# nanless/universal-speech-enhancement

Hardware: AMD Instinct MI355X
Metric: spectrogram-frames/sec through 30-step PC sampler, 24 kHz (higher is better)
Workload: dtype bf16; 1 GPU; configs[1]: NCSN++ Large score net, batch=8x4 s utterances per GPU, 30-step PC sampler (reverse_diffusion + langevin x1, snr 0.5, 60 NFE), bf16, hipGraph=on; global_batch=8, frames_per_utt=601, padded_frames_per_utt=640, n_freq=512, N=30, nfe=60, parallelism=utterance-sharded x1

## Files before the change

### include/use_hip.h

```cpp
#ifndef USE_HIP_H
#define USE_HIP_H

#include <stddef.h>
#include <stdint.h>

#ifdef __cplusplus
extern "C" {
#endif

typedef struct use_handle use_handle;
typedef void* use_stream_t;

enum { USE_OK = 0, USE_E_INVALID = -1, USE_E_HIP = -2, USE_E_STATE = -3, USE_E_NOMEM = -4 };
enum { USE_PREC_FP32 = 0, USE_PREC_BF16 = 1, USE_PREC_FP16 = 2 };
enum { USE_PRED_REVERSE_DIFFUSION = 0, USE_PRED_EULER_MARUYAMA = 1, USE_PRED_NONE = 2 };
enum { USE_CORR_NONE = 0, USE_CORR_LANGEVIN = 1, USE_CORR_ALD = 2 };

typedef struct use_config {
    int nf;
    int n_levels;
    int ch_mult[8];
    int num_res_blocks;
    int n_freq;
    int precision;
    float theta, sigma_min, sigma_max;
    int input_channels;
    int unconditional;
    int no_sigma_scale;
} use_config;

typedef struct use_sampler_config {
    int N;
    int predictor;
    int corrector;
    int corrector_steps;
    float snr;
    float t_eps;
    int use_graph;
} use_sampler_config;

int use_set_option(const char* name, long long value);
const char* use_last_error(void);
const char* use_version(void);

int use_create(const use_config* cfg, int device, use_handle** out);
int use_destroy(use_handle* h);

int use_set_weight(use_handle* h, const char* name, const float* data, const int64_t* shape, int ndim);
int use_commit_weights(use_handle* h);
int use_alloc_weight_blob(use_handle* h);
int use_weight_blob(use_handle* h, void** dev_ptr, size_t* bytes);
int use_save_weight_blob(use_handle* h, const char* path);
int use_load_weight_blob(use_handle* h, const char* path);
int use_num_expected_weights(use_handle* h);
int use_expected_weight(use_handle* h, int index, const char** name, int64_t* shape4, int* ndim);

int use_plan(use_handle* h, int B, int Tpad);
int use_workspace_bytes(use_handle* h, size_t* bytes);

int use_score(use_handle* h, const void* x, const void* y, const float* t, void* out, use_stream_t stream);
int use_score2(use_handle* h, const void* x, const void* y, const void* y2, const float* t, void* out, use_stream_t stream);

int use_set_sampler(use_handle* h, const use_sampler_config* sc);
int use_num_noise_draws(use_handle* h);
int use_get_timesteps(use_handle* h, float* out, int n);
int use_sample(use_handle* h, const void* y, const void* noise, uint64_t seed, void* out, use_stream_t stream);
int use_sample_cond(use_handle* h, const void* y, const void* cond, const void* noise, uint64_t seed, void* out, use_stream_t stream);
int use_sample_cond2(use_handle* h, const void* y, const void* cond, const void* cond2, const void* noise, uint64_t seed, void* out,
                     use_stream_t stream);

int use_sample_items(use_handle* h, const void* y, const void* cond, const void* cond2, const void* noise,
                     const uint64_t* seeds_host , void* out, use_stream_t stream);

typedef struct use_ode_config {
    float rtol, atol;
    float t_eps;
    int N;
    int group;
    int denoise;
    float first_step, max_step;
    int max_nfe;
    int use_graph;
} use_ode_config;
enum { USE_ODE_FINISHED = 0, USE_ODE_TOO_SMALL_STEP = -1, USE_ODE_MAX_NFE = -2 };
int use_set_ode(use_handle* h, const use_ode_config* cfg);
int use_sample_ode(use_handle* h, const void* y, const void* cond, const void* cond2, const void* noise, uint64_t seed, void* out,
                   int* nfev, int* status, use_stream_t stream);
typedef struct use_ode use_ode;
int use_ode_create(use_handle* h, int B, int64_t n_per_item, const use_ode_config* cfg, use_ode** out);
int use_ode_start(use_ode* o, const void* y_sde, const void* x0, use_stream_t stream);
int use_ode_request(use_ode* o, void* x, float* t, use_stream_t stream);
int use_ode_supply(use_ode* o, const void* f, int kind, use_stream_t stream);
int use_ode_result(use_ode* o, void* out, int* nfev, int* status, use_stream_t stream);
int use_ode_state(use_ode* o, double* t, double* h_abs, int* nfev, int* status, int* steps, use_stream_t stream);
int use_ode_num_groups(use_ode* o);
int use_ode_destroy(use_ode* o);

int use_sde_prior(use_handle* h, const void* y, const void* noise, uint64_t seed, void* x, int64_t n, use_stream_t s);
int use_sde_predictor(use_handle* h, int predictor, float t, int N, const void* x, const void* y, const void* score,
                      const void* noise, uint64_t seed, void* x_out, void* x_mean, int64_t n, use_stream_t s);
int use_sde_corrector(use_handle* h, int corrector, float t, float snr, int B, const void* x, const void* score,
                      const void* noise, uint64_t seed, void* x_out, void* x_mean, int64_t n, use_stream_t s);

int use_fill_noise(use_handle* h, uint64_t seed, int draw, void* out, int64_t n, use_stream_t s);

int use_fill_noise_items(use_handle* h, const uint64_t* seeds_host , int B, int draw, void* out,
                         int64_t n , use_stream_t s);

int use_forward(use_handle* h, const void* x, const void* y, const float* t, void* out, use_stream_t stream);

int use_spec_fwd(const void* stft, void* Y, int B, int F, int T, int Tpad, float factor, float exponent, use_stream_t s);
int use_spec_back(const void* X, void* stft, int B, int F, int T, int Tpad, float factor, float exponent, use_stream_t s);

int use_stft_fwd(const float* wav, void* Y, int B, int L, int n_fft, int hop, const float* window, int Tpad, float factor,
                 float exponent, use_stream_t s);
int use_istft_back(const void* X, float* wav, int B, int L, int n_fft, int hop, const float* window, int Tpad, float factor,
                   float exponent, use_stream_t s);

int use_chunk_count(int Tp, int C, int overlap);
int use_chunk_split(const void* Y, void* chunks, int B, int F, int Tp, int C, int overlap, use_stream_t s);
int use_chunk_merge(const void* chunks, void* X, int B, int F, int Tp, int C, int overlap, use_stream_t s);

enum { USE_METRIC_SI_SDR = 0, USE_METRIC_SI_SIR = 1, USE_METRIC_SI_SAR = 2, USE_METRIC_LSD = 3, USE_METRIC_COUNT = 4 };
size_t use_metrics_workspace(int B, int stride);
int use_metrics(const float* est, const float* clean, const float* noise, const int* len_host, int B, int stride, void* work,
                size_t work_bytes, double* out_dev, use_stream_t s);

int use_get_stat(use_handle* h, const char* name, long long* value);
int use_profile_score(use_handle* h, const void* x, const void* y, const float* t, void* out, use_stream_t stream,
                      double* conv_ms, double* conv_flops, double* conv_bytes, int* conv_launches, double* total_ms);
int use_profile_aux(use_handle* h, int index, char* name, int name_cap, int* H, int* W, double* bytes, double* ms);
int use_profile_aux_flops(use_handle* h, int index, double* flops);
typedef struct use_conv_case {
    int B, H, W, C0, C1, Cout, XC0, XC1;
    int act, gn, temb, res, stats;
    int dtype;
    int variant, iters;
} use_conv_case;
int use_conv_bench(const use_conv_case* c, float* out_host, float* stats_host, double* ms_avg, double* flops);
typedef struct use_conv_op {
    int B, H, W, C0, C1, Cout, XC0, XC1, ntaps, act, dtype, out_dtype, variant;
    const void *src0, *src1;
    const float* coef;
    const float* w;
    const float* bias;
    const float* temb;
    const void *x0, *x1;
    const float* w2;
    const void* res;
    float out_scale;
    void* out;
    long long* stats;
    const float* pyr;
    const float* w4;
    const float* b4;
    const long long *gn_st0, *gn_st1;
    const float *gn_gamma, *gn_beta;
    int gn_groups;
    float gn_eps;
    int temb_bstride;
} use_conv_op;
int use_op_conv(const use_conv_op* c, use_stream_t stream);
size_t use_op_conv_dev_workspace(const use_conv_op* c);
int use_op_conv_dev(const use_conv_op* c, int w_mode, void* work, size_t work_bytes, use_stream_t stream);
int use_op_fir(const void* src, int dtype, const float* coef, int act, void* out_act, void* out_raw, int B, int H, int W, int C, int up,
               use_stream_t stream);
int use_op_attention(const void* q, const void* k, const void* v, void* out, int dtype, int B, int N, int C, use_stream_t stream);
int use_op_gn_finalize(const long long* st0, int C0, const long long* st1, int C1, const float* gamma, const float* beta, int groups,
                       int hw, float eps, float* coef, int B, use_stream_t stream);
int use_op_attn_block(const void* x, const long long* gn_st, const float* gamma, const float* beta, int groups, float eps, const void* wq,
                      const void* wk, const void* wv, const void* wo, const float* bq, const float* bk, const float* bv, const float* bo,
                      void* out, long long* stats, int dtype, int B, int N, int C, use_stream_t stream);
int use_op_combine_add(void* h, int dtype, const float* pyr, const float* w8, const float* b8, long long* stats, int B, int64_t pix_per_b, int C,
                       use_stream_t stream);
int use_op_temb_mlp(const float* t, int t_stride, const float* gfp_w, const float* w1, const float* b1, const float* w2, const float* b2,
                    float* out_silu, int B, int nf, use_stream_t stream);
int use_op_temb_dense(const float* silu_temb, const float* W, const float* bias, float* out, int B, int rows, int dim, use_stream_t stream);
int use_op_score_out(const float* pyr, int pc, const float* t, int t_stride, const float* w, const float* bias, void* score, int B,
                     int64_t pix_per_b, float sign, use_stream_t stream);
int use_op_pack_input(const void* x, const void* y, const void* y2, float* x4, int64_t npix, use_stream_t stream);
int use_op_softmax_rows(void* x, int dtype, int64_t rows, int cols, use_stream_t stream);
int use_op_transpose_nc(const void* in, void* out, int dtype, int B, int N, int C, use_stream_t stream);
size_t use_op_wgrad_workspace(int B, int H, int W, int Cout, int Cin, int ntaps, int dtype);
int use_op_wgrad(const void* dy, const void* x, int dtype, float* dw, float* db, int B, int H, int W, int Cout, int Cin, int ntaps, float alpha,
                 float* work, size_t work_floats, use_stream_t stream);
size_t use_op_gn_workspace(int B, int C, int groups);
int use_op_gn_act_bwd(const void* x, const void* dy, int dtype, const float* gamma, const float* beta, int groups, float eps, int act, const void* add,
                      float add_scale, int B, int HW, int C, float* work, int have_stats, void* dx, float* dgamma, float* dbeta, use_stream_t stream);
int use_op_gn_act_fwd(const void* x, int dtype, const float* gamma, const float* beta, int groups, float eps, int act, int B, int HW, int C, float* work,
                      void* y, use_stream_t stream);
int use_op_colsum(const void* x, int dtype, int B, int HW, int C, float scale, float* out, float* work, use_stream_t stream);
int use_op_dense_bwd(const float* g, const float* temb, const float* Wd, int B, int K, int Cout, float* dW, float* db, float* dtemb,
                     use_stream_t stream);
int use_op_attention_bwd(const float* q, const float* k, const float* v, const float* dO, float* work, float* dq, float* dk, float* dv, int B, int N,
                         int C, use_stream_t stream);
enum { USE_WAV_PCM16 = 0, USE_WAV_FLOAT32 = 1 };
int use_wav_read(const char* path, double** samples, int64_t* frames, int* channels, int* sample_rate);
int use_wav_write(const char* path, const float* samples, int64_t frames, int channels, int sample_rate, int subtype);
int use_resample_fft(const double* x, int64_t n, int64_t num, double* y);
int use_load_utterance(const char* path, int target_rate, int normalize, float** wav, int64_t* length, int* sample_rate);
void use_free(void* p);

int use_timesteps(int N, float t_eps, float* out);
int use_debug_tensor(use_handle* h, const char* name, void** dev_ptr, int* dims4, int* dtype);
double use_flops_per_score(use_handle* h);

#ifdef __cplusplus
}
#endif
#endif
```

### universal_speech_enhancement_amd/_lib.py

```python
from __future__ import annotations

import ctypes as C
import os

_HERE = os.path.dirname(os.path.abspath(__file__))
LIB_PATH = os.environ.get("USE_HIP_LIB") or os.path.join(_HERE, "libuse_hip.so")

PREC = {"fp32": 0, "bf16": 1, "fp16": 2}
PREDICTORS = {"reverse_diffusion": 0, "euler_maruyama": 1, "none": 2}
CORRECTORS = {"none": 0, "langevin": 1, "ald": 2}


class UseConfig(C.Structure):
    _fields_ = [("nf", C.c_int), ("n_levels", C.c_int), ("ch_mult", C.c_int * 8), ("num_res_blocks", C.c_int),
                ("n_freq", C.c_int), ("precision", C.c_int), ("theta", C.c_float), ("sigma_min", C.c_float),
                ("sigma_max", C.c_float), ("input_channels", C.c_int), ("unconditional", C.c_int),
                ("no_sigma_scale", C.c_int)]


class UseSamplerConfig(C.Structure):
    _fields_ = [("N", C.c_int), ("predictor", C.c_int), ("corrector", C.c_int), ("corrector_steps", C.c_int),
                ("snr", C.c_float), ("t_eps", C.c_float), ("use_graph", C.c_int)]


class UseOdeConfig(C.Structure):
    _fields_ = [("rtol", C.c_float), ("atol", C.c_float), ("t_eps", C.c_float), ("N", C.c_int), ("group", C.c_int), ("denoise", C.c_int),
                ("first_step", C.c_float), ("max_step", C.c_float), ("max_nfe", C.c_int), ("use_graph", C.c_int)]


class UseConvCase(C.Structure):
    _fields_ = [(k, C.c_int) for k in ("B", "H", "W", "C0", "C1", "Cout", "XC0", "XC1", "act", "gn", "temb", "res", "stats",
                                       "dtype", "variant", "iters")]


class UseConvOp(C.Structure):
    _fields_ = ([(k, C.c_int) for k in ("B", "H", "W", "C0", "C1", "Cout", "XC0", "XC1", "ntaps", "act", "dtype", "out_dtype", "variant")] +
                [(k, C.c_void_p) for k in ("src0", "src1", "coef", "w", "bias", "temb", "x0", "x1", "w2", "res")] +
                [("out_scale", C.c_float), ("out", C.c_void_p), ("stats", C.c_void_p)] +
                [(k, C.c_void_p) for k in ("pyr", "w4", "b4", "gn_st0", "gn_st1", "gn_gamma", "gn_beta")] +
                [("gn_groups", C.c_int), ("gn_eps", C.c_float), ("temb_bstride", C.c_int)])


class UseHipError(RuntimeError):
    pass


_lib = None

_vp, _i, _i64, _u64, _f = C.c_void_p, C.c_int, C.c_int64, C.c_uint64, C.c_float
SYMBOLS = {
    "use_set_option": (C.c_int, [C.c_char_p, C.c_longlong]),
    "use_last_error": (C.c_char_p, []),
    "use_version": (C.c_char_p, []),
    "use_create": (_i, [C.POINTER(UseConfig), _i, C.POINTER(_vp)]),
    "use_destroy": (_i, [_vp]),
    "use_set_weight": (_i, [_vp, C.c_char_p, _vp, C.POINTER(_i64), _i]),
    "use_commit_weights": (_i, [_vp]),
    "use_alloc_weight_blob": (_i, [_vp]),
    "use_weight_blob": (_i, [_vp, C.POINTER(_vp), C.POINTER(C.c_size_t)]),
    "use_save_weight_blob": (C.c_int, [C.c_void_p, C.c_char_p]),
    "use_load_weight_blob": (C.c_int, [C.c_void_p, C.c_char_p]),
    "use_num_expected_weights": (_i, [_vp]),
    "use_expected_weight": (_i, [_vp, _i, C.POINTER(C.c_char_p), C.POINTER(_i64), C.POINTER(_i)]),
    "use_plan": (_i, [_vp, _i, _i]),
    "use_workspace_bytes": (_i, [_vp, C.POINTER(C.c_size_t)]),
    "use_score": (_i, [_vp, _vp, _vp, _vp, _vp, _vp]),
    "use_forward": (_i, [_vp, _vp, _vp, _vp, _vp, _vp]),
    "use_score2": (_i, [_vp, _vp, _vp, _vp, _vp, _vp, _vp]),
    "use_sample_cond2": (_i, [_vp, _vp, _vp, _vp, _vp, _u64, _vp, _vp]),
    "use_sample_items": (_i, [_vp, _vp, _vp, _vp, _vp, C.POINTER(_u64), _vp, _vp]),
    "use_set_sampler": (_i, [_vp, C.POINTER(UseSamplerConfig)]),
    "use_num_noise_draws": (_i, [_vp]),
    "use_get_timesteps": (_i, [_vp, C.POINTER(_f), _i]),
    "use_sample": (_i, [_vp, _vp, _vp, _u64, _vp, _vp]),
    "use_sample_cond": (_i, [_vp, _vp, _vp, _vp, _u64, _vp, _vp]),
    "use_set_ode": (_i, [_vp, C.POINTER(UseOdeConfig)]),
    "use_sample_ode": (_i, [_vp, _vp, _vp, _vp, _vp, _u64, _vp, C.POINTER(_i), C.POINTER(_i), _vp]),
    "use_ode_create": (_i, [_vp, _i, _i64, C.POINTER(UseOdeConfig), C.POINTER(_vp)]),
    "use_ode_start": (_i, [_vp, _vp, _vp, _vp]),
    "use_ode_request": (_i, [_vp, _vp, _vp, _vp]),
    "use_ode_supply": (_i, [_vp, _vp, _i, _vp]),
    "use_ode_result": (_i, [_vp, _vp, C.POINTER(_i), C.POINTER(_i), _vp]),
    "use_ode_state": (_i, [_vp, C.POINTER(C.c_double), C.POINTER(C.c_double), C.POINTER(_i), C.POINTER(_i), C.POINTER(_i), _vp]),
    "use_ode_num_groups": (_i, [_vp]),
    "use_ode_destroy": (_i, [_vp]),
    "use_spec_fwd": (_i, [_vp, _vp, _i, _i, _i, _i, C.c_float, C.c_float, _vp]),
    "use_spec_back": (_i, [_vp, _vp, _i, _i, _i, _i, C.c_float, C.c_float, _vp]),
    "use_stft_fwd": (_i, [_vp, _vp, _i, _i, _i, _i, _vp, _i, C.c_float, C.c_float, _vp]),
    "use_istft_back": (_i, [_vp, _vp, _i, _i, _i, _i, _vp, _i, C.c_float, C.c_float, _vp]),
    "use_chunk_count": (_i, [_i, _i, _i]),
    "use_chunk_split": (_i, [_vp, _vp, _i, _i, _i, _i, _i, _vp]),
    "use_chunk_merge": (_i, [_vp, _vp, _i, _i, _i, _i, _i, _vp]),
    "use_metrics_workspace": (C.c_size_t, [_i, _i]),
    "use_metrics": (_i, [_vp, _vp, _vp, C.POINTER(_i), _i, _i, _vp, C.c_size_t, _vp, _vp]),
    "use_sde_prior": (_i, [_vp, _vp, _vp, _u64, _vp, _i64, _vp]),
    "use_fill_noise": (_i, [_vp, _u64, _i, _vp, _i64, _vp]),
    "use_fill_noise_items": (_i, [_vp, C.POINTER(_u64), _i, _i, _vp, _i64, _vp]),
    "use_sde_predictor": (_i, [_vp, _i, _f, _i, _vp, _vp, _vp, _vp, _u64, _vp, _vp, _i64, _vp]),
    "use_sde_corrector": (_i, [_vp, _i, _f, _f, _i, _vp, _vp, _vp, _u64, _vp, _vp, _i64, _vp]),
    "use_debug_tensor": (_i, [_vp, C.c_char_p, C.POINTER(_vp), C.POINTER(_i), C.POINTER(_i)]),
    "use_flops_per_score": (C.c_double, [_vp]),
    "use_get_stat": (_i, [_vp, C.c_char_p, C.POINTER(C.c_longlong)]),
    "use_profile_aux": (_i, [_vp, _i, C.c_char_p, _i, C.POINTER(_i), C.POINTER(_i), C.POINTER(C.c_double), C.POINTER(C.c_double)]),
    "use_profile_aux_flops": (_i, [_vp, _i, C.POINTER(C.c_double)]),
    "use_profile_score": (_i, [_vp, _vp, _vp, _vp, _vp, _vp, C.POINTER(C.c_double), C.POINTER(C.c_double), C.POINTER(C.c_double), C.POINTER(_i), C.POINTER(C.c_double)]),
    "use_timesteps": (_i, [_i, _f, C.POINTER(_f)]),
    "use_conv_bench": (_i, [C.POINTER(UseConvCase), _vp, _vp, C.POINTER(C.c_double), C.POINTER(C.c_double)]),
    "use_op_conv": (_i, [C.POINTER(UseConvOp), _vp]),
    "use_op_conv_dev_workspace": (C.c_size_t, [C.POINTER(UseConvOp)]),
    "use_op_conv_dev": (_i, [C.POINTER(UseConvOp), _i, _vp, C.c_size_t, _vp]),
    "use_op_fir": (_i, [_vp, _i, _vp, _i, _vp, _vp, _i, _i, _i, _i, _i, _vp]),
    "use_op_attention": (_i, [_vp, _vp, _vp, _vp, _i, _i, _i, _i, _vp]),
    "use_op_gn_finalize": (_i, [_vp, _i, _vp, _i, _vp, _vp, _i, _i, _f, _vp, _i, _vp]),
    "use_op_attn_block": (_i, [_vp, _vp, _vp, _vp, _i, _f, _vp, _vp, _vp, _vp, _vp, _vp, _vp, _vp, _vp, _vp, _i, _i, _i, _i, _vp]),
    "use_op_combine_add": (_i, [_vp, _i, _vp, _vp, _vp, _vp, _i, _i64, _i, _vp]),
    "use_op_temb_mlp": (_i, [_vp, _i, _vp, _vp, _vp, _vp, _vp, _vp, _i, _i, _vp]),
    "use_op_temb_dense": (_i, [_vp, _vp, _vp, _vp, _i, _i, _i, _vp]),
    "use_op_score_out": (_i, [_vp, _i, _vp, _i, _vp, _vp, _vp, _i, _i64, _f, _vp]),
    "use_op_pack_input": (_i, [_vp, _vp, _vp, _vp, _i64, _vp]),
    "use_op_softmax_rows": (_i, [_vp, _i, _i64, _i, _vp]),
    "use_op_transpose_nc": (_i, [_vp, _vp, _i, _i, _i, _i, _vp]),
    "use_op_wgrad_workspace": (C.c_size_t, [_i, _i, _i, _i, _i, _i, _i]),
    "use_op_wgrad": (_i, [_vp, _vp, _i, _vp, _vp, _i, _i, _i, _i, _i, _i, _f, _vp, C.c_size_t, _vp]),
    "use_op_gn_workspace": (C.c_size_t, [_i, _i, _i]),
    "use_op_gn_act_bwd": (_i, [_vp, _vp, _i, _vp, _vp, _i, _f, _i, _vp, _f, _i, _i, _i, _vp, _i, _vp, _vp, _vp, _vp]),
    "use_op_gn_act_fwd": (_i, [_vp, _i, _vp, _vp, _i, _f, _i, _i, _i, _i, _vp, _vp, _vp]),
    "use_op_colsum": (_i, [_vp, _i, _i, _i, _i, _f, _vp, _vp, _vp]),
    "use_op_attention_bwd": (_i, [_vp, _vp, _vp, _vp, _vp, _vp, _vp, _vp, _i, _i, _i, _vp]),
    "use_op_dense_bwd": (_i, [_vp, _vp, _vp, _i, _i, _i, _vp, _vp, _vp, _vp]),
    "use_wav_read": (_i, [C.c_char_p, C.POINTER(C.POINTER(C.c_double)), C.POINTER(_i64), C.POINTER(_i), C.POINTER(_i)]),
    "use_wav_write": (_i, [C.c_char_p, _vp, _i64, _i, _i, _i]),
    "use_resample_fft": (_i, [_vp, _i64, _i64, _vp]),
    "use_load_utterance": (_i, [C.c_char_p, _i, _i, C.POINTER(C.POINTER(C.c_float)), C.POINTER(_i64), C.POINTER(_i)]),
    "use_free": (None, [_vp]),
}


def lib() -> C.CDLL:
    global _lib
    if _lib is None:
        if not os.path.exists(LIB_PATH):
            raise UseHipError(
                f"{LIB_PATH} not found: the HIP extension is not built (run __graft_entry__.build()). "
                "There is no CPU fallback for the sampling path.")
        L = C.CDLL(LIB_PATH)
        for name, (res, args) in SYMBOLS.items():
            if os.environ.get("USE_HIP_LIB") and not hasattr(L, name):
                continue
            fn = getattr(L, name)
            fn.restype, fn.argtypes = res, args
        for kv in filter(None, os.environ.get("USE_HIP_OPTS", "").split(",")):
            k, sep, v = kv.partition("=")
            if not sep or not k.strip():
                raise UseHipError(f"USE_HIP_OPTS: entry {kv!r} is not name=value")
            try:
                iv = int(v)
            except ValueError:
                raise UseHipError(f"USE_HIP_OPTS: {kv!r}: the value must be an integer") from None
            if L.use_set_option(k.strip().encode(), iv) < 0:
                raise UseHipError(f"USE_HIP_OPTS: {kv}: " + L.use_last_error().decode(errors="replace"))
        _lib = L
    return _lib


def check(rc: int, what: str = "") -> int:
    if rc < 0:
        msg = lib().use_last_error().decode(errors="replace")
        raise UseHipError(f"{what or 'libuse_hip'} failed ({rc}): {msg}")
    return rc
```

### universal_speech_enhancement_amd/csrc/use_engine.cpp

```cpp
#include "../../include/use_hip.h"
#include "use_kernels.h"

#include <hip/hip_runtime.h>

#include <algorithm>
#include <cmath>
#include <cstdarg>
#include <cstdio>
#include <cstdlib>
#include <cstring>
#include <map>
#include <mutex>
#include <string>
#include <unordered_map>
#include <vector>

using namespace use;

static thread_local std::string g_err;
static int fail(int code, const char* fmt, ...) {
    char buf[1024];
    va_list ap; va_start(ap, fmt); vsnprintf(buf, sizeof buf, fmt, ap); va_end(ap);
    g_err = buf;
    return code;
}
int use_set_error(int code, const char* msg) { g_err = msg ? msg : ""; return code; }
#define HIPCHK(expr)                                                                                         \
    do {                                                                                                     \
        hipError_t e_ = (expr);                                                                              \
        if (e_ != hipSuccess) return fail(USE_E_HIP, "%s failed: %s (%s:%d)", #expr, hipGetErrorString(e_), __FILE__, __LINE__); \
    } while (0)

static inline uint16_t f32_to_bf16(float f) {
    uint32_t u; memcpy(&u, &f, 4);
    if ((u & 0x7fffffffu) > 0x7f800000u) return (uint16_t)((u >> 16) | 0x40);
    u += 0x7fffu + ((u >> 16) & 1u);
    return (uint16_t)(u >> 16);
}

static inline uint16_t f32_to_f16(float f) {
    uint32_t u; memcpy(&u, &f, 4);
    const uint32_t sign = (u >> 16) & 0x8000u;
    u &= 0x7fffffffu;
    if (u > 0x7f800000u) return (uint16_t)(sign | 0x7e00u);
    if (u >= 0x477ff000u) return (uint16_t)(sign | 0x7c00u);
    if (u < 0x38800000u) {
        if (u < 0x33000000u) return (uint16_t)sign;
        const int shift = 126 - (int)(u >> 23);
        uint32_t m = (u & 0x7fffffu) | 0x800000u;
        const uint32_t half = 1u << (shift - 1), rest = m & ((1u << shift) - 1);
        m >>= shift;
        if (rest > half || (rest == half && (m & 1))) ++m;
        return (uint16_t)(sign | m);
    }
    uint32_t v = u - 0x38000000u;
    const uint32_t rest = v & 0x1fffu;
    v >>= 13;
    if (rest > 0x1000u || (rest == 0x1000u && (v & 1))) ++v;
    return (uint16_t)(sign | v);
}

struct ConvW { std::string wname, bname; int cin = 0, cout = 0, cout_pad = 0, ntaps = 1, w_dtype = DT_F32;
               bool nin = false; size_t w_off = 0, b_off = 0;
               int cin_src = 0, cout_src = 0;
               size_t wb_off = 0; bool has_wb = false;
               bool split_in = false; };
struct GNW { std::string prefix; int C = 0; size_t g_off = 0, b_off = 0; };
struct ResW { int idx = 0, in_ch = 0, out_ch = 0; bool up = false, down = false, has_c2 = false;
              GNW gn0, gn1; ConvW c0, c1, c2; int dense_row0 = 0; size_t b12_off = 0; };
struct CombineW { int idx = 0, C = 0; size_t w_off = 0, b_off = 0; };
struct AttnW { int idx = 0, C = 0; GNW gn; ConvW q, k, v, o; };
struct PyrW { GNW gn; ConvW conv; };

struct Expected { std::string name; std::vector<int64_t> shape; };

constexpr int MAX_SUB = 8;

struct Act { void* p = nullptr; int C = 0, H = 0, W = 0, dtype = DT_F32; long long* stats = nullptr;
             long long* part = nullptr; int ntiles = 0; };

struct Arena {
    char* base = nullptr; size_t cap = 0, off = 0, peak = 0;
    bool overflow = false;
    bool* dry_on_overflow = nullptr;
    void reset() { off = 0; }
    void* alloc(size_t bytes) {
        off = (off + 255) & ~(size_t)255;
        void* p = base ? (void*)(base + off) : nullptr;
        off += bytes;
        if (off > peak) peak = off;
        if (base && off > cap) {
            overflow = true;
            if (dry_on_overflow) *dry_on_overflow = true;
            p = base;
        }
        return p;
    }
};

struct use_handle {
    use_config cfg{};
    int device = 0;
    int act_dtype = DT_F32;
    std::vector<Expected> expected;
    std::unordered_map<std::string, size_t> expected_index;
    ConvW conv_in;
    std::vector<ResW> res;
    std::vector<CombineW> combines;
    AttnW attn;
    std::vector<PyrW> pyrs;
    int dense_rows = 0;
    size_t gfp_off = 0, l1w_off = 0, l1b_off = 0, l2w_off = 0, l2b_off = 0, dense_w_off = 0, dense_b_off = 0,
           outw_off = 0, outb_off = 0;
    size_t blob_bytes = 0;
    std::unordered_map<std::string, std::vector<float>> host_w;
    char* blob = nullptr; bool weights_ready = false;
    int B = 0, T = 0;
    Arena arena;
    char* persist = nullptr; size_t persist_bytes = 0;
    size_t arena_alloc = 0, persist_alloc = 0;
    size_t arena_plan_bytes = 0;
    float *x4 = nullptr, *silu_temb = nullptr, *tembias = nullptr, *t_dev = nullptr;
    float2 *Y = nullptr, *X = nullptr, *Xmean = nullptr, *score = nullptr, *xin = nullptr;
    float2 *cond_buf = nullptr, *cond2_buf = nullptr;
    int pcp = 4;
    float2 *Cond = nullptr;
    float *lang_partial = nullptr, *lang_step = nullptr;
    unsigned long long* rng_state = nullptr;
    unsigned long long* item_seeds = nullptr;
    float* item_step = nullptr;
    int lang_blocks = 0;
    use_sampler_config sc{};
    bool sampler_set = false;
    std::vector<float> timesteps;
    float* ts_dev = nullptr; float* temb_table = nullptr; float* silu_table = nullptr;
    float2* noise_copy = nullptr; size_t noise_copy_bytes = 0;
    hipStream_t cap_stream = nullptr;
    int nsub = 1, sub_B[MAX_SUB] = {};
    Arena sub_arena[MAX_SUB];
    Arena st_arena[MAX_SUB];
    hipStream_t aux_stream[MAX_SUB] = {};
    hipEvent_t ev_fork = nullptr, ev_stagger[MAX_SUB] = {},
               ev_join[MAX_SUB] = {};
    int debug_B = 0;
    std::vector<hipGraphExec_t> graph_exec[4];
    hipGraphExec_t score_graph = nullptr;
    use_ode_config oc{};
    bool ode_set = false;
    use_ode* ode_run = nullptr;
    hipGraphExec_t ode_graph = nullptr;
    std::vector<const void*> ode_graph_key;
    long long ode_steps = 0, ode_rejected = 0, ode_nfev_max = 0;
    struct PlanState;
    std::vector<PlanState*> plan_cache;
    long long opt_gen_at_plan = -1;
    long long n_graph_captures = 0, n_plans_built = 0, n_plan_cache_hits = 0;
    char* sde_buf = nullptr; unsigned long long* sde_rng = nullptr; float* sde_step = nullptr; float* sde_partial = nullptr; unsigned long long* sde_seeds = nullptr;
    static constexpr int SDE_MAX_B = 1024, SDE_BLOCKS = 128;
    bool profile = false, profile_all = false; std::vector<std::pair<hipEvent_t, hipEvent_t>> prof_events; std::vector<double> prof_flops, prof_bytes; std::vector<char> prof_main; std::vector<std::pair<int, int>> prof_hw;
    struct AuxProf { std::string name; int H = 0, W = 0; double bytes = 0.0; hipEvent_t e0 = nullptr, e1 = nullptr; double ms = 0.0; double flops = 0.0; };
    std::vector<AuxProf> prof_aux;
    std::vector<std::string> prof_desc;
    bool dry = false;
    std::map<std::string, Act> debug;
    double flops = 0.0;
};

static void add_expected(use_handle* h, const std::string& name, std::vector<int64_t> shape) {
    h->expected_index[name] = h->expected.size();
    h->expected.push_back({name, std::move(shape)});
}

static ConvW make_conv(use_handle* h, const std::string& prefix, int cin, int cout, int ntaps, int w_dtype,
                       int cin_src = 0, int cout_src = 0) {
    ConvW c; c.wname = prefix + ".weight"; c.bname = prefix + ".bias"; c.cin = cin; c.cout = cout; c.ntaps = ntaps;
    c.w_dtype = w_dtype;
    c.cin_src = cin_src ? cin_src : cin; c.cout_src = cout_src ? cout_src : cout;
    c.cout_pad = cout <= 32 ? 32 : (cout + 127) / 128 * 128;
    const int k = ntaps == 9 ? 3 : 1;
    add_expected(h, c.wname, {c.cout_src, c.cin_src, k, k});
    add_expected(h, c.bname, {c.cout_src});
    return c;
}
static ConvW make_nin(use_handle* h, const std::string& prefix, int C, int w_dtype) {
    ConvW c; c.wname = prefix + ".W"; c.bname = prefix + ".b"; c.cin = C; c.cout = C; c.ntaps = 1; c.w_dtype = w_dtype;
    c.nin = true; c.cout_pad = (C + 127) / 128 * 128; c.cin_src = C; c.cout_src = C;
    add_expected(h, c.wname, {C, C});
    add_expected(h, c.bname, {C});
    return c;
}
static GNW make_gn(use_handle* h, const std::string& prefix, int C) {
    GNW g; g.prefix = prefix; g.C = C;
    add_expected(h, prefix + ".weight", {C});
    add_expected(h, prefix + ".bias", {C});
    return g;
}

static ResW make_res(use_handle* h, int idx, int in_ch, int out_ch, bool up, bool down) {
    const std::string p = "all_modules." + std::to_string(idx);
    const int dt = h->act_dtype;
    ResW r; r.idx = idx; r.in_ch = in_ch; r.out_ch = out_ch; r.up = up; r.down = down;
    r.gn0 = make_gn(h, p + ".GroupNorm_0", in_ch);
    r.c0 = make_conv(h, p + ".Conv_0", in_ch, out_ch, 9, dt);
    add_expected(h, p + ".Dense_0.weight", {out_ch, 4 * h->cfg.nf});
    add_expected(h, p + ".Dense_0.bias", {out_ch});
    r.dense_row0 = h->dense_rows; h->dense_rows += out_ch;
    r.gn1 = make_gn(h, p + ".GroupNorm_1", out_ch);
    r.c1 = make_conv(h, p + ".Conv_1", out_ch, out_ch, 9, dt);
    r.has_c2 = (in_ch != out_ch) || up || down;
    if (r.has_c2) r.c2 = make_conv(h, p + ".Conv_2", in_ch, out_ch, 1, dt);
    return r;
}

static int build_arch(use_handle* h) {
    const use_config& c = h->cfg;
    const int nf = c.nf, L = c.n_levels, nrb = c.num_res_blocks, dt = h->act_dtype;
    const int pc = c.input_channels ? c.input_channels : 4;
    const int pcp = pc > 4 ? 8 : 4;
    h->pcp = pcp;
    add_expected(h, "output_layer.weight", {2, pc, 1, 1});
    add_expected(h, "output_layer.bias", {2});
    int m = 0;
    add_expected(h, "all_modules.0.W", {nf}); m++;
    if (!c.unconditional) {
        add_expected(h, "all_modules.1.weight", {4 * nf, 2 * nf}); add_expected(h, "all_modules.1.bias", {4 * nf}); m++;
        add_expected(h, "all_modules.2.weight", {4 * nf, 4 * nf}); add_expected(h, "all_modules.2.bias", {4 * nf}); m++;
    }
    h->conv_in = make_conv(h, "all_modules." + std::to_string(m), pcp, nf, 9, DT_F32, pc, 0); m++;
    std::vector<int> hs_c{nf};
    int in_ch = nf;
    for (int lvl = 0; lvl < L; ++lvl) {
        for (int k = 0; k < nrb; ++k) {
            const int out_ch = nf * c.ch_mult[lvl];
            h->res.push_back(make_res(h, m++, in_ch, out_ch, false, false));
            in_ch = out_ch; hs_c.push_back(in_ch);
        }
        if (lvl != L - 1) {
            h->res.push_back(make_res(h, m++, in_ch, in_ch, false, true));
            CombineW cb; cb.idx = m; cb.C = in_ch;
            add_expected(h, "all_modules." + std::to_string(m) + ".Conv_0.weight", {in_ch, pc, 1, 1});
            add_expected(h, "all_modules." + std::to_string(m) + ".Conv_0.bias", {in_ch});
            h->combines.push_back(cb); m++;
            hs_c.push_back(in_ch);
        }
    }
    in_ch = hs_c.back();
    h->res.push_back(make_res(h, m++, in_ch, in_ch, false, false));
    {
        const std::string p = "all_modules." + std::to_string(m);
        h->attn.idx = m; h->attn.C = in_ch;
        h->attn.gn = make_gn(h, p + ".GroupNorm_0", in_ch);
        h->attn.q = make_nin(h, p + ".NIN_0", in_ch, dt);
        h->attn.k = make_nin(h, p + ".NIN_1", in_ch, dt);
        h->attn.v = make_nin(h, p + ".NIN_2", in_ch, dt);
        h->attn.o = make_nin(h, p + ".NIN_3", in_ch, dt);
        m++;
    }
    h->res.push_back(make_res(h, m++, in_ch, in_ch, false, false));
    for (int lvl = L - 1; lvl >= 0; --lvl) {
        for (int k = 0; k < nrb + 1; ++k) {
            const int out_ch = nf * c.ch_mult[lvl];
            const int skip = hs_c.back(); hs_c.pop_back();
            h->res.push_back(make_res(h, m++, in_ch + skip, out_ch, false, false));
            in_ch = out_ch;
        }
        PyrW pw;
        pw.gn = make_gn(h, "all_modules." + std::to_string(m), in_ch); m++;
        pw.conv = make_conv(h, "all_modules." + std::to_string(m), in_ch, pcp, 9, dt, 0, pc); m++;
        h->pyrs.push_back(pw);
        if (lvl != 0) h->res.push_back(make_res(h, m++, in_ch, in_ch, true, false));
    }
    if (!hs_c.empty()) return fail(USE_E_INVALID, "internal: skip stack not empty");

    size_t off = 0;
    auto take = [&](size_t bytes) { off = (off + 255) & ~(size_t)255; size_t o = off; off += bytes; return o; };
    auto lay_conv = [&](ConvW& w) {
        w.w_off = take((size_t)w.ntaps * w.cout_pad * w.cin * dtype_size(w.w_dtype));
        w.b_off = take((size_t)w.cout * 4);
        w.has_wb = !w.nin && w.cout_pad % 128 == 0 && w.cin % conv_v4_chunk(w.w_dtype) == 0 && (w.ntaps == 9 || w.ntaps == 1);
        if (w.has_wb) w.wb_off = take((size_t)w.ntaps * w.cout_pad * w.cin * dtype_size(w.w_dtype));
    };
    auto lay_conv_in = [&](ConvW& w) {
        lay_conv(w);
        if (dt != DT_F32 && w.cin == 4 && w.ntaps == 9 && w.cout_pad % 128 == 0) {
            w.split_in = true; w.has_wb = true;
            w.wb_off = take((size_t)w.cout_pad * CONV_IN_SPLIT_K * 2);
        }
    };
    auto lay_gn = [&](GNW& g) { g.g_off = take((size_t)g.C * 4); g.b_off = take((size_t)g.C * 4); };
    h->outw_off = take((size_t)2 * pcp * 4); h->outb_off = take(2 * 4);
    h->gfp_off = take((size_t)nf * 4);
    h->l1w_off = take((size_t)4 * nf * 2 * nf * 4); h->l1b_off = take((size_t)4 * nf * 4);
    h->l2w_off = take((size_t)4 * nf * 4 * nf * 4); h->l2b_off = take((size_t)4 * nf * 4);
    h->dense_w_off = take((size_t)h->dense_rows * 4 * nf * 4); h->dense_b_off = take((size_t)h->dense_rows * 4);
    lay_conv_in(h->conv_in);
    for (auto& r : h->res) {
        lay_gn(r.gn0); lay_conv(r.c0); lay_gn(r.gn1); lay_conv(r.c1);
        if (r.has_c2) { lay_conv(r.c2); r.b12_off = take((size_t)r.out_ch * 4); }
    }
    for (auto& cb : h->combines) { cb.w_off = take((size_t)cb.C * pcp * 4); cb.b_off = take((size_t)cb.C * 4); }
    lay_gn(h->attn.gn); lay_conv(h->attn.q); lay_conv(h->attn.k); lay_conv(h->attn.v); lay_conv(h->attn.o);
    for (auto& p : h->pyrs) { lay_gn(p.gn); lay_conv(p.conv); }
    h->blob_bytes = (off + 255) & ~(size_t)255;
    return USE_OK;
}

static void pack_conv_raw(const float* src, const ConvW& w, char* dst, char* dstb) {
    const size_t es = dtype_size(w.w_dtype);
    auto put = [&](char* base, size_t o, float v) {
        if (w.w_dtype == DT_F32) ((float*)base)[o] = v;
        else ((uint16_t*)base)[o] = w.w_dtype == DT_F16 ? f32_to_f16(v) : f32_to_bf16(v);
    };
    memset(dst, 0, (size_t)w.ntaps * w.cout_pad * w.cin * es);
    for (int tap = 0; tap < w.ntaps; ++tap)
        for (int co = 0; co < w.cout_src; ++co)
            for (int ci = 0; ci < w.cin_src; ++ci) {
                const float v = w.nin ? src[(size_t)ci * w.cout + co] : src[((size_t)co * w.cin_src + ci) * w.ntaps + tap];
                put(dst, ((size_t)co * w.ntaps + tap) * w.cin + ci, v);
            }
    if (dstb) {
        const int ck = conv_v4_chunk(w.w_dtype), nchunks = w.cin / ck;
        memset(dstb, 0, (size_t)w.ntaps * w.cout_pad * w.cin * es);
        for (int tap = 0; tap < w.ntaps; ++tap)
            for (int co = 0; co < w.cout_src; ++co)
                for (int ci = 0; ci < w.cin_src; ++ci) {
                    const float v = src[((size_t)co * w.cin_src + ci) * w.ntaps + tap];
                    const int vec = 16 / (int)es, e = ci % ck;
                    put(dstb, (((size_t)tap * nchunks + ci / ck) * w.cout_pad + co) * ck + (((e / vec) ^ ((co >> 2) & 3)) * vec + e % vec), v);
                }
    }
}
static void pack_conv_in_split(const float* src, const ConvW& w, char* dst) {
    uint16_t* d = (uint16_t*)dst;
    memset(dst, 0, (size_t)w.cout_pad * CONV_IN_SPLIT_K * 2);
    for (int co = 0; co < w.cout_src; ++co)
        for (int tap = 0; tap < 9; ++tap)
            for (int ci = 0; ci < w.cin_src; ++ci) {
                const float v = src[((size_t)co * w.cin_src + ci) * 9 + tap];
                const uint16_t hi = f32_to_bf16(v);
                uint32_t hb = (uint32_t)hi << 16; float hf; memcpy(&hf, &hb, 4);
                const uint16_t lo = f32_to_bf16(v - hf);
                uint16_t* row = d + (size_t)co * CONV_IN_SPLIT_K;
                row[(0 * 9 + tap) * 4 + ci] = hi; row[(1 * 9 + tap) * 4 + ci] = lo; row[(2 * 9 + tap) * 4 + ci] = hi;
            }
}
static void pack_conv(const use_handle* h, const ConvW& w, char* blob) {
    const std::vector<float>& bias = h->host_w.at(w.bname);
    pack_conv_raw(h->host_w.at(w.wname).data(), w, blob + w.w_off, (w.has_wb && !w.split_in) ? blob + w.wb_off : nullptr);
    if (w.split_in) pack_conv_in_split(h->host_w.at(w.wname).data(), w, blob + w.wb_off);
    memset(blob + w.b_off, 0, (size_t)w.cout * 4);
    memcpy(blob + w.b_off, bias.data(), (size_t)w.cout_src * 4);
}
static void pack_gn(const use_handle* h, const GNW& g, char* blob) {
    memcpy(blob + g.g_off, h->host_w.at(g.prefix + ".weight").data(), (size_t)g.C * 4);
    memcpy(blob + g.b_off, h->host_w.at(g.prefix + ".bias").data(), (size_t)g.C * 4);
}

static int pack_all(use_handle* h, char* blob) {
    for (const auto& e : h->expected)
        if (!h->host_w.count(e.name)) return fail(USE_E_STATE, "weight '%s' was never set", e.name.c_str());
    const int nf = h->cfg.nf;
    auto cp = [&](size_t off, const char* name) {
        const auto& v = h->host_w.at(name); memcpy(blob + off, v.data(), v.size() * 4);
    };
    const int pc = h->cfg.input_channels ? h->cfg.input_channels : 4;
    const int pcp = h->pcp;
    auto cp_rows = [&](size_t off, const std::string& name, int rows) {
        const auto& v = h->host_w.at(name);
        float* d = (float*)(blob + off);
        for (int r = 0; r < rows; ++r)
            for (int k = 0; k < pcp; ++k) d[r * pcp + k] = k < pc ? v[(size_t)r * pc + k] : 0.f;
    };
    cp_rows(h->outw_off, "output_layer.weight", 2); cp(h->outb_off, "output_layer.bias");
    cp(h->gfp_off, "all_modules.0.W");
    if (!h->cfg.unconditional) {
        cp(h->l1w_off, "all_modules.1.weight"); cp(h->l1b_off, "all_modules.1.bias");
        cp(h->l2w_off, "all_modules.2.weight"); cp(h->l2b_off, "all_modules.2.bias");
    }
    pack_conv(h, h->conv_in, blob);
    for (const auto& r : h->res) {
        pack_gn(h, r.gn0, blob); pack_conv(h, r.c0, blob); pack_gn(h, r.gn1, blob); pack_conv(h, r.c1, blob);
        const std::string p = "all_modules." + std::to_string(r.idx);
        if (r.has_c2) {
            pack_conv(h, r.c2, blob);
            const auto& b1 = h->host_w.at(p + ".Conv_1.bias"); const auto& b2 = h->host_w.at(p + ".Conv_2.bias");
            float* d = (float*)(blob + r.b12_off);
            for (int i = 0; i < r.out_ch; ++i) d[i] = b1[i] + b2[i];
        }
        memcpy(blob + h->dense_w_off + (size_t)r.dense_row0 * 4 * nf * 4, h->host_w.at(p + ".Dense_0.weight").data(),
               (size_t)r.out_ch * 4 * nf * 4);
        memcpy(blob + h->dense_b_off + (size_t)r.dense_row0 * 4, h->host_w.at(p + ".Dense_0.bias").data(),
               (size_t)r.out_ch * 4);
    }
    for (const auto& cb : h->combines) {
        const std::string p = "all_modules." + std::to_string(cb.idx);
        cp_rows(cb.w_off, p + ".Conv_0.weight", cb.C); cp(cb.b_off, (p + ".Conv_0.bias").c_str());
    }
    pack_gn(h, h->attn.gn, blob);
    pack_conv(h, h->attn.q, blob); pack_conv(h, h->attn.k, blob); pack_conv(h, h->attn.v, blob); pack_conv(h, h->attn.o, blob);
    for (const auto& p : h->pyrs) { pack_gn(h, p.gn, blob); pack_conv(h, p.conv, blob); }
    return USE_OK;
}

static int g_subbatch_min_items = 2;
static int g_subbatch = -1;
static long g_gn_inline = 128L * 160L;
static int g_attn_fused = 1;
static int g_stats_part = 1;
static int g_stagger_level = 2;

__global__ __launch_bounds__(256) void zero16_kernel(uint4* __restrict__ p, size_t n16) {
    for (size_t i = (size_t)blockIdx.x * 256 + threadIdx.x; i < n16; i += (size_t)gridDim.x * 256) p[i] = make_uint4(0, 0, 0, 0);
}

struct Fwd {
    use_handle* h; hipStream_t s;
    const float* tembias; int temb_bstride;
    const float* t; int t_stride;
    int B = 0;
    Arena* arena = nullptr;
    Arena* st_arena = nullptr;
    bool primary = true;
    hipEvent_t ev_stagger = nullptr;
    int stagger_level = 2;
    template <typename T> const T* W(size_t off) const { return (const T*)(h->blob + off); }

    Act new_act(int C, int H, int Wd, int dtype, bool stats) {
        Act a; a.C = C; a.H = H; a.W = Wd; a.dtype = dtype;
        a.p = arena->alloc((size_t)B * H * Wd * C * dtype_size(dtype));
        if (stats) a.stats = (long long*)st_arena->alloc((size_t)B * C * 2 * sizeof(long long));
        return a;
    }

    template <typename F> void timed_aux(const char* name, int Hm, int Wm, double bytes, F&& launch) {
        if (!h->profile) { launch(); return; }
        use_handle::AuxProf a{name, Hm, Wm, bytes, nullptr, nullptr, 0.0};
        (void)hipEventCreate(&a.e0); (void)hipEventCreate(&a.e1);
        (void)hipEventRecord(a.e0, s);
        launch();
        (void)hipEventRecord(a.e1, s);
        h->prof_aux.push_back(a);
    }

    float* gn_coef(const Act& a, const Act* a2, const GNW& g) {
        const int C = a.C + (a2 ? a2->C : 0);
        float* coef = (float*)arena->alloc((size_t)B * C * 2 * 4);
        if (!h->dry)
            launch_gn_finalize(a.stats, a.C, a2 ? a2->stats : nullptr, a2 ? a2->C : 0, W<float>(g.g_off), W<float>(g.b_off),
                               std::min(C / 4, 32), a.H * a.W, 1e-6f, coef, B, s, a.part, a.ntiles, a2 ? a2->part : nullptr, a2 ? a2->ntiles : 0);
        return coef;
    }

    Act conv(const Act& a, const Act* a2, const GNW* gn, int act, const ConvW& w, const float* temb,
             const Act* res, float scale, const float* pyr, const CombineW* cb, int out_dtype, bool stats,
             const Act* sx0 = nullptr, const Act* sx1 = nullptr, const ConvW* w2 = nullptr, size_t bias_off = 0) {
        Act o = new_act(w.cout, a.H, a.W, out_dtype, stats);
        double fl = 2.0 * B * a.H * a.W * (double)w.cout * w.cin * w.ntaps;
        if (w2) fl += 2.0 * B * a.H * a.W * (double)w2->cout * w2->cin;
        h->flops += fl;
        const float* coef_arr = (gn && (long)a.H * a.W > g_gn_inline) ? gn_coef(a, a2, *gn) : nullptr;
        const bool in_shape = a.dtype == DT_F32 && w.cin <= 8 && w.ntaps == 9 && out_dtype != DT_F32;
        const bool v4_shape = w.ntaps == 9 && w.cout > 32 && a.dtype == out_dtype && a.H % 16 == 0 && a.W % 32 == 0;
        const int part_rows = in_shape ? conv_in_split_wgs(a.H, a.W) : v4_shape ? conv_v4_tiles(a.H, a.W) : 0;
        long long* part = (stats && g_stats_part && part_rows > 0 && (long)a.H * a.W > g_gn_inline)
                              ? (long long*)arena->alloc((size_t)B * part_rows * w.cout * 2 * sizeof(long long)) : nullptr;
        if (h->dry) return o;
        ConvArgs p{};
        p.src0 = a.p; p.C0 = a.C; p.src1 = a2 ? a2->p : nullptr; p.C1 = a2 ? a2->C : 0; p.in_dtype = a.dtype;
        p.coef = coef_arr; p.act = act; p.w = h->blob + w.w_off; p.cout_pad = w.cout_pad;
        if (gn && !coef_arr) {
            const int C = a.C + (a2 ? a2->C : 0), groups = std::min(C / 4, 32);
            p.gn_st0 = a.stats; p.gn_st1 = a2 ? a2->stats : nullptr;
            p.gn_gamma = W<float>(gn->g_off); p.gn_beta = W<float>(gn->b_off); p.gn_groups = groups;
            p.gn_inv_n = 1.0f / ((float)(C / groups) * (float)(a.H * a.W)); p.gn_eps = 1e-6f;
        }
        p.wb = w.has_wb ? h->blob + w.wb_off : nullptr;
        p.bias = W<float>(w2 ? bias_off : w.b_off);
        if (w2) { p.x0 = sx0->p; p.XC0 = sx0->C; p.x1 = sx1 ? sx1->p : nullptr; p.XC1 = sx1 ? sx1->C : 0; p.w2 = h->blob + w2->w_off;
                  p.w2b = w2->has_wb ? h->blob + w2->wb_off : nullptr; }
        p.temb = temb; p.temb_bstride = temb_bstride;
        p.res = res ? res->p : nullptr; p.out_scale = scale;
        p.pyr = pyr; p.w4 = cb ? W<float>(cb->w_off) : nullptr; p.b4 = cb ? W<float>(cb->b_off) : nullptr;
        p.out = o.p; p.out_dtype = out_dtype; p.stats = o.stats;
        p.B = B; p.H = a.H; p.W = a.W; p.Cout = w.cout; p.ntaps = w.ntaps;
        const bool main_variant = conv_v4_eligible(p);
        if (const int nparts = part ? conv_stats_parts(p) : 0) {
            if (nparts <= part_rows) { p.stats_part = part; p.stats = nullptr; o.part = part; o.ntiles = nparts; }
        }
        if (gn && !coef_arr && (a.part || (a2 && a2->part))) { arena->overflow = true; h->dry = true; return o; }
        if (h->profile && (main_variant || (h->profile_all && conv_v2_eligible(p)))) {
            hipEvent_t e0, e1; (void)hipEventCreate(&e0); (void)hipEventCreate(&e1);
            (void)hipEventRecord(e0, s);
            launch_conv(p, s);
            (void)hipEventRecord(e1, s);
            h->prof_events.push_back({e0, e1});
            h->prof_flops.push_back(fl); h->prof_main.push_back(main_variant); h->prof_hw.push_back({a.H, a.W});
            {
                const double es = (double)dtype_size(a.dtype), px = (double)B * a.H * a.W;
                double by = px * (w.cin + (w2 ? w2->cin : 0)) * es + px * w.cout * dtype_size(out_dtype) * (res ? 2.0 : 1.0);
                by += (double)w.ntaps * w.cin * w.cout * es + (w2 ? (double)w2->cin * w2->cout * es : 0.0);
                if (pyr) by += px * 4 * 4;
                h->prof_bytes.push_back(by);
            }
            char d[160]; snprintf(d, sizeof d, "%-28s H=%3d W=%3d Cin=%3d Cout=%3d taps=%d gn=%d res=%d sc=%d", w.wname.c_str(), a.H, a.W, w.cin, w.cout, w.ntaps, gn != nullptr, res != nullptr, w2 ? w2->cin : 0);
            h->prof_desc.push_back(d);
        } else if (h->profile && w.ntaps == 9 && w.cout > 8 && !(a.dtype == DT_F32 && w.cin <= 8)) {
            const double es = (double)dtype_size(a.dtype), px = (double)B * a.H * a.W;
            double by = px * (w.cin + (w2 ? w2->cin : 0)) * es + px * w.cout * dtype_size(out_dtype) * (res ? 2.0 : 1.0);
            by += (double)w.ntaps * w.cin * w.cout * es + (w2 ? (double)w2->cin * w2->cout * es : 0.0);
            timed_aux(conv_sk_eligible(p) ? "conv_sk" : conv_v2_eligible(p) ? "conv_v2" : "conv_generic", a.H, a.W, by, [&] { launch_conv(p, s); });
            h->prof_aux.back().flops = fl;
        } else if (h->profile && (w.cout <= 8 || (a.dtype == DT_F32 && w.cin <= 8))) {
            const double px = (double)B * a.H * a.W;
            const double by = px * w.cin * dtype_size(a.dtype) + px * w.cout * dtype_size(out_dtype) * (res ? 2.0 : 1.0) + (double)w.ntaps * w.cin * w.cout * dtype_size(a.dtype);
            timed_aux(w.cout <= 8 ? "pyr_conv" : "conv_in", a.H, a.W, by, [&] { launch_conv(p, s); });
        } else {
            launch_conv(p, s);
        }
        return o;
    }

    Act resblock(const Act& x, const Act* skip, const ResW& r, const float* pyr = nullptr, const CombineW* cb = nullptr) {
        const float rs = 0.70710678118654752440f;
        const float* temb = tembias ? tembias + r.dense_row0 : nullptr;
        const int dt = h->act_dtype;
        Act hcur, xr;
        const Act* sx0 = &x; const Act* sx1 = skip;
        if (r.up || r.down) {
            const int H2 = r.up ? x.H * 2 : x.H / 2, W2 = r.up ? x.W * 2 : x.W / 2;
            Act hr = new_act(x.C, H2, W2, dt, false);
            xr = new_act(x.C, H2, W2, dt, false);
            float* coef0 = gn_coef(x, skip, r.gn0);
            if (!h->dry) {
                const double by = (double)B * x.H * x.W * x.C * dtype_size(dt) + 2.0 * B * H2 * W2 * x.C * dtype_size(dt);
                if (r.up) timed_aux("fir_up", x.H, x.W, by, [&] { launch_fir_up2(x.p, dt, coef0, 1, hr.p, xr.p, B, x.H, x.W, x.C, s); });
                else      timed_aux("fir_down", x.H, x.W, by, [&] { launch_fir_down2(x.p, dt, coef0, 1, hr.p, xr.p, B, x.H, x.W, x.C, s); });
            }
            hcur = conv(hr, nullptr, nullptr, 0, r.c0, temb, nullptr, 1.f, nullptr, nullptr, dt, true);
            sx0 = &xr; sx1 = nullptr;
        } else {
            hcur = conv(x, skip, &r.gn0, 1, r.c0, temb, nullptr, 1.f, nullptr, nullptr, dt, true);
        }
        if (r.has_c2)
            return conv(hcur, nullptr, &r.gn1, 1, r.c1, nullptr, nullptr, rs, pyr, cb, dt, true, sx0, sx1, &r.c2, r.b12_off);
        return conv(hcur, nullptr, &r.gn1, 1, r.c1, nullptr, &x, rs, pyr, cb, dt, true);
    }

    Act attention(const Act& x, const AttnW& aw) {
        const int dt = h->act_dtype;
        if (g_attn_fused && x.stats && attn_fused_eligible(dt, x.H * x.W, x.C)) {
            Act o = new_act(x.C, x.H, x.W, dt, true);
            h->flops += 4.0 * 2.0 * B * x.H * x.W * (double)x.C * x.C;
            if (h->dry) return o;
            if (x.part) { arena->overflow = true; h->dry = true; return o; }
            AttnArgs a{};
            a.x = x.p; a.out = o.p; a.N = x.H * x.W;
            a.gn_st = x.stats; a.gn_gamma = W<float>(aw.gn.g_off); a.gn_beta = W<float>(aw.gn.b_off); a.gn_groups = std::min(x.C / 4, 32); a.gn_eps = 1e-6f;
            a.wq = h->blob + aw.q.w_off; a.wk = h->blob + aw.k.w_off; a.wv = h->blob + aw.v.w_off; a.wo = h->blob + aw.o.w_off;
            a.bq = W<float>(aw.q.b_off); a.bk = W<float>(aw.k.b_off); a.bv = W<float>(aw.v.b_off); a.bo = W<float>(aw.o.b_off);
            a.stats = o.stats;
            launch_attn_fused(a, dt, B, s);
            return o;
// ... 35 lines not shown
        }
        return conv(a, nullptr, nullptr, 0, aw.o, nullptr, &x, 0.70710678118654752440f, nullptr, nullptr, dt, true);
    }

    Act run(const float* x4) {
        use_handle* H = h;
        const use_config& c = H->cfg;
        const int L = c.n_levels, nrb = c.num_res_blocks, dt = H->act_dtype;
        arena->reset();
        st_arena->reset();
        if (!H->dry && st_arena->base) {
            const size_t n16 = st_arena->cap / 16;
            hipLaunchKernelGGL(zero16_kernel, dim3((unsigned)std::min<size_t>((n16 + 255) / 256, 1024)), dim3(256), 0, s, (uint4*)st_arena->base, n16);
        }
        if (primary) { H->flops = 0.0; H->debug.clear(); H->debug_B = B; }
        const int pcp = H->pcp;
        Act xin; xin.p = (void*)x4; xin.C = pcp; xin.H = c.n_freq; xin.W = H->T; xin.dtype = DT_F32;
        std::vector<Act> hs;
        hs.push_back(conv(xin, nullptr, nullptr, 0, H->conv_in, nullptr, nullptr, 1.f, nullptr, nullptr, dt, true));
        if (primary) H->debug["h_in"] = hs.back();
        Act ipyr = xin;
        size_t ri = 0, ci = 0;
        for (int lvl = 0; lvl < L; ++lvl) {
            for (int k = 0; k < nrb; ++k) hs.push_back(resblock(hs.back(), nullptr, H->res[ri++]));
            if (lvl == std::min(stagger_level, L - 1) && ev_stagger && !H->dry) (void)hipEventRecord(ev_stagger, s);
            if (lvl != L - 1) {
                Act nip = new_act(pcp, ipyr.H / 2, ipyr.W / 2, DT_F32, false);
                if (!H->dry) launch_fir_down2(ipyr.p, DT_F32, nullptr, 0, nullptr, nip.p, B, ipyr.H, ipyr.W, pcp, s);
                ipyr = nip;
                if (pcp == 4) {
                    hs.push_back(resblock(hs.back(), nullptr, H->res[ri++], (const float*)ipyr.p, &H->combines[ci++]));
                } else {
                    Act o = resblock(hs.back(), nullptr, H->res[ri++]);
                    const CombineW& cb = H->combines[ci++];
                    if (!H->dry) {
                        hipLaunchKernelGGL(zero16_kernel, dim3((unsigned)(((size_t)B * o.C + 255) / 256)), dim3(256), 0, s, (uint4*)o.stats,
                                           (size_t)B * o.C);
                        launch_combine_add(o.p, o.dtype, (const float*)ipyr.p, W<float>(cb.w_off), W<float>(cb.b_off), o.stats, B,
                                           (long)o.H * o.W, o.C, s);
                    }
                    o.part = nullptr; o.ntiles = 0;
                    hs.push_back(o);
                }
            }
        }
        if (primary) H->debug["down_out"] = hs.back();
        Act hc = resblock(hs.back(), nullptr, H->res[ri++]);
        if (primary) H->debug["pre_attn"] = hc;
        hc = attention(hc, H->attn);
        if (primary) H->debug["post_attn"] = hc;
        hc = resblock(hc, nullptr, H->res[ri++]);
        Act pyr; bool have_pyr = false; size_t pi = 0;
        for (int lvl = L - 1; lvl >= 0; --lvl) {
            for (int k = 0; k < nrb + 1; ++k) {
                Act sk = hs.back(); hs.pop_back();
                hc = resblock(hc, &sk, H->res[ri++]);
            }
            const PyrW& pw = H->pyrs[pi++];
            if (!have_pyr) {
                pyr = conv(hc, nullptr, &pw.gn, 1, pw.conv, nullptr, nullptr, 1.f, nullptr, nullptr, DT_F32, false);
                have_pyr = true;
            } else {
                Act up = new_act(pcp, pyr.H * 2, pyr.W * 2, DT_F32, false);
                if (!H->dry) launch_fir_up2(pyr.p, DT_F32, nullptr, 0, nullptr, up.p, B, pyr.H, pyr.W, pcp, s);
                pyr = conv(hc, nullptr, &pw.gn, 1, pw.conv, nullptr, &up, 1.f, nullptr, nullptr, DT_F32, false);
            }
            if (lvl != 0) hc = resblock(hc, nullptr, H->res[ri++]);
        }
        if (primary) H->debug["h_last"] = hc;
        if (primary) H->debug["pyramid"] = pyr;
        return pyr;
    }
};

static void run_temb(use_handle* h, const float* t, int n, float* silu_buf, float* out, hipStream_t s) {
    const int nf = h->cfg.nf;
    launch_temb_mlp(t, 1, (const float*)(h->blob + h->gfp_off), (const float*)(h->blob + h->l1w_off),
                    (const float*)(h->blob + h->l1b_off), (const float*)(h->blob + h->l2w_off),
                    (const float*)(h->blob + h->l2b_off), silu_buf, n, nf, s);
    launch_temb_dense(silu_buf, (const float*)(h->blob + h->dense_w_off), (const float*)(h->blob + h->dense_b_off), out,
                      n, h->dense_rows, 4 * nf, s);
}

static void run_score(use_handle* h, const float2* x, const float2* y, const float* tembias, int temb_bstride,
                      const float* t, int t_stride, float2* out, hipStream_t s, float sign = -1.f, const float2* y2 = nullptr) {
    if (h->cfg.no_sigma_scale) t = nullptr;
    const long n_per_b = (long)h->cfg.n_freq * h->T;
    const int pcp = h->pcp;
    launch_pack_input(x, y, y2, h->x4, (long)h->B * n_per_b, s);
    const float* outw = (const float*)(h->blob + h->outw_off); const float* outb = (const float*)(h->blob + h->outb_off);
    if (h->nsub == 1) {
        Fwd f0{h, s, tembias, temb_bstride, t, t_stride};
        f0.B = h->B; f0.arena = &h->arena; f0.st_arena = &h->st_arena[0];
        Act pyr = f0.run(h->x4);
        if (!h->dry) launch_score_out((const float*)pyr.p, pcp, t, t_stride, outw, outb, out, h->B, n_per_b, sign, s);
        return;
    }
    const bool overlap = !h->profile;
    if (overlap) (void)hipEventRecord(h->ev_fork, s);
    int b0 = 0;
    for (int i = 0; i < h->nsub; ++i) {
        hipStream_t si = (i == 0 || !overlap) ? s : h->aux_stream[i];
        if (overlap && i) {
            (void)hipStreamWaitEvent(si, h->ev_fork, 0);
            (void)hipStreamWaitEvent(si, h->ev_stagger[i - 1], 0);
        }
        Fwd f{h, si, tembias ? tembias + (size_t)b0 * temb_bstride : nullptr, temb_bstride,
              t ? t + (size_t)b0 * t_stride : nullptr, t_stride};
        f.B = h->sub_B[i]; f.arena = i ? &h->sub_arena[i] : &h->arena; f.st_arena = &h->st_arena[i]; f.primary = i == 0;
        if (overlap && i + 1 < h->nsub) { f.ev_stagger = h->ev_stagger[i]; f.stagger_level = g_stagger_level; }
        Act pyr = f.run(h->x4 + (size_t)b0 * n_per_b * pcp);
        if (!h->dry)
        launch_score_out((const float*)pyr.p, pcp, t ? t + (size_t)b0 * t_stride : nullptr, t_stride, outw, outb,
                         out + (size_t)b0 * n_per_b, h->sub_B[i], n_per_b, sign, si);
        if (overlap && i) (void)hipEventRecord(h->ev_join[i], si);
        b0 += h->sub_B[i];
    }
    if (overlap)
        for (int i = 1; i < h->nsub; ++i) (void)hipStreamWaitEvent(s, h->ev_join[i], 0);
}

static double ouve_logsig(const use_config& c) { return std::log((double)c.sigma_max / (double)c.sigma_min); }
static float ouve_std(const use_config& c, float t) {
    const double th = c.theta, ls = ouve_logsig(c), sm = c.sigma_min, tt = t;
    return (float)std::sqrt(sm * sm * std::exp(-2 * th * tt) * (std::exp(2 * (th + ls) * tt) - 1) * ls / (th + ls));
}
static float ouve_diffusion(const use_config& c, float t) {
    const float sigma = c.sigma_min * std::pow(c.sigma_max / c.sigma_min, t);
    return (float)((double)sigma * std::sqrt(2 * ouve_logsig(c)));
}
static void linspace_f32(float start, float end, int steps, std::vector<float>& out) {
    out.resize(steps);
    if (steps == 1) { out[0] = start; return; }
    const float step = (end - start) / (float)(steps - 1);
    const int half = steps / 2;
    for (int i = 0; i < steps; ++i) out[i] = i < half ? std::fmaf(step, (float)i, start) : std::fmaf(-step, (float)(steps - 1 - i), end);
}

static void predictor_coeffs(const use_config& c, int predictor, float t, int N, float& cd, float& cs, float& cn) {
    const float g = ouve_diffusion(c, t);
    if (predictor == USE_PRED_REVERSE_DIFFUSION) {
        const float dt = (float)(1.0 / N);
        const float G = g * std::sqrt(dt);
        cd = c.theta * dt; cs = G * G; cn = G;
    } else {
        const double dt = 1.0 / N;
        cd = (float)(c.theta * dt); cs = (float)((double)(g * g) * dt); cn = (float)((double)g * std::sqrt(dt));
    }
}

__global__ void set_rng_kernel(unsigned long long* st, unsigned long long seed, unsigned long long base) { st[0] = seed; st[1] = base; }
__global__ void fill_f32_kernel(float* p, float v, int n) { for (int i = threadIdx.x; i < n; i += blockDim.x) p[i] = v; }

static void run_sampler(use_handle* h, const float2* noise, hipStream_t s, int i0, int i1, bool per_item = false) {
    const use_sampler_config& sc = h->sc;
    const long n = (long)h->B * h->cfg.n_freq * h->T, n_per_b = (long)h->cfg.n_freq * h->T;
    const int ncorr = sc.corrector == USE_CORR_NONE ? 0 : sc.corrector_steps;
    struct PerImage { bool on; PerImage(bool o) : on(o) { if (on) conv_sk_set_per_image(true); } ~PerImage() { if (on) conv_sk_set_per_image(false); } } per_image(per_item);
    auto nz = [&](unsigned d) { return noise ? noise + (size_t)d * n : nullptr; };
    unsigned d = 1 + (unsigned)i0 * (unsigned)(ncorr + (sc.predictor == USE_PRED_NONE ? 0 : 1));
    if (i0 == 0) {
        if (per_item) launch_prior_items(h->Y, nz(0), ItemRng{h->item_seeds, 0}, ouve_std(h->cfg, 1.0f), h->X, h->B, n_per_b, s);
        else launch_prior(h->Y, nz(0), RngRef{h->rng_state, 0}, ouve_std(h->cfg, 1.0f), h->X, n, s);
    }
    for (int i = i0; i < i1; ++i) {
        const float t = h->timesteps[i];
        const float* temb = h->temb_table + (size_t)i * h->dense_rows;
        for (int k = 0; k < ncorr; ++k) {
            run_score(h, h->X, h->Cond, temb, 0, h->ts_dev + i, 0, h->score, s, -1.f, h->pcp == 8 ? h->cond2_buf : nullptr);
            RngRef rr{h->rng_state, d};
            ItemRng ir{h->item_seeds, d};
            if (per_item && sc.corrector == USE_CORR_LANGEVIN) {
                launch_langevin_norms_items(h->score, nz(d), ir, h->lang_partial, h->B, n_per_b, h->lang_blocks, s);
                launch_langevin_step_items(h->lang_partial, h->B, h->lang_blocks, sc.snr, h->item_step, s);
                launch_corrector_items(h->X, h->score, nz(d), ir, h->item_step, 0.f, h->X, nullptr, h->B, n_per_b, s);
            } else if (per_item) {
                const float sd = sc.snr * ouve_std(h->cfg, t);
                launch_corrector_items(h->X, h->score, nz(d), ir, nullptr, sd * sd * 2.f, h->X, nullptr, h->B, n_per_b, s);
            } else if (sc.corrector == USE_CORR_LANGEVIN) {
                launch_langevin_norms(h->score, nz(d), rr, h->lang_partial, h->B, n_per_b, h->lang_blocks, s);
                launch_langevin_step(h->lang_partial, h->B, h->lang_blocks, sc.snr, h->lang_step, s);
                launch_corrector(h->X, h->score, nz(d), rr, h->lang_step, 0.f, h->X, nullptr, n, s);
            } else {
                const float sd = sc.snr * ouve_std(h->cfg, t);
                launch_corrector(h->X, h->score, nz(d), rr, nullptr, sd * sd * 2.f, h->X, nullptr, n, s);
            }
            d++;
        }
        if (sc.predictor == USE_PRED_NONE) {
            if (i == sc.N - 1) (void)hipMemcpyAsync(h->Xmean, h->X, (size_t)n * 8, hipMemcpyDeviceToDevice, s);
        } else {
            run_score(h, h->X, h->Cond, temb, 0, h->ts_dev + i, 0, h->score, s, -1.f, h->pcp == 8 ? h->cond2_buf : nullptr);
            float cd, cs, cn; predictor_coeffs(h->cfg, sc.predictor, t, sc.N, cd, cs, cn);
            if (per_item)
                launch_predictor_items(h->X, h->Y, h->score, nz(d), ItemRng{h->item_seeds, d}, cd, cs, cn, h->X,
                                       i == sc.N - 1 ? h->Xmean : nullptr, h->B, n_per_b, s);
            else
            launch_predictor(h->X, h->Y, h->score, nz(d), RngRef{h->rng_state, d}, cd, cs, cn, h->X,
                             i == sc.N - 1 ? h->Xmean : nullptr, n, s);
            d++;
        }
    }
}

static void drop_graphs(use_handle* h) {
    for (auto& v : h->graph_exec) { for (auto g : v) if (g) (void)hipGraphExecDestroy(g); v.clear(); }
    if (h->score_graph) { (void)hipGraphExecDestroy(h->score_graph); h->score_graph = nullptr; }
    if (h->ode_graph) { (void)hipGraphExecDestroy(h->ode_graph); h->ode_graph = nullptr; }
}

#define USE_PLAN_FIELDS(X)                                                                                            \
    X(B) X(T) X(nsub) X(arena) X(arena_alloc) X(arena_plan_bytes) X(persist) X(persist_bytes) X(persist_alloc) X(x4) X(silu_temb) X(tembias) X(t_dev) \
    X(Y) X(X) X(Xmean) X(score) X(xin) X(cond_buf) X(cond2_buf) X(Cond) X(lang_partial) X(lang_step) X(rng_state) X(item_seeds) X(item_step) X(lang_blocks)   \
    X(sc) X(sampler_set) X(timesteps) X(ts_dev) X(temb_table) X(silu_table) X(noise_copy) X(noise_copy_bytes) X(score_graph)      \
    X(debug) X(debug_B) X(opt_gen_at_plan) X(oc) X(ode_set)
struct use_handle::PlanState {
#define X(f) decltype(use_handle::f) f;
    USE_PLAN_FIELDS(X)
#undef X
    int sub_B[MAX_SUB]; Arena sub_arena[MAX_SUB], st_arena[MAX_SUB];
    std::vector<hipGraphExec_t> graph_exec[4];
};
static long long g_opt_gen = 0;
static int g_plan_cache = 4;
static void plan_stash(use_handle* h, use_handle::PlanState& p) {
#define X(f) p.f = std::move(h->f);
    USE_PLAN_FIELDS(X)
#undef X
    for (int i = 0; i < MAX_SUB; ++i) { p.sub_B[i] = h->sub_B[i]; p.sub_arena[i] = h->sub_arena[i]; p.st_arena[i] = h->st_arena[i]; }
    for (int i = 0; i < 4; ++i) { p.graph_exec[i] = std::move(h->graph_exec[i]); h->graph_exec[i].clear(); }
    h->B = h->T = 0; h->arena = Arena{}; h->arena_alloc = 0; h->persist = nullptr; h->persist_bytes = h->persist_alloc = 0;
    h->ts_dev = h->temb_table = h->silu_table = nullptr; h->noise_copy = nullptr; h->noise_copy_bytes = 0; h->score_graph = nullptr;
    h->sampler_set = false; h->timesteps.clear(); h->debug.clear(); h->ode_set = false;
}
static void plan_restore(use_handle* h, use_handle::PlanState& p) {
#define X(f) h->f = std::move(p.f);
    USE_PLAN_FIELDS(X)
#undef X
    for (int i = 0; i < MAX_SUB; ++i) { h->sub_B[i] = p.sub_B[i]; h->sub_arena[i] = p.sub_arena[i]; h->st_arena[i] = p.st_arena[i]; }
    for (int i = 0; i < 4; ++i) h->graph_exec[i] = std::move(p.graph_exec[i]);
}
static void plan_free(use_handle::PlanState* p) {
    for (auto& v : p->graph_exec) for (auto g : v) if (g) (void)hipGraphExecDestroy(g);
    if (p->score_graph) (void)hipGraphExecDestroy(p->score_graph);
    if (p->arena.base) (void)hipFree(p->arena.base);
    if (p->persist) (void)hipFree(p->persist);
    if (p->temb_table) (void)hipFree(p->temb_table);
    if (p->silu_table) (void)hipFree(p->silu_table);
    if (p->ts_dev) (void)hipFree(p->ts_dev);
    if (p->noise_copy) (void)hipFree(p->noise_copy);
    delete p;
}
static void plan_cache_clear(use_handle* h) {
    for (auto* p : h->plan_cache) plan_free(p);
    h->plan_cache.clear();
}

static int ensure_sde_scratch(use_handle* h) {
    if (!h) return fail(USE_E_INVALID, "null handle");
    HIPCHK(hipSetDevice(h->device));
    if (!h->sde_buf) {
        const size_t part = (size_t)use_handle::SDE_MAX_B * use_handle::SDE_BLOCKS * 2 * 4;
        const size_t bytes = 512 + part + (size_t)use_handle::SDE_MAX_B * 8;
        HIPCHK(hipMalloc((void**)&h->sde_buf, bytes));
        HIPCHK(hipMemset(h->sde_buf, 0, bytes));
        h->sde_rng = (unsigned long long*)h->sde_buf; h->sde_step = (float*)(h->sde_buf + 256);
        h->sde_partial = (float*)(h->sde_buf + 512); h->sde_seeds = (unsigned long long*)(h->sde_buf + 512 + part);
    }
    return USE_OK;
}

static int ensure_cap_stream(use_handle* h) {
    if (!h->cap_stream) HIPCHK(hipStreamCreateWithFlags(&h->cap_stream, hipStreamNonBlocking));
    return USE_OK;
}

extern "C" {

int use_get_stat(use_handle* h, const char* name, long long* value) {
    if (!h || !name || !value) return fail(USE_E_INVALID, "null argument");
    if (!strcmp(name, "graph_captures")) { *value = h->n_graph_captures; return USE_OK; }
    if (!strcmp(name, "plans_built")) { *value = h->n_plans_built; return USE_OK; }
    if (!strcmp(name, "plan_cache_hits")) { *value = h->n_plan_cache_hits; return USE_OK; }
    if (!strcmp(name, "plans_parked")) { *value = (long long)h->plan_cache.size(); return USE_OK; }
    if (!strcmp(name, "ode_steps")) { *value = h->ode_steps; return USE_OK; }
    if (!strcmp(name, "ode_rejected")) { *value = h->ode_rejected; return USE_OK; }
    if (!strcmp(name, "ode_nfev_max")) { *value = h->ode_nfev_max; return USE_OK; }
    if (!strcmp(name, "plan_stale")) { *value = h->B && h->opt_gen_at_plan != g_opt_gen ? 1 : 0; return USE_OK; }
    return fail(USE_E_INVALID, "unknown statistic '%s'", name);
}

int use_set_option(const char* name, long long value) {
    if (!name) return fail(USE_E_INVALID, "option name is null");
    ++g_opt_gen;
    if (!strcmp(name, "attn_fused")) { g_attn_fused = (int)value; return USE_OK; }
    if (!strcmp(name, "plan_cache")) { g_plan_cache = (int)std::max(0LL, std::min(16LL, value)); return USE_OK; }
    if (!strcmp(name, "subbatch_min_items")) { g_subbatch_min_items = (int)std::max(1LL, value); return USE_OK; }
    if (!strcmp(name, "subbatch")) { g_subbatch = (int)value; return USE_OK; }
    if (!strcmp(name, "stagger_level")) { g_stagger_level = (int)value; return USE_OK; }
    if (!strcmp(name, "stats_part")) { g_stats_part = (int)value; return USE_OK; }
    if (!strcmp(name, "gn_inline")) { g_gn_inline = (long)value; return USE_OK; }
    if (!strcmp(name, "conv_v4_min_blocks")) { conv_v4_set_min_blocks((long)value); return USE_OK; }
    if (!strcmp(name, "conv_v5")) { conv_v5_set((int)value); return USE_OK; }
    if (!strcmp(name, "fir_strip")) { fir_set_strip((int)value); return USE_OK; }
    if (!strcmp(name, "pyr_ws")) { pyr_conv_set_ws((int)value); return USE_OK; }
    if (!strcmp(name, "wgrad_mfma16")) { wgrad_set_mfma16((int)value); return USE_OK; }
    if (!strcmp(name, "wgrad_blocks")) { wgrad_set_blocks((int)value); return USE_OK; }
    if (!strcmp(name, "conv_in_wgs")) { if (value < 1 || value > 4096) return fail(USE_E_INVALID, "conv_in_wgs: 1 ... 4096"); g_conv_in_wgs = (int)value; return USE_OK; }
    if (!strcmp(name, "conv_sk_max_px")) { conv_sk_set_max_px((long)value); return USE_OK; }
    return fail(USE_E_INVALID, "unknown option '%s'", name);
}
const char* use_last_error(void) { return g_err.c_str(); }
const char* use_version(void) { return "use_hip 0.1 (gfx950)"; }

int use_create(const use_config* cfg, int device, use_handle** out) {
    if (!cfg || !out) return fail(USE_E_INVALID, "null argument");
    if (cfg->n_levels < 1 || cfg->n_levels > 8 || cfg->nf % 32 != 0 || cfg->nf < 32 || cfg->num_res_blocks < 1)
        return fail(USE_E_INVALID, "unsupported architecture (nf must be a multiple of 32, 1..8 levels)");
    for (int i = 0; i < cfg->n_levels; ++i)
        if (cfg->ch_mult[i] < 1 || cfg->nf * cfg->ch_mult[i] > 512) return fail(USE_E_INVALID, "unsupported architecture (1 <= nf * ch_mult <= 512)");
    if (cfg->n_freq % (1 << (cfg->n_levels - 1)) != 0)
        return fail(USE_E_INVALID, "n_freq=%d is not divisible by 2^(levels-1)", cfg->n_freq);
    if (cfg->precision != USE_PREC_FP32 && cfg->precision != USE_PREC_BF16 && cfg->precision != USE_PREC_FP16) return fail(USE_E_INVALID, "bad precision");
    if (cfg->input_channels != 0 && cfg->input_channels != 2 && cfg->input_channels != 4 && cfg->input_channels != 6)
        return fail(USE_E_INVALID, "input_channels must be 4 (x and y), 6 (x, y and a second conditioning) or 2 (y alone), got %d", cfg->input_channels);
    use_handle* h = new use_handle();
    h->cfg = *cfg; h->device = device;
    h->act_dtype = cfg->precision == USE_PREC_BF16 ? DT_BF16 : cfg->precision == USE_PREC_FP16 ? DT_F16 : DT_F32;
    int rc = build_arch(h);
    if (rc) { delete h; return rc; }
    *out = h;
    return USE_OK;
}

int use_destroy(use_handle* h) {
    if (!h) return USE_OK;
    (void)hipSetDevice(h->device);
    (void)hipDeviceSynchronize();
    drop_graphs(h); plan_cache_clear(h);
    if (h->ode_run) (void)use_ode_destroy(h->ode_run);
    if (h->cap_stream) (void)hipStreamDestroy(h->cap_stream);
    for (int i = 0; i < MAX_SUB; ++i) {
        if (h->aux_stream[i]) (void)hipStreamDestroy(h->aux_stream[i]);
        if (h->ev_stagger[i]) { (void)hipEventDestroy(h->ev_stagger[i]); (void)hipEventDestroy(h->ev_join[i]); }
    }
    if (h->ev_fork) (void)hipEventDestroy(h->ev_fork);
    if (h->blob) (void)hipFree(h->blob);
    if (h->arena.base) (void)hipFree(h->arena.base);
    if (h->persist) (void)hipFree(h->persist);
    if (h->temb_table) (void)hipFree(h->temb_table);
    if (h->silu_table) (void)hipFree(h->silu_table);
    if (h->ts_dev) (void)hipFree(h->ts_dev);
    if (h->noise_copy) (void)hipFree(h->noise_copy);
    if (h->sde_buf) (void)hipFree(h->sde_buf);
    delete h;
    return USE_OK;
}

int use_num_expected_weights(use_handle* h) { return h ? (int)h->expected.size() : USE_E_INVALID; }
int use_expected_weight(use_handle* h, int index, const char** name, int64_t* shape4, int* ndim) {
    if (!h || index < 0 || index >= (int)h->expected.size()) return fail(USE_E_INVALID, "bad index");
    const Expected& e = h->expected[index];
    if (name) *name = e.name.c_str();
    if (ndim) *ndim = (int)e.shape.size();
    if (shape4) for (size_t i = 0; i < 4; ++i) shape4[i] = i < e.shape.size() ? e.shape[i] : 1;
    return USE_OK;
}

int use_set_weight(use_handle* h, const char* name, const float* data, const int64_t* shape, int ndim) {
    if (!h || !name || !data || !shape) return fail(USE_E_INVALID, "null argument");
    auto it = h->expected_index.find(name);
    if (it == h->expected_index.end()) return fail(USE_E_INVALID, "unexpected weight name '%s'", name);
    const Expected& e = h->expected[it->second];
    if ((int)e.shape.size() != ndim) return fail(USE_E_INVALID, "weight '%s': rank %d, expected %zu", name, ndim, e.shape.size());
    size_t n = 1;
    for (int i = 0; i < ndim; ++i) {
        if (shape[i] != e.shape[i]) return fail(USE_E_INVALID, "weight '%s': dim %d is %lld, expected %lld", name, i, (long long)shape[i], (long long)e.shape[i]);
        n *= (size_t)shape[i];
    }
    h->host_w[name].assign(data, data + n);
    h->weights_ready = false;
    return USE_OK;
}

int use_alloc_weight_blob(use_handle* h) {
    if (!h) return fail(USE_E_INVALID, "null handle");
    HIPCHK(hipSetDevice(h->device));
    if (!h->blob) HIPCHK(hipMalloc((void**)&h->blob, h->blob_bytes));
    h->weights_ready = true;
    h->sampler_set = false;
    drop_graphs(h); plan_cache_clear(h);
    return USE_OK;
}

int use_commit_weights(use_handle* h) {
    if (!h) return fail(USE_E_INVALID, "null handle");
    HIPCHK(hipSetDevice(h->device));
    std::vector<char> host(h->blob_bytes, 0);
    int rc = pack_all(h, host.data());
    if (rc) return rc;
    if (!h->blob) HIPCHK(hipMalloc((void**)&h->blob, h->blob_bytes));
    HIPCHK(hipMemcpy(h->blob, host.data(), h->blob_bytes, hipMemcpyHostToDevice));
    h->host_w.clear();
    h->weights_ready = true;
    h->sampler_set = false;
    drop_graphs(h); plan_cache_clear(h);
    return USE_OK;
}

namespace {
constexpr uint32_t BLOB_LAYOUT = 7;
struct BlobHeader {
    char magic[8];
    uint32_t header_bytes, layout;
    int32_t nf, n_levels, ch_mult[8], num_res_blocks, precision, input_channels, unconditional, no_sigma_scale;
    uint32_t crc32, reserved;
    uint64_t blob_bytes;
};
uint32_t crc32_of(const unsigned char* p, size_t n) {
    static uint32_t table[256]; static bool init = false;
    if (!init) {
        for (uint32_t i = 0; i < 256; ++i) { uint32_t c = i; for (int k = 0; k < 8; ++k) c = c & 1 ? 0xEDB88320u ^ (c >> 1) : c >> 1; table[i] = c; }
        init = true;
    }
    uint32_t c = 0xFFFFFFFFu;
    for (size_t i = 0; i < n; ++i) c = table[(c ^ p[i]) & 0xFF] ^ (c >> 8);
    return c ^ 0xFFFFFFFFu;
}
BlobHeader make_header(const use_handle* h) {
    BlobHeader hd{};
    memcpy(hd.magic, "USEHIPWB", 8);
    hd.header_bytes = sizeof(BlobHeader); hd.layout = BLOB_LAYOUT;
    const use_config& c = h->cfg;
    hd.nf = c.nf; hd.n_levels = c.n_levels; for (int i = 0; i < 8; ++i) hd.ch_mult[i] = i < c.n_levels ? c.ch_mult[i] : 0;
    hd.num_res_blocks = c.num_res_blocks; hd.precision = c.precision;
    hd.input_channels = c.input_channels ? c.input_channels : 4; hd.unconditional = c.unconditional != 0; hd.no_sigma_scale = c.no_sigma_scale != 0;
    hd.blob_bytes = h->blob_bytes;
    return hd;
}
}

int use_save_weight_blob(use_handle* h, const char* path) {
    if (!h || !path) return fail(USE_E_INVALID, "null argument");
    std::vector<char> host(h->blob_bytes, 0);
    if (!h->host_w.empty()) {
        int rc = pack_all(h, host.data());
        if (rc) return rc;
    } else if (h->blob && h->weights_ready) {
        HIPCHK(hipSetDevice(h->device));
        HIPCHK(hipMemcpy(host.data(), h->blob, h->blob_bytes, hipMemcpyDeviceToHost));
    } else {
        return fail(USE_E_STATE, "no weights to save (use_set_weight every tensor, or commit / load first)");
    }
    BlobHeader hd = make_header(h);
    hd.crc32 = crc32_of((const unsigned char*)host.data(), host.size());
    FILE* f = fopen(path, "wb");
    if (!f) return fail(USE_E_INVALID, "cannot open '%s' for writing", path);
    const bool ok = fwrite(&hd, sizeof hd, 1, f) == 1 && fwrite(host.data(), 1, host.size(), f) == host.size();
    if (fclose(f) != 0 || !ok) return fail(USE_E_INVALID, "short write to '%s'", path);
    return USE_OK;
}

int use_load_weight_blob(use_handle* h, const char* path) {
    if (!h || !path) return fail(USE_E_INVALID, "null argument");
    FILE* f = fopen(path, "rb");
    if (!f) return fail(USE_E_INVALID, "cannot open '%s'", path);
    BlobHeader hd{}, want = make_header(h);
    std::vector<char> host(h->blob_bytes);
    if (fread(&hd, sizeof hd, 1, f) != 1) { fclose(f); return fail(USE_E_INVALID, "'%s' is truncated", path); }
    if (memcmp(hd.magic, want.magic, 8) != 0 || hd.header_bytes != sizeof hd) { fclose(f); return fail(USE_E_INVALID, "'%s' is not a use_hip weight file", path); }
    if (hd.layout != want.layout) { fclose(f); return fail(USE_E_INVALID, "'%s' has blob layout %u, this build reads %u: re-pack the checkpoint", path, hd.layout, want.layout); }
    {
        BlobHeader a = hd; a.crc32 = 0;
        if (memcmp(&a, &want, sizeof a) != 0) { fclose(f); return fail(USE_E_INVALID, "'%s' was packed for a different network configuration / precision", path); }
    }
    const bool ok = fread(host.data(), 1, host.size(), f) == host.size();
    fclose(f);
    if (!ok) return fail(USE_E_INVALID, "'%s' is truncated", path);
    if (crc32_of((const unsigned char*)host.data(), host.size()) != hd.crc32) return fail(USE_E_INVALID, "'%s': checksum mismatch", path);
    HIPCHK(hipSetDevice(h->device));
    if (!h->blob) HIPCHK(hipMalloc((void**)&h->blob, h->blob_bytes));
    HIPCHK(hipMemcpy(h->blob, host.data(), h->blob_bytes, hipMemcpyHostToDevice));
    h->host_w.clear();
    h->weights_ready = true;
    h->sampler_set = false;
    drop_graphs(h); plan_cache_clear(h);
    return USE_OK;
}

int use_weight_blob(use_handle* h, void** dev_ptr, size_t* bytes) {
    if (!h) return fail(USE_E_INVALID, "null handle");
    if (dev_ptr) *dev_ptr = h->blob;
    if (bytes) *bytes = h->blob_bytes;
    return USE_OK;
}

int use_plan(use_handle* h, int B, int Tpad) {
    if (!h) return fail(USE_E_INVALID, "null handle");
    if (B < 1 || Tpad < 64 || Tpad % 64 != 0) return fail(USE_E_INVALID, "plan needs B >= 1 and T' a positive multiple of 64 (got B=%d T'=%d)", B, Tpad);
    if ((Tpad >> (h->cfg.n_levels - 1)) < 1) return fail(USE_E_INVALID, "T' too small for %d levels", h->cfg.n_levels);
    HIPCHK(hipSetDevice(h->device));
    if (h->arena.base && h->B == B && h->T == Tpad && h->opt_gen_at_plan == g_opt_gen) return USE_OK;
    HIPCHK(hipDeviceSynchronize());
    if (h->ode_graph) { (void)hipGraphExecDestroy(h->ode_graph); h->ode_graph = nullptr; }
    use_handle::PlanState* hit = nullptr;
    for (size_t i = 0; i < h->plan_cache.size(); ++i) {
        use_handle::PlanState* p = h->plan_cache[i];
        if (p->B == B && p->T == Tpad && p->opt_gen_at_plan == g_opt_gen) { hit = p; h->plan_cache.erase(h->plan_cache.begin() + (long)i); break; }
    }
    if (h->arena.base) {
        auto* p = new use_handle::PlanState();
        plan_stash(h, *p);
        if (g_plan_cache > 0 && p->opt_gen_at_plan == g_opt_gen) h->plan_cache.push_back(p); else plan_free(p);
        while ((int)h->plan_cache.size() > g_plan_cache) { plan_free(h->plan_cache.front()); h->plan_cache.erase(h->plan_cache.begin()); }
    }
    if (hit) {
        plan_restore(h, *hit);
        delete hit;
        ++h->n_plan_cache_hits;
        return USE_OK;
    }
    ++h->n_plans_built;
    h->opt_gen_at_plan = g_opt_gen;
    h->B = B; h->T = Tpad; h->sampler_set = false; h->ode_set = false;
    const int want = g_subbatch >= 0 ? g_subbatch : (B >= 6 && B <= 11) ? 3 : 2;
    h->nsub = std::max(1, std::min(std::min(want, MAX_SUB), B / std::max(1, g_subbatch_min_items)));
    for (int i = 0; i < MAX_SUB; ++i) h->sub_B[i] = i < h->nsub ? B / h->nsub + (i < B % h->nsub ? 1 : 0) : 0;
    char* old_base = h->arena.base;
    h->arena = Arena{};
    h->dry = true;
    size_t caps[MAX_SUB] = {}, stcaps[MAX_SUB] = {}, total = 0;
    for (int i = 0; i < h->nsub; ++i) {
        Arena& ar = i ? h->sub_arena[i] : h->arena;
        ar = Arena{}; h->st_arena[i] = Arena{};
        Fwd f{h, nullptr, nullptr, 0, nullptr, 0};
        f.B = h->sub_B[i]; f.arena = &ar; f.st_arena = &h->st_arena[i]; f.primary = i == 0;
        f.run(nullptr);
        caps[i] = (ar.peak + 4096 + 255) & ~(size_t)255; total += caps[i];
        stcaps[i] = (h->st_arena[i].peak + 255) & ~(size_t)255; total += stcaps[i];
    }
    h->dry = false;
    char* base = old_base;
    if (!base || total > h->arena_alloc) {
        if (base) { HIPCHK(hipFree(base)); base = nullptr; h->arena_alloc = 0; }
        if (hipMalloc((void**)&base, total) != hipSuccess) {
            (void)hipGetLastError();
            plan_cache_clear(h);
            if (hipMalloc((void**)&base, total) != hipSuccess)
                return fail(USE_E_NOMEM, "cannot allocate %.1f MB of activation workspace", total / 1e6);
        }
        h->arena_alloc = total;
    }
    h->arena.base = base; h->arena.cap = caps[0];
    h->arena_plan_bytes = total;
    {
        size_t off = caps[0];
        for (int i = 1; i < h->nsub; ++i) { h->sub_arena[i].base = base + off; h->sub_arena[i].cap = caps[i]; off += caps[i]; }
        for (int i = 0; i < h->nsub; ++i) { h->st_arena[i].base = base + off; h->st_arena[i].cap = stcaps[i]; off += stcaps[i]; }
        h->arena.dry_on_overflow = &h->dry;
        for (int i = 0; i < h->nsub; ++i) { h->sub_arena[i].dry_on_overflow = &h->dry; h->st_arena[i].dry_on_overflow = &h->dry; }
    }
    if (h->nsub > 1 && !h->ev_fork) HIPCHK(hipEventCreateWithFlags(&h->ev_fork, hipEventDisableTiming));
    for (int i = 0; i < h->nsub; ++i) {
        if (i && !h->aux_stream[i]) HIPCHK(hipStreamCreateWithFlags(&h->aux_stream[i], hipStreamNonBlocking));
        if (h->nsub > 1 && !h->ev_stagger[i]) {
            HIPCHK(hipEventCreateWithFlags(&h->ev_stagger[i], hipEventDisableTiming));
            HIPCHK(hipEventCreateWithFlags(&h->ev_join[i], hipEventDisableTiming));
        }
    }
    const size_t n = (size_t)B * h->cfg.n_freq * Tpad;
    h->lang_blocks = (int)std::min<size_t>(256, ((size_t)h->cfg.n_freq * Tpad + 255) / 256);
    size_t off = 0;
    auto take = [&](size_t bytes) { off = (off + 255) & ~(size_t)255; size_t o = off; off += bytes; return o; };
    const size_t o_x4 = take(n * 4 * h->pcp), o_c2 = take(h->pcp == 8 ? n * 8 : 0), o_Y = take(n * 8), o_X = take(n * 8), o_Xm = take(n * 8), o_sc = take(n * 8),
                 o_xin = take(n * 8), o_cond = take(n * 8), o_st = take((size_t)B * 4 * h->cfg.nf * 4), o_tb = take((size_t)B * h->dense_rows * 4),
                 o_t = take((size_t)B * 4), o_lp = take((size_t)B * h->lang_blocks * 2 * 4), o_ls = take(256), o_rng = take(256),
                 o_is = take((size_t)B * 8), o_ist = take((size_t)B * 4);
    h->persist_bytes = off;
    if (!h->persist || off > h->persist_alloc) {
        if (h->persist) { HIPCHK(hipFree(h->persist)); h->persist = nullptr; h->persist_alloc = 0; }
        if (hipMalloc((void**)&h->persist, off) != hipSuccess) {
            (void)hipGetLastError();
            plan_cache_clear(h);
            if (hipMalloc((void**)&h->persist, off) != hipSuccess) return fail(USE_E_NOMEM, "cannot allocate %.1f MB of state", off / 1e6);
        }
        h->persist_alloc = off;
    }
    h->x4 = (float*)(h->persist + o_x4); h->Y = (float2*)(h->persist + o_Y); h->X = (float2*)(h->persist + o_X);
    h->Xmean = (float2*)(h->persist + o_Xm); h->score = (float2*)(h->persist + o_sc); h->xin = (float2*)(h->persist + o_xin);
    h->cond_buf = (float2*)(h->persist + o_cond); h->Cond = h->Y;
    h->cond2_buf = h->pcp == 8 ? (float2*)(h->persist + o_c2) : nullptr;
    h->silu_temb = (float*)(h->persist + o_st); h->tembias = (float*)(h->persist + o_tb); h->t_dev = (float*)(h->persist + o_t);
    h->lang_partial = (float*)(h->persist + o_lp); h->lang_step = (float*)(h->persist + o_ls);
    h->rng_state = (unsigned long long*)(h->persist + o_rng);
    h->item_seeds = (unsigned long long*)(h->persist + o_is); h->item_step = (float*)(h->persist + o_ist);
    HIPCHK(hipMemset(h->persist, 0, off));
    return USE_OK;
}

int use_workspace_bytes(use_handle* h, size_t* bytes) {
    if (!h || !bytes) return fail(USE_E_INVALID, "null argument");
    *bytes = h->arena_plan_bytes + h->persist_bytes + h->blob_bytes;
    return USE_OK;
}

double use_flops_per_score(use_handle* h) { return h ? h->flops : 0.0; }

static int check_ready(use_handle* h) {
    if (!h) return fail(USE_E_INVALID, "null handle");
    if (!h->weights_ready) return fail(USE_E_STATE, "weights not committed (use_commit_weights / use_alloc_weight_blob)");
    if (!h->B) return fail(USE_E_STATE, "use_plan has not been called");
    if (h->opt_gen_at_plan != g_opt_gen)
        return fail(USE_E_STATE, "use_set_option was called after use_plan: the plan is stale, call use_plan (and use_set_sampler) again");
    return USE_OK;
}

static int eval_status(use_handle* h) {
    bool bad = h->arena.overflow;
    for (int i = 0; i < MAX_SUB; ++i) bad = bad || h->sub_arena[i].overflow || h->st_arena[i].overflow;
    if (!bad) return USE_OK;
    h->arena.overflow = false; h->dry = false;
    for (int i = 0; i < MAX_SUB; ++i) h->sub_arena[i].overflow = h->st_arena[i].overflow = false;
    return fail(USE_E_STATE, "activation workspace too small for this evaluation (an option that sizes plan buffers changed after use_plan?): call use_plan again; the output is invalid");
}

static int eval_net(use_handle* h, const void* x, const void* y, const float* t, void* out, use_stream_t stream, float sign,
                    const void* y2 = nullptr) {
    int rc = check_ready(h); if (rc) return rc;
    const use_config& c = h->cfg;
    const bool two_ch = c.input_channels == 2;
    if (!x || !out) return fail(USE_E_INVALID, "null tensor");
    if ((c.input_channels == 6) != (y2 != nullptr))
        return fail(USE_E_INVALID, c.input_channels == 6 ? "a 6-channel network takes two conditioning tensors (use_score2)" : "this network takes one conditioning tensor");
    if (two_ch ? y != nullptr : y == nullptr) return fail(USE_E_INVALID, two_ch ? "a 2-channel network takes x alone (y must be null)" : "null tensor");
    if (!t && (!c.unconditional || !c.no_sigma_scale)) return fail(USE_E_INVALID, "this network needs the time t");
    hipStream_t s = (hipStream_t)stream;
    if (!c.unconditional) run_temb(h, t, h->B, h->silu_temb, h->tembias, s);
    run_score(h, (const float2*)x, (const float2*)y, c.unconditional ? nullptr : h->tembias, h->dense_rows, t, 1, (float2*)out, s, sign,
              (const float2*)y2);
    HIPCHK(hipGetLastError());
    return eval_status(h);
}
int use_score2(use_handle* h, const void* x, const void* y, const void* y2, const float* t, void* out, use_stream_t stream) {
    return eval_net(h, x, y, t, out, stream, -1.f, y2);
}
int use_score(use_handle* h, const void* x, const void* y, const float* t, void* out, use_stream_t stream) {
    return eval_net(h, x, y, t, out, stream, -1.f);
}
int use_forward(use_handle* h, const void* x, const void* y, const float* t, void* out, use_stream_t stream) {
    return eval_net(h, x, y, t, out, stream, +1.f);
}

int use_profile_score(use_handle* h, const void* x, const void* y, const float* t, void* out, use_stream_t stream,
                      double* conv_ms, double* conv_flops, double* conv_bytes, int* conv_launches, double* total_ms) {
    int rc = check_ready(h); if (rc) return rc;
    hipStream_t s = (hipStream_t)stream;
    hipEvent_t t0, t1; HIPCHK(hipEventCreate(&t0)); HIPCHK(hipEventCreate(&t1));
    h->profile = true; h->prof_events.clear(); h->prof_flops.clear(); h->prof_bytes.clear(); h->prof_desc.clear(); h->prof_main.clear();
    for (auto& a : h->prof_aux) { if (a.e0) (void)hipEventDestroy(a.e0); if (a.e1) (void)hipEventDestroy(a.e1); }
    h->prof_aux.clear();
    const bool verbose = getenv("USE_HIP_PROFILE_VERBOSE") != nullptr;
    h->profile_all = verbose;
    HIPCHK(hipEventRecord(t0, s));
    rc = use_score(h, x, y, t, out, stream);
    h->profile = false;
    if (rc) return rc;
    HIPCHK(hipEventRecord(t1, s));
    HIPCHK(hipStreamSynchronize(s));
    double ms = 0.0, fl = 0.0, by = 0.0; int nmain = 0;
    for (size_t i = 0; i < h->prof_events.size(); ++i) {
        float e = 0.f; HIPCHK(hipEventElapsedTime(&e, h->prof_events[i].first, h->prof_events[i].second));
        if (h->prof_main[i]) {
            ms += e; fl += h->prof_flops[i]; by += h->prof_bytes[i]; ++nmain;
            use_handle::AuxProf r; r.name = "conv_v4"; r.H = h->prof_hw[i].first; r.W = h->prof_hw[i].second; r.bytes = h->prof_bytes[i]; r.ms = e; r.flops = h->prof_flops[i];
            h->prof_aux.push_back(r);
        }
        if (verbose) fprintf(stderr, "[use_profile] %s  %8.3f ms  %7.1f TFLOP/s\n", h->prof_desc[i].c_str(), e, h->prof_flops[i] / e / 1e9);
        (void)hipEventDestroy(h->prof_events[i].first); (void)hipEventDestroy(h->prof_events[i].second);
    }
    for (auto& a : h->prof_aux) {
        if (!a.e0) continue;
        float e = 0.f; HIPCHK(hipEventElapsedTime(&e, a.e0, a.e1));
        a.ms = e; (void)hipEventDestroy(a.e0); (void)hipEventDestroy(a.e1); a.e0 = a.e1 = nullptr;
    }
    float tot = 0.f; HIPCHK(hipEventElapsedTime(&tot, t0, t1));
    (void)hipEventDestroy(t0); (void)hipEventDestroy(t1);
    if (conv_ms) *conv_ms = ms;
    if (conv_flops) *conv_flops = fl;
    if (conv_bytes) *conv_bytes = by;
    if (conv_launches) *conv_launches = nmain;
    if (total_ms) *total_ms = tot;
    h->profile_all = false;
    h->prof_events.clear(); h->prof_flops.clear(); h->prof_bytes.clear(); h->prof_main.clear(); h->prof_hw.clear();
    return USE_OK;
}

int use_profile_aux(use_handle* h, int index, char* name, int name_cap, int* H, int* W, double* bytes, double* ms) {
    if (!h) return fail(USE_E_INVALID, "null handle");
    if (index < 0 || index >= (int)h->prof_aux.size()) return 1;
    const auto& a = h->prof_aux[(size_t)index];
    if (name && name_cap > 0) { strncpy(name, a.name.c_str(), (size_t)name_cap - 1); name[name_cap - 1] = 0; }
    if (H) *H = a.H; if (W) *W = a.W; if (bytes) *bytes = a.bytes; if (ms) *ms = a.ms;
    return USE_OK;
}

int use_profile_aux_flops(use_handle* h, int index, double* flops) {
    if (!h) return fail(USE_E_INVALID, "null handle");
    if (index < 0 || index >= (int)h->prof_aux.size()) return 1;
    if (flops) *flops = h->prof_aux[(size_t)index].flops;
    return USE_OK;
}

int use_timesteps(int N, float t_eps, float* out) {
    if (N < 1 || !out) return fail(USE_E_INVALID, "bad arguments");
    std::vector<float> ts; linspace_f32(1.0f, t_eps, N, ts);
    memcpy(out, ts.data(), (size_t)N * 4);
    return USE_OK;
}

int use_set_sampler(use_handle* h, const use_sampler_config* sc) {
    int rc = check_ready(h); if (rc) return rc;
    if (!sc || sc->N < 1) return fail(USE_E_INVALID, "sampler needs N >= 1");
    if (h->cfg.unconditional || h->cfg.input_channels == 2 || h->cfg.no_sigma_scale)
        return fail(USE_E_STATE, "the reverse-SDE sampler needs the conditional 4-channel score network");
    if (sc->predictor < 0 || sc->predictor > 2 || sc->corrector < 0 || sc->corrector > 2) return fail(USE_E_INVALID, "unknown predictor/corrector id");
    if (sc->corrector != USE_CORR_NONE && sc->corrector_steps < 0) return fail(USE_E_INVALID, "negative corrector_steps");
    HIPCHK(hipSetDevice(h->device));
    if (h->sampler_set && !memcmp(&h->sc, sc, sizeof *sc)) return USE_OK;
    HIPCHK(hipDeviceSynchronize());
    drop_graphs(h);
    h->sc = *sc;
    linspace_f32(1.0f, sc->t_eps, sc->N, h->timesteps);
    if (h->temb_table) { HIPCHK(hipFree(h->temb_table)); h->temb_table = nullptr; }
    if (h->silu_table) { HIPCHK(hipFree(h->silu_table)); h->silu_table = nullptr; }
    if (h->ts_dev) { HIPCHK(hipFree(h->ts_dev)); h->ts_dev = nullptr; }
    HIPCHK(hipMalloc((void**)&h->temb_table, (size_t)sc->N * h->dense_rows * 4));
    HIPCHK(hipMalloc((void**)&h->silu_table, (size_t)sc->N * 4 * h->cfg.nf * 4));
    HIPCHK(hipMalloc((void**)&h->ts_dev, (size_t)sc->N * 4));
    HIPCHK(hipMemcpy(h->ts_dev, h->timesteps.data(), (size_t)sc->N * 4, hipMemcpyHostToDevice));
    run_temb(h, h->ts_dev, sc->N, h->silu_table, h->temb_table, nullptr);
    HIPCHK(hipDeviceSynchronize());
    h->sampler_set = true;
    return USE_OK;
}

int use_num_noise_draws(use_handle* h) {
    if (!h || !h->sampler_set) return fail(USE_E_STATE, "sampler not configured");
    const int ncorr = h->sc.corrector == USE_CORR_NONE ? 0 : h->sc.corrector_steps;
    return 1 + h->sc.N * (ncorr + (h->sc.predictor == USE_PRED_NONE ? 0 : 1));
}

int use_get_timesteps(use_handle* h, float* out, int n) {
    if (!h || !h->sampler_set || !out) return fail(USE_E_STATE, "sampler not configured");
    for (int i = 0; i < n && i < (int)h->timesteps.size(); ++i) out[i] = h->timesteps[i];
    return (int)h->timesteps.size();
}

int use_sample(use_handle* h, const void* y, const void* noise, uint64_t seed, void* out, use_stream_t stream) {
    return use_sample_cond(h, y, nullptr, noise, seed, out, stream);
}

int use_sample_cond(use_handle* h, const void* y, const void* cond, const void* noise, uint64_t seed, void* out, use_stream_t stream) {
    return use_sample_cond2(h, y, cond, nullptr, noise, seed, out, stream);
}

static int load_sampler_inputs(use_handle* h, const void* y, const void* cond, const void* cond2, hipStream_t s) {
    const size_t n = (size_t)h->B * h->cfg.n_freq * h->T;
    HIPCHK(hipMemcpyAsync(h->Y, y, n * 8, hipMemcpyDeviceToDevice, s));
    if (cond2) HIPCHK(hipMemcpyAsync(h->cond2_buf, cond2, n * 8, hipMemcpyDeviceToDevice, s));
    float2* want = cond ? h->cond_buf : h->Y;
    if (want != h->Cond) { HIPCHK(hipStreamSynchronize(s)); drop_graphs(h); h->Cond = want; }
    if (cond) HIPCHK(hipMemcpyAsync(h->cond_buf, cond, n * 8, hipMemcpyDeviceToDevice, s));
    return USE_OK;
}

}

struct SeedPack { unsigned long long v[32]; };
__global__ void set_item_seeds_kernel(unsigned long long* dst, SeedPack p, int n) { if ((int)threadIdx.x < n) dst[threadIdx.x] = p.v[threadIdx.x]; }
static void upload_item_seeds(unsigned long long* dst, const uint64_t* seeds_host, int B, hipStream_t s) {
    for (int b0 = 0; b0 < B; b0 += 32) {
        SeedPack p{};
        const int k = std::min(32, B - b0);
        for (int i = 0; i < k; ++i) p.v[i] = (unsigned long long)seeds_host[b0 + i];
        hipLaunchKernelGGL(set_item_seeds_kernel, dim3(1), dim3(32), 0, s, dst + b0, p, k);
    }
}

static int sample_impl(use_handle* h, const void* y, const void* cond, const void* cond2, const void* noise, uint64_t seed,
                       const uint64_t* seeds_host, bool per_item, void* out, use_stream_t stream) {
    int rc = check_ready(h); if (rc) return rc;
    if (!h->sampler_set) return fail(USE_E_STATE, "use_set_sampler has not been called");
    if (!y || !out) return fail(USE_E_INVALID, "null tensor");
    if ((h->cfg.input_channels == 6) != (cond2 != nullptr))
        return fail(USE_E_INVALID, h->cfg.input_channels == 6 ? "a 6-channel network samples with two conditioning tensors (use_sample_cond2)"
                                                              : "this network takes one conditioning tensor");
    hipStream_t s = (hipStream_t)stream;
    const size_t n = (size_t)h->B * h->cfg.n_freq * h->T;
    rc = load_sampler_inputs(h, y, cond, cond2, s); if (rc) return rc;
    if (per_item) { if (seeds_host) upload_item_seeds(h->item_seeds, seeds_host, h->B, s); }
    else hipLaunchKernelGGL(set_rng_kernel, dim3(1), dim3(1), 0, s, h->rng_state, (unsigned long long)seed, 0ull);
    if (!h->sc.use_graph) {
        run_sampler(h, (const float2*)noise, s, 0, h->sc.N, per_item);
        rc = eval_status(h); if (rc) return rc;
    } else {
        const int gi = (noise ? 1 : 0) + (per_item ? 2 : 0);
        const float2* nz = nullptr;
        if (noise) {
            const size_t nb = (size_t)use_num_noise_draws(h) * n * 8;
            if (nb > h->noise_copy_bytes) {
                HIPCHK(hipStreamSynchronize(s));
                if (h->noise_copy) HIPCHK(hipFree(h->noise_copy));
                h->noise_copy = nullptr; h->noise_copy_bytes = 0;
                for (int k = 1; k < 4; k += 2) {
                    for (auto g : h->graph_exec[k]) if (g) (void)hipGraphExecDestroy(g);
                    h->graph_exec[k].clear();
                }
                if (hipMalloc((void**)&h->noise_copy, nb) != hipSuccess) return fail(USE_E_NOMEM, "cannot allocate %.1f MB noise staging", nb / 1e6);
                h->noise_copy_bytes = nb;
            }
            HIPCHK(hipMemcpyAsync(h->noise_copy, noise, nb, hipMemcpyDeviceToDevice, s));
            nz = h->noise_copy;
        }
        if (h->graph_exec[gi].empty()) {
            rc = ensure_cap_stream(h); if (rc) return rc;
            const int ncorr = h->sc.corrector == USE_CORR_NONE ? 0 : h->sc.corrector_steps;
            const int per_seg = std::max(1, 64 / (ncorr + 1));
            for (int i0 = 0; i0 < h->sc.N; i0 += per_seg) {
                hipGraph_t g = nullptr;
                hipGraphExec_t ge = nullptr;
                HIPCHK(hipStreamBeginCapture(h->cap_stream, hipStreamCaptureModeThreadLocal));
                run_sampler(h, nz, h->cap_stream, i0, std::min(h->sc.N, i0 + per_seg), per_item);
                hipError_t e = hipStreamEndCapture(h->cap_stream, &g);
                if (eval_status(h)) { if (g) (void)hipGraphDestroy(g); (void)hipGetLastError(); drop_graphs(h); return USE_E_STATE; }
                if (e != hipSuccess || !g) {
                    if (g) (void)hipGraphDestroy(g);
                    (void)hipGetLastError();
                    drop_graphs(h);
                    return fail(USE_E_HIP, "capturing the sampling loop failed: %s", hipGetErrorString(e));
                }
                e = hipGraphInstantiate(&ge, g, nullptr, nullptr, 0);
                (void)hipGraphDestroy(g);
                if (e != hipSuccess) { drop_graphs(h); return fail(USE_E_HIP, "hipGraphInstantiate: %s", hipGetErrorString(e)); }
                h->graph_exec[gi].push_back(ge);
                ++h->n_graph_captures;
            }
        }
        for (auto ge : h->graph_exec[gi]) HIPCHK(hipGraphLaunch(ge, s));
    }
    HIPCHK(hipMemcpyAsync(out, h->Xmean, n * 8, hipMemcpyDeviceToDevice, s));
    HIPCHK(hipGetLastError());
    return USE_OK;
}

extern "C" {

int use_sample_cond2(use_handle* h, const void* y, const void* cond, const void* cond2, const void* noise, uint64_t seed, void* out,
                     use_stream_t stream) {
    return sample_impl(h, y, cond, cond2, noise, seed, nullptr, false, out, stream);
}

int use_sample_items(use_handle* h, const void* y, const void* cond, const void* cond2, const void* noise, const uint64_t* seeds_host,
                     void* out, use_stream_t stream) {
    if (!noise && !seeds_host) return fail(USE_E_INVALID, "use_sample_items needs per-item seeds or injected noise");
    return sample_impl(h, y, cond, cond2, noise, 0, seeds_host, true, out, stream);
}

}

struct use_ode {
    use_handle* h = nullptr;
    use_ode_config cfg{};
    OdeDev d{};
    OdeCtl c{};
    char* buf = nullptr;
    float2* ysde_buf = nullptr;
    int* done_host = nullptr;
    int phase = -1;
};

namespace {
double float_as_decimal(float f) {
    char b[48];
    for (int p = 6; p <= 9; ++p) {
        snprintf(b, sizeof b, "%.*g", p, (double)f);
        if (strtof(b, nullptr) == f) break;
    }
    return strtod(b, nullptr);
}

int ode_check_config(const use_ode_config* oc) {
    if (!oc) return fail(USE_E_INVALID, "null ODE configuration");
    if (!(oc->rtol > 0.f) || !(oc->atol >= 0.f)) return fail(USE_E_INVALID, "ODE sampler needs rtol > 0 and atol >= 0 (got %g, %g)", oc->rtol, oc->atol);
    if (!(oc->t_eps > 0.f && oc->t_eps < 1.f)) return fail(USE_E_INVALID, "ODE sampler needs 0 < t_eps < T = 1 (got %g)", oc->t_eps);
    if (oc->group < 0) return fail(USE_E_INVALID, "ODE group must be >= 0 (0 = the whole batch), got %d", oc->group);
    if (oc->denoise && oc->N < 1) return fail(USE_E_INVALID, "the denoise step needs N >= 1");
    if (!(oc->first_step >= 0.f) || !(oc->max_step >= 0.f) || oc->max_nfe < 0) return fail(USE_E_INVALID, "first_step, max_step and max_nfe must be >= 0");
    if (oc->first_step > 0.f && float_as_decimal(oc->first_step) > 1.0 - float_as_decimal(oc->t_eps))
        return fail(USE_E_INVALID, "first_step exceeds the integration interval");
    return USE_OK;
}

void ode_supply_impl(use_ode* o, const float2* f, int kind, hipStream_t s) {
    launch_ode_stage(o->d, o->phase, f, kind, s);
    switch (o->phase) {
        case 0:
            launch_ode_ctrl(o->c, o->d, ODE_INIT1, s);
            if (o->c.first_step > 0) { launch_ode_commit(o->d, 0.2, s); o->phase = 1; }
            else { launch_ode_commit(o->d, 1.0, s); o->phase = 7; }
            break;
        case 7:
            launch_ode_ctrl(o->c, o->d, ODE_INIT2, s);
            launch_ode_commit(o->d, 0.2, s);
            o->phase = 1;
            break;
        case 6:
            launch_ode_ctrl(o->c, o->d, ODE_STEP, s);
            launch_ode_commit(o->d, 0.2, s);
            o->phase = 1;
            break;
        default: ++o->phase;
    }
}

void ode_start_impl(use_ode* o, hipStream_t s) {
    launch_ode_load(o->d, s);
    launch_ode_ctrl(o->c, o->d, ODE_START, s);
    o->phase = 0;
}

int ode_all_done(use_ode* o, hipStream_t s, bool* done) {
    HIPCHK(hipMemcpyAsync(o->done_host, o->d.done, sizeof(int), hipMemcpyDeviceToHost, s));
    HIPCHK(hipStreamSynchronize(s));
    *done = *o->done_host != 0;
    return USE_OK;
}

int ode_read_groups(use_ode* o, std::vector<OdeGroup>& g, hipStream_t s) {
    g.resize((size_t)o->c.ngroups);
    HIPCHK(hipMemcpyAsync(g.data(), o->d.grp, g.size() * sizeof(OdeGroup), hipMemcpyDeviceToHost, s));
    HIPCHK(hipStreamSynchronize(s));
    return USE_OK;
}
}

extern "C" {

int use_ode_create(use_handle* h, int B, int64_t n_per_item, const use_ode_config* cfg, use_ode** out) {
    if (!h || !out) return fail(USE_E_INVALID, "null argument");
    *out = nullptr;
    int rc = ode_check_config(cfg); if (rc) return rc;
    if (B < 1 || n_per_item < 1) return fail(USE_E_INVALID, "ODE stepper needs B >= 1 and n_per_item >= 1");
// ... 234 lines not shown
    return rc ? rc : n;
}
static int chunk_args(const void* a, const void* b, int B, int F, int Tp, int C, int overlap, int* n) {
    if (!a || !b) return fail(USE_E_INVALID, "null tensor");
    if (B < 1 || F < 1) return fail(USE_E_INVALID, "B=%d and F=%d must be positive", B, F);
    const int rc = chunk_geometry(Tp, C, overlap, n); if (rc) return rc;
    if ((long long)B * *n * F > (1ll << 30)) return fail(USE_E_INVALID, "B * n * F = %lld rows exceed 2^30", (long long)B * *n * F);
    return USE_OK;
}
int use_chunk_split(const void* Y, void* chunks, int B, int F, int Tp, int C, int overlap, use_stream_t s) {
    int n = 0;
    const int rc = chunk_args(Y, chunks, B, F, Tp, C, overlap, &n); if (rc) return rc;
    launch_chunk_split((const float2*)Y, (float2*)chunks, B, F, n, Tp, C, overlap, (hipStream_t)s);
    HIPCHK(hipGetLastError());
    return USE_OK;
}
int use_chunk_merge(const void* chunks, void* X, int B, int F, int Tp, int C, int overlap, use_stream_t s) {
    int n = 0;
    const int rc = chunk_args(chunks, X, B, F, Tp, C, overlap, &n); if (rc) return rc;
    launch_chunk_merge((const float2*)chunks, (float2*)X, B, F, n, Tp, C, overlap, (hipStream_t)s);
    HIPCHK(hipGetLastError());
    return USE_OK;
}

size_t use_metrics_workspace(int B, int stride) {
    if (B < 1 || B > 65535 || stride < 1) return 0;
    return metrics_layout(B, stride).bytes;
}
int use_metrics(const float* est, const float* clean, const float* noise, const int* len_host, int B, int stride, void* work,
                size_t work_bytes, double* out_dev, use_stream_t s) {
    if (B < 1 || B > 65535) return fail(USE_E_INVALID, "B=%d must lie in 1 ... 65535", B);
    if (stride < 1) return fail(USE_E_INVALID, "stride=%d must be positive", stride);
    if (!est) return fail(USE_E_INVALID, "est is null");
    if (!clean) return fail(USE_E_INVALID, "clean is null");
    if (!len_host) return fail(USE_E_INVALID, "len_host is null");
    if (!work) return fail(USE_E_INVALID, "work is null");
    if (!out_dev) return fail(USE_E_INVALID, "out_dev is null");
    for (int b = 0; b < B; ++b)
        if (len_host[b] < 256 || len_host[b] > stride)
            return fail(USE_E_INVALID, "len[%d]=%d must lie in 256 ... stride = %d (reflect padding of the 510-point STFT needs more than 255 samples)",
                        b, len_host[b], stride);
    const size_t need = metrics_layout(B, stride).bytes;
    if (work_bytes < need) return fail(USE_E_INVALID, "work_bytes=%zu is smaller than use_metrics_workspace(%d, %d) = %zu", work_bytes, B, stride, need);
    if ((uintptr_t)work & 7) return fail(USE_E_INVALID, "work must be 8-byte aligned");
    launch_metrics(est, clean, noise, len_host, B, stride, work, out_dev, (hipStream_t)s);
    HIPCHK(hipGetLastError());
    return USE_OK;
}

namespace {
std::mutex g_tw_mutex;
std::map<std::pair<int, int>, float2*> g_tw_tables;
int twiddles(int n_fft, hipStream_t s, const float2** out) {
    int dev = 0;
    HIPCHK(hipGetDevice(&dev));
    std::lock_guard<std::mutex> lock(g_tw_mutex);
    auto it = g_tw_tables.find({dev, n_fft});
    if (it == g_tw_tables.end()) {
        float2* tw = nullptr;
        HIPCHK(hipMalloc((void**)&tw, (size_t)n_fft * sizeof(float2)));
        launch_twiddle_table(tw, n_fft, s);
        HIPCHK(hipStreamSynchronize(s));
        it = g_tw_tables.emplace(std::make_pair(dev, n_fft), tw).first;
    }
    *out = it->second;
    return USE_OK;
}
int check_stft_args(int B, int L, int n_fft, int hop, int Tpad) {
    if (B < 1 || L < 1 || n_fft < 4 || (n_fft & 1) || hop < 1 || hop > n_fft) return fail(USE_E_INVALID, "bad STFT arguments (n_fft must be even, 1 <= hop <= n_fft)");
    if (L <= n_fft / 2) return fail(USE_E_INVALID, "signal of %d samples is too short for reflect padding with n_fft=%d", L, n_fft);
    if (Tpad < 1 + L / hop) return fail(USE_E_INVALID, "Tpad=%d is smaller than the %d frames of the signal", Tpad, 1 + L / hop);
    if ((size_t)n_fft * 8 + (size_t)((n_fft + hop - 1) / hop) * (n_fft / 2 + 1) * 8 > 64 * 1024) return fail(USE_E_INVALID, "n_fft / hop combination exceeds the synthesis kernel's LDS");
    return USE_OK;
}
}

int use_stft_fwd(const float* wav, void* Y, int B, int L, int n_fft, int hop, const float* window, int Tpad, float factor,
                 float exponent, use_stream_t s) {
    if (!wav || !Y || !window) return fail(USE_E_INVALID, "null argument");
    int rc = check_stft_args(B, L, n_fft, hop, Tpad); if (rc) return rc;
    const float2* tw = nullptr;
    rc = twiddles(n_fft, (hipStream_t)s, &tw); if (rc) return rc;
    launch_stft_fwd(wav, window, tw, (float2*)Y, B, L, n_fft, hop, 1 + L / hop, Tpad, factor, exponent, (hipStream_t)s);
    HIPCHK(hipGetLastError());
    return USE_OK;
}
int use_istft_back(const void* X, float* wav, int B, int L, int n_fft, int hop, const float* window, int Tpad, float factor,
                   float exponent, use_stream_t s) {
    if (!wav || !X || !window || factor == 0.f || exponent == 0.f) return fail(USE_E_INVALID, "bad arguments");
    int rc = check_stft_args(B, L, n_fft, hop, Tpad); if (rc) return rc;
    const float2* tw = nullptr;
    rc = twiddles(n_fft, (hipStream_t)s, &tw); if (rc) return rc;
    launch_istft_back((const float2*)X, window, tw, wav, B, L, n_fft, hop, Tpad, factor, exponent, (hipStream_t)s);
    HIPCHK(hipGetLastError());
    return USE_OK;
}

int use_sde_prior(use_handle* h, const void* y, const void* noise, uint64_t seed, void* x, int64_t n, use_stream_t s) {
    int rc = ensure_sde_scratch(h); if (rc) return rc;
    hipLaunchKernelGGL(set_rng_kernel, dim3(1), dim3(1), 0, (hipStream_t)s, h->sde_rng, (unsigned long long)seed, 0ull);
    launch_prior((const float2*)y, (const float2*)noise, RngRef{h->sde_rng, 0}, ouve_std(h->cfg, 1.0f), (float2*)x, n, (hipStream_t)s);
    HIPCHK(hipGetLastError());
    return USE_OK;
}

int use_fill_noise_items(use_handle* h, const uint64_t* seeds_host, int B, int draw, void* out, int64_t n, use_stream_t s) {
    if (!seeds_host || !out || B < 1 || draw < 0 || n < 0 || n % B != 0) return fail(USE_E_INVALID, "use_fill_noise_items: null argument, or n is no multiple of B");
    if (B > use_handle::SDE_MAX_B) return fail(USE_E_INVALID, "B=%d exceeds %d", B, use_handle::SDE_MAX_B);
    int rc = ensure_sde_scratch(h); if (rc) return rc;
    if (n == 0) return USE_OK;
    upload_item_seeds(h->sde_seeds, seeds_host, B, (hipStream_t)s);
    launch_fill_noise_items((float2*)out, ItemRng{h->sde_seeds, (unsigned)draw}, B, (long)(n / B), (hipStream_t)s);
    HIPCHK(hipGetLastError());
    return USE_OK;
}

int use_fill_noise(use_handle* h, uint64_t seed, int draw, void* out, int64_t n, use_stream_t s) {
    int rc = ensure_sde_scratch(h); if (rc) return rc;
    if (!out || n < 1 || draw < 0) return fail(USE_E_INVALID, "bad arguments");
    hipLaunchKernelGGL(set_rng_kernel, dim3(1), dim3(1), 0, (hipStream_t)s, h->sde_rng, (unsigned long long)seed, 0ull);
    launch_fill_noise((float2*)out, RngRef{h->sde_rng, (unsigned)draw}, (long)n, (hipStream_t)s);
    HIPCHK(hipGetLastError());
    return USE_OK;
}

int use_sde_predictor(use_handle* h, int predictor, float t, int N, const void* x, const void* y, const void* score,
                      const void* noise, uint64_t seed, void* x_out, void* x_mean, int64_t n, use_stream_t s) {
    int rc = ensure_sde_scratch(h); if (rc) return rc;
    if (predictor != USE_PRED_REVERSE_DIFFUSION && predictor != USE_PRED_EULER_MARUYAMA) return fail(USE_E_INVALID, "predictor id %d has no update kernel", predictor);
    float cd, cs, cn; predictor_coeffs(h->cfg, predictor, t, N, cd, cs, cn);
    hipLaunchKernelGGL(set_rng_kernel, dim3(1), dim3(1), 0, (hipStream_t)s, h->sde_rng, (unsigned long long)seed, 0ull);
    launch_predictor((const float2*)x, (const float2*)y, (const float2*)score, (const float2*)noise, RngRef{h->sde_rng, 0},
                     cd, cs, cn, (float2*)x_out, (float2*)x_mean, n, (hipStream_t)s);
    HIPCHK(hipGetLastError());
    return USE_OK;
}

int use_sde_corrector(use_handle* h, int corrector, float t, float snr, int B, const void* x, const void* score,
                      const void* noise, uint64_t seed, void* x_out, void* x_mean, int64_t n, use_stream_t st) {
    int rc = ensure_sde_scratch(h); if (rc) return rc;
    hipStream_t s = (hipStream_t)st;
    if (B < 1 || n % B != 0) return fail(USE_E_INVALID, "n must be a multiple of B");
    hipLaunchKernelGGL(set_rng_kernel, dim3(1), dim3(1), 0, s, h->sde_rng, (unsigned long long)seed, 0ull);
    RngRef rr{h->sde_rng, 0};
    if (corrector == USE_CORR_LANGEVIN) {
        if (B > use_handle::SDE_MAX_B) return fail(USE_E_INVALID, "B=%d exceeds %d", B, use_handle::SDE_MAX_B);
        launch_langevin_norms((const float2*)score, (const float2*)noise, rr, h->sde_partial, B, n / B, use_handle::SDE_BLOCKS, s);
        launch_langevin_step(h->sde_partial, B, use_handle::SDE_BLOCKS, snr, h->sde_step, s);
        launch_corrector((const float2*)x, (const float2*)score, (const float2*)noise, rr, h->sde_step, 0.f, (float2*)x_out, (float2*)x_mean, n, s);
    } else if (corrector == USE_CORR_ALD) {
        const float sd = snr * ouve_std(h->cfg, t);
        launch_corrector((const float2*)x, (const float2*)score, (const float2*)noise, rr, nullptr, sd * sd * 2.f, (float2*)x_out, (float2*)x_mean, n, s);
    } else return fail(USE_E_INVALID, "corrector id %d has no update kernel", corrector);
    HIPCHK(hipGetLastError());
    return USE_OK;
}

namespace {
__global__ void fill_uniform_kernel(void* p, size_t n, int dtype, unsigned seed, float lo, float hi) {
    const size_t i = (size_t)blockIdx.x * blockDim.x + threadIdx.x;
    if (i >= n) return;
    unsigned long long z = (unsigned long long)i * 0x9E3779B97F4A7C15ull + ((unsigned long long)seed << 32 | 0x1234567u);
    z = (z ^ (z >> 30)) * 0xBF58476D1CE4E5B9ull; z = (z ^ (z >> 27)) * 0x94D049BB133111EBull; z ^= z >> 31;
    const float v = lo + (hi - lo) * (float)((z >> 40) * (1.0 / 16777216.0));
    if (dtype == DT_F32) ((float*)p)[i] = v;
    else if (dtype == DT_BF16) ((__bf16*)p)[i] = (__bf16)v;
    else ((_Float16*)p)[i] = (_Float16)v;
}
__global__ void to_float_kernel(const void* p, float* out, size_t n, int dtype) {
    const size_t i = (size_t)blockIdx.x * blockDim.x + threadIdx.x;
    if (i >= n) return;
    out[i] = dtype == DT_F32 ? ((const float*)p)[i] : dtype == DT_BF16 ? (float)((const __bf16*)p)[i] : (float)((const _Float16*)p)[i];
}
}

static int op_temb_bstride(const use_conv_op* c) { return c->temb_bstride == 0 ? c->Cout : c->temb_bstride < 0 ? 0 : c->temb_bstride; }

int use_conv_bench(const use_conv_case* c, float* out_host, float* stats_host, double* ms_avg, double* flops) {
    if (!c || c->B < 1 || c->H < 1 || c->W < 1 || c->C0 < 1 || c->Cout < 1) return fail(USE_E_INVALID, "bad conv case");
    const int dt = c->dtype;
    if (dt != DT_F32 && dt != DT_BF16 && dt != DT_F16) return fail(USE_E_INVALID, "bad dtype");
    const size_t es = dtype_size(dt);
    const int Cin = c->C0 + c->C1, XC = c->XC0 + c->XC1;
    const size_t px = (size_t)c->B * c->H * c->W;
    std::vector<void*> bufs;
    auto dalloc = [&](size_t bytes) -> void* { void* q = nullptr; if (hipMalloc(&q, bytes) != hipSuccess) return nullptr; bufs.push_back(q); return q; };
    auto cleanup = [&]() { for (void* q : bufs) (void)hipFree(q); };
    auto fill = [&](void* q, size_t n, int dtype, unsigned seed, float lo, float hi) {
        hipLaunchKernelGGL(fill_uniform_kernel, dim3((unsigned)((n + 255) / 256)), dim3(256), 0, 0, q, n, dtype, seed, lo, hi);
    };
    ConvW w; w.cin = Cin; w.cout = c->Cout; w.ntaps = 9; w.w_dtype = dt; w.cin_src = Cin; w.cout_src = c->Cout;
    w.cout_pad = c->Cout <= 32 ? 32 : (c->Cout + 127) / 128 * 128;
    ConvW w2 = w; w2.cin = XC; w2.cin_src = XC; w2.ntaps = 1;
    ConvArgs a{};
    a.B = c->B; a.H = c->H; a.W = c->W; a.Cout = c->Cout; a.ntaps = 9; a.in_dtype = dt; a.out_dtype = dt;
    a.C0 = c->C0; a.C1 = c->C1; a.XC0 = c->XC0; a.XC1 = c->XC1; a.act = c->act; a.out_scale = c->res || XC ? 0.70710678f : 1.f;
    a.cout_pad = w.cout_pad;
    void* src0 = dalloc(px * c->C0 * es); void* src1 = c->C1 ? dalloc(px * c->C1 * es) : nullptr;
    void* x0 = c->XC0 ? dalloc(px * c->XC0 * es) : nullptr; void* x1 = c->XC1 ? dalloc(px * c->XC1 * es) : nullptr;
    void* res = c->res ? dalloc(px * c->Cout * es) : nullptr;
    void* out = dalloc(px * c->Cout * es);
    float* outf = (float*)dalloc(px * c->Cout * 4);
    float* coef = c->gn ? (float*)dalloc((size_t)c->B * Cin * 2 * 4) : nullptr;
    float* bias = (float*)dalloc((size_t)c->Cout * 4); float* temb = (float*)dalloc((size_t)c->B * c->Cout * 4);
    const size_t wbytes = (size_t)9 * w.cout_pad * Cin * es, w2bytes = (size_t)w2.cout_pad * std::max(XC, 1) * es;
    char* dw = (char*)dalloc(wbytes); char* dwb = (char*)dalloc(wbytes);
    char* dw2 = XC ? (char*)dalloc(w2bytes) : nullptr; char* dw2b = XC ? (char*)dalloc(w2bytes) : nullptr;
    const size_t stats_bytes = (size_t)c->B * c->Cout * 2 * sizeof(long long);
    long long* stats = c->stats ? (long long*)dalloc(stats_bytes) : nullptr;
    if (!src0 || !out || !outf || !dw || !dwb || (c->stats && !stats)) { cleanup(); return fail(USE_E_NOMEM, "conv bench allocation failed"); }
    fill(src0, px * c->C0, dt, 1, -2.f, 2.f); if (src1) fill(src1, px * c->C1, dt, 2, -2.f, 2.f);
    if (x0) fill(x0, px * c->XC0, dt, 3, -1.f, 1.f); if (x1) fill(x1, px * c->XC1, dt, 4, -1.f, 1.f);
    if (res) fill(res, px * c->Cout, dt, 5, -1.f, 1.f);
    if (coef) fill(coef, (size_t)c->B * Cin * 2, DT_F32, 6, -0.9f, 1.1f);
    fill(bias, c->Cout, DT_F32, 7, -0.5f, 0.5f); fill(temb, (size_t)c->B * c->Cout, DT_F32, 8, -0.5f, 0.5f);
    {
        std::vector<float> hw((size_t)c->Cout * Cin * 9), hw2((size_t)c->Cout * std::max(XC, 1));
        unsigned long long st = 88172645463325252ull;
        auto rnd = [&]() { st ^= st << 13; st ^= st >> 7; st ^= st << 17; return (float)((st >> 40) * (1.0 / 16777216.0)) * 2.f - 1.f; };
        const float sc = 1.0f / std::sqrt((float)Cin * 9.f / 3.f);
        for (auto& v : hw) v = rnd() * sc;
        for (auto& v : hw2) v = rnd() * (1.0f / std::sqrt((float)std::max(XC, 1) / 3.f));
        std::vector<char> hp(wbytes), hpb(wbytes);
        const bool slab = w.cout_pad % 128 == 0 && Cin % conv_v4_chunk(dt) == 0;
        pack_conv_raw(hw.data(), w, hp.data(), slab ? hpb.data() : nullptr);
        (void)hipMemcpy(dw, hp.data(), wbytes, hipMemcpyHostToDevice);
        if (slab) (void)hipMemcpy(dwb, hpb.data(), wbytes, hipMemcpyHostToDevice);
        a.w = dw; a.wb = slab ? dwb : nullptr;
        if (XC) {
            std::vector<char> hq(w2bytes), hqb(w2bytes);
            const bool slab2 = XC % conv_v4_chunk(dt) == 0 && w2.cout_pad % 128 == 0;
            pack_conv_raw(hw2.data(), w2, hq.data(), slab2 ? hqb.data() : nullptr);
            (void)hipMemcpy(dw2, hq.data(), w2bytes, hipMemcpyHostToDevice);
            if (slab2) (void)hipMemcpy(dw2b, hqb.data(), w2bytes, hipMemcpyHostToDevice);
            a.w2 = dw2; a.w2b = slab2 ? dw2b : nullptr;
        }
    }
    a.src0 = src0; a.src1 = src1; a.x0 = x0; a.x1 = x1; a.coef = coef; a.bias = bias; a.temb = c->temb ? temb : nullptr;
    a.temb_bstride = c->Cout; a.res = res; a.out = out; a.stats = stats;
    auto run = [&]() -> int {
        switch (c->variant) {
            case 0: launch_conv(a, 0); return 0;
            case 1: launch_conv_generic(a, 0); return 0;
            case 7: if (!conv_sk_eligible(a)) return -1; launch_conv_sk(a, 0); return 0;
            case 2: if (!conv_v2_eligible(a)) return -1; launch_conv_v2(a, 0); return 0;
            case 4: if (conv_v4_unrunnable(a)) return -1; launch_conv_v4(a, 0); return 0;
            case 5: if (conv_v5_unrunnable(a)) return -1; launch_conv_v5(a, 0); return 0;
            default: return -1;
        }
    };
    if (getenv("USE_HIP_DBG")) a.dbg = atoi(getenv("USE_HIP_DBG"));
    unsigned long long* trace = nullptr;
    if (getenv("USE_HIP_TRACE")) {
        trace = (unsigned long long*)dalloc(512 * 8);
        if (trace) { (void)hipMemset(trace, 0, 512 * 8); a.trace = trace; a.dbg = atoi(getenv("USE_HIP_TRACE")); }
    }
    if (stats) (void)hipMemset(stats, 0, stats_bytes);
    if (run() != 0) {
        const char* why = c->variant == 4 ? conv_v4_unrunnable(a) : c->variant == 5 ? conv_v5_unrunnable(a) : nullptr;
        cleanup(); return fail(USE_E_INVALID, "variant %d cannot run this case%s%s", c->variant, why ? ": needs " : "", why ? why : "");
    }
    if (hipDeviceSynchronize() != hipSuccess) { cleanup(); return fail(USE_E_HIP, "conv bench: launch failed: %s", hipGetErrorString(hipGetLastError())); }
    if (trace) {
        unsigned long long hb[512];
        (void)hipMemcpy(hb, trace, sizeof hb, hipMemcpyDeviceToHost);
        for (int g = 0; g < 2; ++g) {
            unsigned long long prev = hb[g * 256 + 1];
            for (int i = 0; i < 125 && hb[g * 256 + 2 * i]; ++i) {
                fprintf(stderr, "[trace G%d] id %3llu  +%6llu  @%8llu\n", g, hb[g * 256 + 2 * i], hb[g * 256 + 2 * i + 1] - prev, hb[g * 256 + 2 * i + 1] - hb[1]);
                prev = hb[g * 256 + 2 * i + 1];
            }
        }
        a.trace = nullptr;
    }
    hipEvent_t e0, e1; (void)hipEventCreate(&e0); (void)hipEventCreate(&e1);
    const int iters = std::max(1, c->iters);
    (void)hipEventRecord(e0, 0);
    for (int i = 0; i < iters; ++i) run();
    (void)hipEventRecord(e1, 0);
    (void)hipEventSynchronize(e1);
    float ms = 0.f; (void)hipEventElapsedTime(&ms, e0, e1);
    (void)hipEventDestroy(e0); (void)hipEventDestroy(e1);
    if (ms_avg) *ms_avg = ms / iters;
    if (flops) *flops = 2.0 * (double)px * c->Cout * ((double)Cin * 9 + XC);
    int rc = USE_OK;
    if (out_host) {
        hipLaunchKernelGGL(to_float_kernel, dim3((unsigned)((px * c->Cout + 255) / 256)), dim3(256), 0, 0, out, outf, px * c->Cout, dt);
        if (hipMemcpy(out_host, outf, px * c->Cout * 4, hipMemcpyDeviceToHost) != hipSuccess) rc = fail(USE_E_HIP, "copy back failed");
    }
    if (stats_host && stats) {
        (void)hipMemset(stats, 0, stats_bytes);
        run();
        std::vector<long long> hs((size_t)c->B * c->Cout * 2);
        if (hipMemcpy(hs.data(), stats, stats_bytes, hipMemcpyDeviceToHost) != hipSuccess) rc = fail(USE_E_HIP, "copy back failed");
        for (size_t i = 0; i < hs.size(); i += 2) {
            stats_host[i] = (float)((double)hs[i] / 1048576.0); stats_host[i + 1] = (float)((double)hs[i + 1] / 1048576.0);
        }
    }
    cleanup();
    return rc;
}

int use_op_conv(const use_conv_op* c, use_stream_t stream) {
    if (!c || c->B < 1 || c->H < 1 || c->W < 1 || c->C0 < 1 || c->Cout < 1 || !c->src0 || !c->w || !c->out) return fail(USE_E_INVALID, "use_op_conv: bad argument");
    const int dt = c->dtype, odt = c->out_dtype;
    if ((dt != DT_F32 && dt != DT_BF16 && dt != DT_F16) || (odt != DT_F32 && odt != DT_BF16 && odt != DT_F16)) return fail(USE_E_INVALID, "use_op_conv: bad dtype");
// ... 291 lines not shown
```

### universal_speech_enhancement_amd/csrc/use_kernels.h

```cpp
#pragma once
#include <hip/hip_runtime.h>
#include <stdint.h>
#include <atomic>
#include <thread>

namespace use {

constexpr int USE_MAX_DEVICES = 64;
struct LdsAttrOnce {
    std::atomic<int> st[USE_MAX_DEVICES] = {};
    template <typename F> void once(F&& f) {
        int d = 0;
        if (hipGetDevice(&d) != hipSuccess || d < 0 || d >= USE_MAX_DEVICES) { f(); return; }
        if (st[d].load(std::memory_order_acquire) == 2) return;
        int expected = 0;
        if (st[d].compare_exchange_strong(expected, 1, std::memory_order_acq_rel)) { f(); st[d].store(2, std::memory_order_release); }
        else while (st[d].load(std::memory_order_acquire) != 2) std::this_thread::yield();
    }
    template <typename K> void operator()(K kern, int bytes) {
        once([&] { (void)hipFuncSetAttribute(reinterpret_cast<const void*>(kern), hipFuncAttributeMaxDynamicSharedMemorySize, bytes); });
    }
};


enum DType { DT_F32 = 0, DT_BF16 = 1, DT_F16 = 2 };
inline size_t dtype_size(int dt) { return dt == DT_F32 ? 4 : 2; }

constexpr int CONV_IN_SPLIT_K = 112;
constexpr int TILE_H = 8;
constexpr int TILE_W = 16;

inline int tiles_per_image(int H, int W) { return ((H + TILE_H - 1) / TILE_H) * ((W + TILE_W - 1) / TILE_W); }
extern int g_conv_in_wgs;
inline int conv_in_split_tpw(int H, int W) { const int nt = tiles_per_image(H, W); return (nt + g_conv_in_wgs - 1) / g_conv_in_wgs; }
inline int conv_in_split_wgs(int H, int W) { const int nt = tiles_per_image(H, W), tpw = conv_in_split_tpw(H, W); return (nt + tpw - 1) / tpw; }
inline int conv_v2_tiles(int H, int W) { return ((H + 15) / 16) * ((W + 15) / 16); }

struct ConvArgs {
    const void* src0; const void* src1; int C0; int C1; int in_dtype;
    const float* coef;
    const long long* gn_st0; const long long* gn_st1;
    const float* gn_gamma; const float* gn_beta; int gn_groups; float gn_inv_n; float gn_eps;
    int act;
    const void* w;
    const void* wb;
    int cout_pad;
    const void* x0; const void* x1; int XC0; int XC1; const void* w2;
    const void* w2b;
    const float* bias;
    const float* temb;
    int temb_bstride;
    const void* res;
    float out_scale;
    const float* pyr;
    const float* w4;
    const float* b4;
    void* out; int out_dtype;
    long long* stats_part;
    long long* stats;
    int B, H, W, Cout, ntaps;
    int dbg;
    unsigned long long* trace;
};
void launch_conv(const ConvArgs& a, hipStream_t s);
int conv_stats_parts(const ConvArgs& a);
bool conv_v2_eligible(const ConvArgs& a);
void launch_conv_v2(const ConvArgs& a, hipStream_t s);
inline int conv_v4_chunk(int dtype) { return dtype == DT_F32 ? 16 : 32; }
inline int conv_v4_tiles(int H, int W) { return ((H + 15) / 16) * ((W + 31) / 32); }
bool conv_sk_eligible(const ConvArgs& a);
void conv_sk_set_max_px(long n);
void launch_conv_sk(const ConvArgs& a, hipStream_t s);
void conv_sk_set_per_image(bool on);
void launch_conv_generic(const ConvArgs& a, hipStream_t s);
void pyr_conv_set_ws(int n);
bool conv_v4_eligible(const ConvArgs& a);
const char* conv_v4_unrunnable(const ConvArgs& a);
void conv_v4_set_min_blocks(long n);
void launch_conv_v4(const ConvArgs& a, hipStream_t s);
const char* conv_v5_unrunnable(const ConvArgs& a);
void conv_v5_set(int on);
bool conv_v5_enabled(const ConvArgs& a);
void launch_conv_v5(const ConvArgs& a, hipStream_t s);
void launch_gn_finalize(const long long* st0, int C0, const long long* st1, int C1, const float* gamma, const float* beta,
                        int groups, int hw, float eps, float* coef, int B, hipStream_t s, const long long* pt0 = nullptr, int nt0 = 0,
                        const long long* pt1 = nullptr, int nt1 = 0);

void launch_fir_up2(const void* src, int dtype, const float* coef, int act, void* out_act, void* out_raw, int B,
                    int H, int W, int C, hipStream_t s);
void fir_set_strip(int on);
void launch_fir_down2(const void* src, int dtype, const float* coef, int act, void* out_act, void* out_raw, int B,
                      int H, int W, int C, hipStream_t s);

void launch_spec_map(const float2* in, float2* out, long rows, int Tin, int Tin_stride, int Tout, float pre, float power,
                     float post, hipStream_t s);

void launch_chunk_split(const float2* Y, float2* chunks, int B, int F, int n, int Tp, int C, int overlap, hipStream_t s);
void launch_chunk_merge(const float2* chunks, float2* X, int B, int F, int n, int Tp, int C, int overlap, hipStream_t s);

constexpr int METRICS_SLICE = 2048;
struct MetricsWork { size_t part1, part2, alpha, lsd, bytes; int nblk, Tmax; };
MetricsWork metrics_layout(int B, int stride);
void launch_metrics(const float* est, const float* clean, const float* noise, const int* len_host, int B, int stride, void* work,
                    double* out, hipStream_t s);

void launch_twiddle_table(float2* tw, int N, hipStream_t s);
void launch_stft_fwd(const float* wav, const float* win, const float2* tw, float2* Y, int B, int L, int N, int hop, int T,
                     int Tpad, float factor, float expo, hipStream_t s);
void launch_istft_back(const float2* X, const float* win, const float2* tw, float* wav, int B, int L, int N, int hop, int Tpad,
                       float factor, float expo, hipStream_t s);

void launch_pack_input(const float2* x, const float2* y, const float2* y2, float* x4, long npix, hipStream_t s);
void launch_combine_add(void* h, int dtype, const float* pyr, const float* w8, const float* b8, long long* stats, int B, long pix_per_b,
                        int C, hipStream_t s);

void launch_temb_mlp(const float* t, int t_stride, const float* gfp_w, const float* w1, const float* b1,
                     const float* w2, const float* b2, float* out_silu, int B, int nf, hipStream_t s);
void launch_temb_dense(const float* silu_temb, const float* W, const float* bias, float* out, int B, int rows,
                       int dim, hipStream_t s);

void launch_attention(const void* q, const void* k, const void* v, void* out, int dtype, int B, int N, int C,
                      hipStream_t s);

struct AttnArgs {
    const void* x; void* out; int N;
    const long long* gn_st; const float* gn_gamma; const float* gn_beta; int gn_groups; float gn_eps;
    const void *wq, *wk, *wv, *wo; const float *bq, *bk, *bv, *bo;
    long long* stats;
};
bool attn_fused_eligible(int dtype, int N, int C);
void launch_attn_fused(const AttnArgs& a, int dtype, int B, hipStream_t s);

void launch_softmax_rows(void* x, int dtype, long rows, int cols, hipStream_t s);
void launch_transpose_nc(const void* in, void* out, int dtype, int B, int N, int C, hipStream_t s);

void launch_score_out(const float* pyr, int pc, const float* t, int t_stride, const float* w, const float* bias,
                      float2* score, int B, long pix_per_b, float sign, hipStream_t s);

size_t wgrad_workspace_floats(int B, int H, int W, int Cout, int Cin, int ntaps, int dtype);
void wgrad_set_mfma16(int v);
void wgrad_set_blocks(int n);
bool launch_wgrad(const void* dy, const void* x, int dtype, float* dw, float* db, int B, int H, int W, int Cout, int Cin, int ntaps, float alpha,
                  float* work, hipStream_t s);
bool launch_gn_stats(const void* x, int dtype, int B, int HW, int C, int G, float eps, float* mean, float* rstd, double* part, hipStream_t s);
constexpr int GN_MAX_SLICES = 256;
size_t gn_workspace_floats(int B, int C, int G);
bool launch_gn_act_bwd(const void* x, const void* dy, int dtype, const float* mean, const float* rstd, const float* gamma, const float* beta, int act,
                       const void* add, float add_scale, int B, int HW, int C, int G, float* s1, float* s2, float* m12, double* part, void* dx,
                       float* dgamma, float* dbeta, hipStream_t s);
bool launch_gn_act_fwd(const void* x, int dtype, const float* mean, const float* rstd, const float* gamma, const float* beta, int act, int B, int HW,
                       int C, int G, void* y, hipStream_t s);
bool launch_colsum(const void* x, int dtype, int B, int HW, int C, float scale, float* out, double* part, hipStream_t s);
void launch_attention_bwd(const float* q, const float* k, const float* v, const float* dO, float* work, float* dq, float* dk, float* dv, int B,
                          int N, int C, hipStream_t s);
void launch_dense_bwd(const float* g, const float* temb, const float* Wd, int B, int K, int Cout, float* dW, float* db, float* dtemb, hipStream_t s);
void launch_pack_conv_dev(const float* src, int mode, int cout, int cin, int ntaps, int cout_pad, int dtype, int ck, void* dst, void* dstb,
                          const float* bias, float* bias_out, hipStream_t s);

struct RngRef { const unsigned long long* state; unsigned draw; };
void launch_prior(const float2* y, const float2* noise, RngRef rng, float std1, float2* x, long n, hipStream_t s);
void launch_predictor(const float2* x, const float2* y, const float2* score, const float2* noise, RngRef rng,
                      float c_drift, float c_score, float c_noise, float2* x_out, float2* x_mean, long n,
                      hipStream_t s);
void launch_langevin_norms(const float2* score, const float2* noise, RngRef rng, float* partial, int B,
                           long n_per_b, int blocks_per_b, hipStream_t s);
void launch_langevin_step(const float* partial, int B, int blocks_per_b, float snr, float* step, hipStream_t s);
void launch_corrector(const float2* x, const float2* score, const float2* noise, RngRef rng, const float* step_dev,
                      float step_host, float2* x_out, float2* x_mean, long n, hipStream_t s);
void launch_fill_noise(float2* out, RngRef rng, long n, hipStream_t s);
struct ItemRng { const unsigned long long* seeds; unsigned draw; };
void launch_prior_items(const float2* y, const float2* noise, ItemRng rng, float std1, float2* x, int B, long n_per_b,
                        hipStream_t s);
void launch_predictor_items(const float2* x, const float2* y, const float2* score, const float2* noise, ItemRng rng,
                            float c_drift, float c_score, float c_noise, float2* x_out, float2* x_mean, int B,
                            long n_per_b, hipStream_t s);
void launch_langevin_norms_items(const float2* score, const float2* noise, ItemRng rng, float* partial, int B,
                                 long n_per_b, int blocks_per_b, hipStream_t s);
void launch_langevin_step_items(const float* partial, int B, int blocks_per_b, float snr, float* step, hipStream_t s);
void launch_corrector_items(const float2* x, const float2* score, const float2* noise, ItemRng rng,
                            const float* step_dev, float step_host, float2* x_out, float2* x_mean, int B, long n_per_b,
                            hipStream_t s);
void launch_fill_noise_items(float2* out, ItemRng rng, int B, long n_per_b, hipStream_t s);

struct OdeGroup {
    double t, h_abs;
    double ha, h, t_new, min_step, h0, d1;
    int status;
    int rejected, accepted, nfev, steps, nrej;
};
struct OdeDev {
    double2 *y, *ynew;
    float2* K;
    float2* xin;
    const float2* ysde;
    double* h_item;
    float *ts, *cg;
    double* part;
    OdeGroup* grp;
    int* done;
    long n_per_b;
    int B, G, nblk;
    float theta;
    double rtol, atol;
};
struct OdeCtl {
    double t0, t_bound, first_step, max_step;
    int max_nfe, ngroups, G, B, nblk;
    long n_per_b;
    float sigma_min, base, sq2ls;
};
enum { ODE_START = 0, ODE_INIT1 = 1, ODE_INIT2 = 2, ODE_STEP = 3 };
void launch_ode_load(const OdeDev& d, hipStream_t s);
void launch_ode_stage(const OdeDev& d, int row, const float2* f, int kind, hipStream_t s);
void launch_ode_commit(const OdeDev& d, double coef, hipStream_t s);
void launch_ode_ctrl(const OdeCtl& c, const OdeDev& d, int mode, hipStream_t s);
void launch_ode_result(const OdeDev& d, float2* out, hipStream_t s);

}
```

### universal_speech_enhancement_amd/csrc/use_kernels.hip

```cpp
#include "use_kernels.h"
#include <type_traits>
#include <cstdlib>
#include <cstdio>
#include "use_device.h"

#include <math.h>

namespace use {

#define LDS_BARRIER() asm volatile("s_waitcnt lgkmcnt(0)\n\ts_barrier" ::: "memory")


constexpr int BM = TILE_H * TILE_W;
constexpr int HALO_MAX = (TILE_H + 2) * (TILE_W + 2);

template <typename TIN, typename TOUT, int CK, int BN, int WM, int WN>
__global__ __launch_bounds__(256) void conv_kernel(ConvArgs p) {
    typedef Mfma<TIN> MF;
    constexpr int VEC = 16 / sizeof(TIN);
    constexpr int PARTS = CK / VEC;
    constexpr int ROWB = CK * (int)sizeof(TIN) + 16;
    constexpr int MW = BM / WM, NW = BN / WN;
    constexpr int TM = MW / 32, TN = NW / 32;
    constexpr int KSTEPS = CK / MF::KM;
// ... 1632 lines not shown
    const int i = blockIdx.x, b = blockIdx.y, tid = threadIdx.x;
    const T* qb = q + ((size_t)b * N + i) * C;
    for (int c = tid; c < C; c += 256) sq[c] = to_f(qb[c]);
    __syncthreads();
    const float scale = rsqrtf((float)C);
    float mx = -INFINITY;
    for (int j = tid; j < N; j += 256) {
        const T* kb = k + ((size_t)b * N + j) * C;
        float a = 0.f;
        for (int c = 0; c < C; ++c) a = fmaf(sq[c], to_f(kb[c]), a);
        a *= scale; sc[j] = a; mx = fmaxf(mx, a);
    }
    for (int o = 32; o > 0; o >>= 1) mx = fmaxf(mx, __shfl_xor(mx, o));
    if ((tid & 63) == 0) red[tid >> 6] = mx;
    __syncthreads();
    mx = fmaxf(fmaxf(red[0], red[1]), fmaxf(red[2], red[3]));
    __syncthreads();
    float sum = 0.f;
    for (int j = tid; j < N; j += 256) { const float e = expf(sc[j] - mx); sc[j] = e; sum += e; }
    for (int o = 32; o > 0; o >>= 1) sum += __shfl_xor(sum, o);
    if ((tid & 63) == 0) red[tid >> 6] = sum;
    __syncthreads();
    const float inv = 1.f / (red[0] + red[1] + red[2] + red[3]);
    for (int c = tid; c < C; c += 256) {
        float a = 0.f;
        for (int j = 0; j < N; ++j) a = fmaf(sc[j], to_f(v[((size_t)b * N + j) * C + c]), a);
        out[((size_t)b * N + i) * C + c] = from_f<T>(a * inv);
    }
}
void launch_attention(const void* q, const void* k, const void* v, void* out, int dtype, int B, int N, int C,
                      hipStream_t s) {
    const size_t sh = (size_t)(C + N) * sizeof(float);
    if (dtype == DT_F32)
        hipLaunchKernelGGL((attention_kernel<float>), dim3(N, B), dim3(256), sh, s, (const float*)q, (const float*)k,
                           (const float*)v, (float*)out, N, C);
    else if (dtype == DT_F16)
        hipLaunchKernelGGL((attention_kernel<_Float16>), dim3(N, B), dim3(256), sh, s, (const _Float16*)q,
                           (const _Float16*)k, (const _Float16*)v, (_Float16*)out, N, C);
    else
        hipLaunchKernelGGL((attention_kernel<__bf16>), dim3(N, B), dim3(256), sh, s, (const __bf16*)q,
                           (const __bf16*)k, (const __bf16*)v, (__bf16*)out, N, C);
}

template <typename T>
__global__ __launch_bounds__(256) void softmax_rows_kernel(T* __restrict__ x, int cols) {
    __shared__ float red[4];
    T* row = x + (size_t)blockIdx.x * cols;
    const int tid = threadIdx.x;
    float mx = -INFINITY;
    for (int j = tid; j < cols; j += 256) mx = fmaxf(mx, to_f(row[j]));
    for (int o = 32; o > 0; o >>= 1) mx = fmaxf(mx, __shfl_xor(mx, o));
    if ((tid & 63) == 0) red[tid >> 6] = mx;
    __syncthreads();
    mx = fmaxf(fmaxf(red[0], red[1]), fmaxf(red[2], red[3]));
    __syncthreads();
    float sum = 0.f;
    for (int j = tid; j < cols; j += 256) sum += expf(to_f(row[j]) - mx);
    for (int o = 32; o > 0; o >>= 1) sum += __shfl_xor(sum, o);
    if ((tid & 63) == 0) red[tid >> 6] = sum;
    __syncthreads();
    const float inv = 1.f / (red[0] + red[1] + red[2] + red[3]);
    for (int j = tid; j < cols; j += 256) row[j] = from_f<T>(expf(to_f(row[j]) - mx) * inv);
}
void launch_softmax_rows(void* x, int dtype, long rows, int cols, hipStream_t s) {
    if (dtype == DT_F32) hipLaunchKernelGGL((softmax_rows_kernel<float>), dim3((unsigned)rows), dim3(256), 0, s, (float*)x, cols);
    else if (dtype == DT_F16) hipLaunchKernelGGL((softmax_rows_kernel<_Float16>), dim3((unsigned)rows), dim3(256), 0, s, (_Float16*)x, cols);
    else                 hipLaunchKernelGGL((softmax_rows_kernel<__bf16>), dim3((unsigned)rows), dim3(256), 0, s, (__bf16*)x, cols);
}
template <typename T>
__global__ __launch_bounds__(256) void transpose_nc_kernel(const T* __restrict__ in, T* __restrict__ out, int N, int C) {
    __shared__ T tile[32][33];
    const int b = blockIdx.z, n0 = blockIdx.x * 32, c0 = blockIdx.y * 32;
    const int tx = threadIdx.x & 31, ty = threadIdx.x >> 5;
    for (int r = ty; r < 32; r += 8)
        if (n0 + r < N && c0 + tx < C) tile[r][tx] = in[((size_t)b * N + n0 + r) * C + c0 + tx];
    __syncthreads();
    for (int r = ty; r < 32; r += 8)
        if (c0 + r < C && n0 + tx < N) out[((size_t)b * C + c0 + r) * N + n0 + tx] = tile[tx][r];
}
void launch_transpose_nc(const void* in, void* out, int dtype, int B, int N, int C, hipStream_t s) {
    dim3 grid((N + 31) / 32, (C + 31) / 32, B);
    if (dtype == DT_F32) hipLaunchKernelGGL((transpose_nc_kernel<float>), grid, dim3(256), 0, s, (const float*)in, (float*)out, N, C);
    else if (dtype == DT_F16) hipLaunchKernelGGL((transpose_nc_kernel<_Float16>), grid, dim3(256), 0, s, (const _Float16*)in, (_Float16*)out, N, C);
    else                 hipLaunchKernelGGL((transpose_nc_kernel<__bf16>), grid, dim3(256), 0, s, (const __bf16*)in, (__bf16*)out, N, C);
}

template <int PC>
__global__ __launch_bounds__(256) void score_out_kernel(const float* __restrict__ pyr, const float* __restrict__ t,
                                                        int t_stride, const float* __restrict__ w,
                                                        const float* __restrict__ bias, float2* __restrict__ score,
                                                        long pix_per_b, float sign) {
    const int b = blockIdx.y;
    const float tv = t ? t[(size_t)b * t_stride] : 1.0f;
    float wr[PC], wi[PC];
#pragma unroll
    for (int k = 0; k < PC; ++k) { wr[k] = w[k]; wi[k] = w[PC + k]; }
    const float b0 = bias[0], b1 = bias[1];
    for (long i = (long)blockIdx.x * 256 + threadIdx.x; i < pix_per_b; i += (long)gridDim.x * 256) {
        float hv[PC];
#pragma unroll
        for (int k4 = 0; k4 < PC / 4; ++k4) {
            const float4 q = *reinterpret_cast<const float4*>(pyr + ((size_t)b * pix_per_b + i) * PC + k4 * 4);
            hv[k4 * 4] = q.x; hv[k4 * 4 + 1] = q.y; hv[k4 * 4 + 2] = q.z; hv[k4 * 4 + 3] = q.w;
        }
        float re = b0, im = b1;
#pragma unroll
        for (int k = 0; k < PC; ++k) {
            const float hk = t ? hv[k] / tv : hv[k];
            re += wr[k] * hk; im += wi[k] * hk;
        }
        score[(size_t)b * pix_per_b + i] = make_float2(sign * re, sign * im);
    }
}
void launch_score_out(const float* pyr, int pc, const float* t, int t_stride, const float* w, const float* bias,
                      float2* score, int B, long pix_per_b, float sign, hipStream_t s) {
    int bx = (int)((pix_per_b + 255) / 256); if (bx > 2048) bx = 2048;
    if (pc == 8) hipLaunchKernelGGL(score_out_kernel<8>, dim3(bx, B), dim3(256), 0, s, pyr, t, t_stride, w, bias, score, pix_per_b, sign);
    else         hipLaunchKernelGGL(score_out_kernel<4>, dim3(bx, B), dim3(256), 0, s, pyr, t, t_stride, w, bias, score, pix_per_b, sign);
}

DEVI void philox_round(unsigned (&c)[4], unsigned (&k)[2]) {
    const unsigned long long p0 = (unsigned long long)0xD2511F53u * c[0];
    const unsigned long long p1 = (unsigned long long)0xCD9E8D57u * c[2];
    const unsigned n0 = (unsigned)(p1 >> 32) ^ c[1] ^ k[0], n1 = (unsigned)p1;
    const unsigned n2 = (unsigned)(p0 >> 32) ^ c[3] ^ k[1], n3 = (unsigned)p0;
    c[0] = n0; c[1] = n1; c[2] = n2; c[3] = n3;
    k[0] += 0x9E3779B9u; k[1] += 0xBB67AE85u;
}
DEVI float2 philox_cnormal(unsigned long long seed, unsigned long long draw, unsigned long long idx) {
    unsigned c[4] = {(unsigned)idx, (unsigned)(idx >> 32), (unsigned)draw, (unsigned)(draw >> 32)};
    unsigned k[2] = {(unsigned)seed, (unsigned)(seed >> 32)};
#pragma unroll
    for (int r = 0; r < 10; ++r) philox_round(c, k);
    const float u1 = ((float)(c[0] >> 8) + 0.5f) * (1.0f / 16777216.0f);
    const float u2 = ((float)(c[1] >> 8) + 0.5f) * (1.0f / 16777216.0f);
    const float r = sqrtf(-logf(u1));
    float sn, cs;
    sincosf(6.283185307179586f * u2, &sn, &cs);
    return make_float2(r * cs, r * sn);
}
DEVI float2 get_noise(const float2* noise, RngRef rng, long i) {
    if (noise) return noise[i];
    return philox_cnormal(rng.state[0], rng.state[1] + rng.draw, (unsigned long long)i);
}

__global__ __launch_bounds__(256) void fill_noise_kernel(float2* out, RngRef rng, long n) {
    for (long i = (long)blockIdx.x * 256 + threadIdx.x; i < n; i += (long)gridDim.x * 256)
        out[i] = get_noise(nullptr, rng, i);
}
void launch_fill_noise(float2* out, RngRef rng, long n, hipStream_t s) {
    hipLaunchKernelGGL(fill_noise_kernel, dim3(ew_blocks(n)), dim3(256), 0, s, out, rng, n);
}

__global__ __launch_bounds__(256) void prior_kernel(const float2* __restrict__ y, const float2* __restrict__ noise,
                                                    RngRef rng, float std1, float2* __restrict__ x, long n) {
    for (long i = (long)blockIdx.x * 256 + threadIdx.x; i < n; i += (long)gridDim.x * 256) {
        const float2 z = get_noise(noise, rng, i), yy = y[i];
        x[i] = make_float2(yy.x + z.x * std1, yy.y + z.y * std1);
    }
}
void launch_prior(const float2* y, const float2* noise, RngRef rng, float std1, float2* x, long n, hipStream_t s) {
    hipLaunchKernelGGL(prior_kernel, dim3(ew_blocks(n)), dim3(256), 0, s, y, noise, rng, std1, x, n);
}

__global__ __launch_bounds__(256) void predictor_kernel(const float2* __restrict__ x, const float2* __restrict__ y,
                                                        const float2* __restrict__ score,
                                                        const float2* __restrict__ noise, RngRef rng, float c_drift,
                                                        float c_score, float c_noise, float2* __restrict__ x_out,
                                                        float2* __restrict__ x_mean, long n) {
    for (long i = (long)blockIdx.x * 256 + threadIdx.x; i < n; i += (long)gridDim.x * 256) {
        const float2 xv = x[i], yv = y[i], sv = score[i], z = get_noise(noise, rng, i);
        const float fx = c_drift * (yv.x - xv.x) - c_score * sv.x;
        const float fy = c_drift * (yv.y - xv.y) - c_score * sv.y;
        const float mx = xv.x - fx, my = xv.y - fy;
        if (x_mean) x_mean[i] = make_float2(mx, my);
        x_out[i] = make_float2(mx + c_noise * z.x, my + c_noise * z.y);
    }
}
void launch_predictor(const float2* x, const float2* y, const float2* score, const float2* noise, RngRef rng,
                      float c_drift, float c_score, float c_noise, float2* x_out, float2* x_mean, long n,
                      hipStream_t s) {
    hipLaunchKernelGGL(predictor_kernel, dim3(ew_blocks(n)), dim3(256), 0, s, x, y, score, noise, rng, c_drift,
                       c_score, c_noise, x_out, x_mean, n);
}

__global__ __launch_bounds__(256) void langevin_norms_kernel(const float2* __restrict__ score,
                                                             const float2* __restrict__ noise, RngRef rng,
                                                             float* __restrict__ partial, long n_per_b) {
    const int b = blockIdx.y;
    float g2 = 0.f, z2 = 0.f;
    for (long i = (long)blockIdx.x * 256 + threadIdx.x; i < n_per_b; i += (long)gridDim.x * 256) {
        const long gi = (long)b * n_per_b + i;
        const float2 g = score[gi], z = get_noise(noise, rng, gi);
        g2 += g.x * g.x + g.y * g.y; z2 += z.x * z.x + z.y * z.y;
    }
    __shared__ float rg[4], rz[4];
    for (int o = 32; o > 0; o >>= 1) { g2 += __shfl_xor(g2, o); z2 += __shfl_xor(z2, o); }
    if ((threadIdx.x & 63) == 0) { rg[threadIdx.x >> 6] = g2; rz[threadIdx.x >> 6] = z2; }
    __syncthreads();
    if (threadIdx.x == 0) {
        float* dst = partial + ((size_t)b * gridDim.x + blockIdx.x) * 2;
        dst[0] = rg[0] + rg[1] + rg[2] + rg[3]; dst[1] = rz[0] + rz[1] + rz[2] + rz[3];
    }
}
void launch_langevin_norms(const float2* score, const float2* noise, RngRef rng, float* partial, int B,
                           long n_per_b, int blocks_per_b, hipStream_t s) {
    hipLaunchKernelGGL(langevin_norms_kernel, dim3(blocks_per_b, B), dim3(256), 0, s, score, noise, rng, partial,
                       n_per_b);
}

__global__ __launch_bounds__(64) void langevin_step_kernel(const float* __restrict__ partial, int B, int blocks_per_b,
                                                           float snr, float* __restrict__ step) {
    double gn = 0.0, zn = 0.0;
    for (int b = 0; b < B; ++b) {
        double g2 = 0.0, z2 = 0.0;
        for (int k = threadIdx.x; k < blocks_per_b; k += 64) {
            g2 += (double)partial[((size_t)b * blocks_per_b + k) * 2];
            z2 += (double)partial[((size_t)b * blocks_per_b + k) * 2 + 1];
        }
        for (int o = 32; o > 0; o >>= 1) { g2 += __shfl_xor(g2, o); z2 += __shfl_xor(z2, o); }
        gn += sqrt(g2); zn += sqrt(z2);
    }
    if (threadIdx.x == 0) {
        const float gm = (float)(gn / B), zm = (float)(zn / B);
        const float r = snr * zm / gm;
        step[0] = r * r * 2.f;
    }
}
void launch_langevin_step(const float* partial, int B, int blocks_per_b, float snr, float* step, hipStream_t s) {
    hipLaunchKernelGGL(langevin_step_kernel, dim3(1), dim3(64), 0, s, partial, B, blocks_per_b, snr, step);
}

__global__ __launch_bounds__(256) void corrector_kernel(const float2* __restrict__ x, const float2* __restrict__ score,
                                                        const float2* __restrict__ noise, RngRef rng,
                                                        const float* __restrict__ step_dev, float step_host,
                                                        float2* __restrict__ x_out, float2* __restrict__ x_mean,
                                                        long n) {
    const float eps = step_dev ? step_dev[0] : step_host;
    const float sq = sqrtf(eps * 2.f);
    for (long i = (long)blockIdx.x * 256 + threadIdx.x; i < n; i += (long)gridDim.x * 256) {
        const float2 xv = x[i], g = score[i], z = get_noise(noise, rng, i);
        const float mx = xv.x + eps * g.x, my = xv.y + eps * g.y;
        if (x_mean) x_mean[i] = make_float2(mx, my);
        x_out[i] = make_float2(mx + z.x * sq, my + z.y * sq);
    }
}
void launch_corrector(const float2* x, const float2* score, const float2* noise, RngRef rng, const float* step_dev,
                      float step_host, float2* x_out, float2* x_mean, long n, hipStream_t s) {
    hipLaunchKernelGGL(corrector_kernel, dim3(ew_blocks(n)), dim3(256), 0, s, x, score, noise, rng, step_dev,
                       step_host, x_out, x_mean, n);
}

DEVI float2 get_noise_item(const float2* noise, ItemRng rng, int b, long n_per_b, long j) {
    if (noise) return noise[(long)b * n_per_b + j];
    return philox_cnormal(rng.seeds[b], rng.draw, (unsigned long long)j);
}
static int item_blocks(long n_per_b, int B) {
    long b = (n_per_b + 255) / 256, cap = 8192 / (B > 0 ? B : 1);
    if (cap < 1) cap = 1;
    if (b > cap) b = cap;
    if (b < 1) b = 1;
    return (int)b;
}

__global__ __launch_bounds__(256) void fill_noise_items_kernel(float2* out, ItemRng rng, long n_per_b) {
    const int b = blockIdx.y;
    for (long j = (long)blockIdx.x * 256 + threadIdx.x; j < n_per_b; j += (long)gridDim.x * 256)
        out[(long)b * n_per_b + j] = get_noise_item(nullptr, rng, b, n_per_b, j);
}
void launch_fill_noise_items(float2* out, ItemRng rng, int B, long n_per_b, hipStream_t s) {
    hipLaunchKernelGGL(fill_noise_items_kernel, dim3(item_blocks(n_per_b, B), B), dim3(256), 0, s, out, rng, n_per_b);
}

__global__ __launch_bounds__(256) void prior_items_kernel(const float2* __restrict__ y, const float2* __restrict__ noise,
                                                          ItemRng rng, float std1, float2* __restrict__ x, long n_per_b) {
    const int b = blockIdx.y;
    for (long j = (long)blockIdx.x * 256 + threadIdx.x; j < n_per_b; j += (long)gridDim.x * 256) {
        const long i = (long)b * n_per_b + j;
        const float2 z = get_noise_item(noise, rng, b, n_per_b, j), yy = y[i];
        x[i] = make_float2(yy.x + z.x * std1, yy.y + z.y * std1);
    }
}
void launch_prior_items(const float2* y, const float2* noise, ItemRng rng, float std1, float2* x, int B, long n_per_b,
                        hipStream_t s) {
    hipLaunchKernelGGL(prior_items_kernel, dim3(item_blocks(n_per_b, B), B), dim3(256), 0, s, y, noise, rng, std1, x,
                       n_per_b);
}

__global__ __launch_bounds__(256) void predictor_items_kernel(const float2* __restrict__ x, const float2* __restrict__ y,
                                                              const float2* __restrict__ score,
                                                              const float2* __restrict__ noise, ItemRng rng,
                                                              float c_drift, float c_score, float c_noise,
                                                              float2* __restrict__ x_out, float2* __restrict__ x_mean,
                                                              long n_per_b) {
    const int b = blockIdx.y;
    for (long j = (long)blockIdx.x * 256 + threadIdx.x; j < n_per_b; j += (long)gridDim.x * 256) {
        const long i = (long)b * n_per_b + j;
        const float2 xv = x[i], yv = y[i], sv = score[i], z = get_noise_item(noise, rng, b, n_per_b, j);
        const float fx = c_drift * (yv.x - xv.x) - c_score * sv.x;
        const float fy = c_drift * (yv.y - xv.y) - c_score * sv.y;
        const float mx = xv.x - fx, my = xv.y - fy;
        if (x_mean) x_mean[i] = make_float2(mx, my);
        x_out[i] = make_float2(mx + c_noise * z.x, my + c_noise * z.y);
    }
}
void launch_predictor_items(const float2* x, const float2* y, const float2* score, const float2* noise, ItemRng rng,
                            float c_drift, float c_score, float c_noise, float2* x_out, float2* x_mean, int B,
                            long n_per_b, hipStream_t s) {
    hipLaunchKernelGGL(predictor_items_kernel, dim3(item_blocks(n_per_b, B), B), dim3(256), 0, s, x, y, score, noise,
                       rng, c_drift, c_score, c_noise, x_out, x_mean, n_per_b);
}

__global__ __launch_bounds__(256) void langevin_norms_items_kernel(const float2* __restrict__ score,
                                                                   const float2* __restrict__ noise, ItemRng rng,
                                                                   float* __restrict__ partial, long n_per_b) {
    const int b = blockIdx.y;
    float g2 = 0.f, z2 = 0.f;
    for (long j = (long)blockIdx.x * 256 + threadIdx.x; j < n_per_b; j += (long)gridDim.x * 256) {
        const float2 g = score[(long)b * n_per_b + j], z = get_noise_item(noise, rng, b, n_per_b, j);
        g2 += g.x * g.x + g.y * g.y; z2 += z.x * z.x + z.y * z.y;
    }
    __shared__ float rg[4], rz[4];
    for (int o = 32; o > 0; o >>= 1) { g2 += __shfl_xor(g2, o); z2 += __shfl_xor(z2, o); }
    if ((threadIdx.x & 63) == 0) { rg[threadIdx.x >> 6] = g2; rz[threadIdx.x >> 6] = z2; }
    __syncthreads();
    if (threadIdx.x == 0) {
        float* dst = partial + ((size_t)b * gridDim.x + blockIdx.x) * 2;
        dst[0] = rg[0] + rg[1] + rg[2] + rg[3]; dst[1] = rz[0] + rz[1] + rz[2] + rz[3];
    }
}
void launch_langevin_norms_items(const float2* score, const float2* noise, ItemRng rng, float* partial, int B,
                                 long n_per_b, int blocks_per_b, hipStream_t s) {
    hipLaunchKernelGGL(langevin_norms_items_kernel, dim3(blocks_per_b, B), dim3(256), 0, s, score, noise, rng, partial,
                       n_per_b);
}

__global__ __launch_bounds__(64) void langevin_step_items_kernel(const float* __restrict__ partial, int blocks_per_b,
                                                                 float snr, float* __restrict__ step) {
    const int b = blockIdx.x;
    double g2 = 0.0, z2 = 0.0;
    for (int k = threadIdx.x; k < blocks_per_b; k += 64) {
        g2 += (double)partial[((size_t)b * blocks_per_b + k) * 2];
        z2 += (double)partial[((size_t)b * blocks_per_b + k) * 2 + 1];
    }
    for (int o = 32; o > 0; o >>= 1) { g2 += __shfl_xor(g2, o); z2 += __shfl_xor(z2, o); }
    if (threadIdx.x == 0) {
        const float gm = (float)sqrt(g2), zm = (float)sqrt(z2);
        const float r = snr * zm / gm;
        step[b] = r * r * 2.f;
    }
}
void launch_langevin_step_items(const float* partial, int B, int blocks_per_b, float snr, float* step, hipStream_t s) {
    hipLaunchKernelGGL(langevin_step_items_kernel, dim3(B), dim3(64), 0, s, partial, blocks_per_b, snr, step);
}

__global__ __launch_bounds__(256) void corrector_items_kernel(const float2* __restrict__ x,
                                                              const float2* __restrict__ score,
                                                              const float2* __restrict__ noise, ItemRng rng,
                                                              const float* __restrict__ step_dev, float step_host,
                                                              float2* __restrict__ x_out, float2* __restrict__ x_mean,
                                                              long n_per_b) {
    const int b = blockIdx.y;
    const float eps = step_dev ? step_dev[b] : step_host;
    const float sq = sqrtf(eps * 2.f);
    for (long j = (long)blockIdx.x * 256 + threadIdx.x; j < n_per_b; j += (long)gridDim.x * 256) {
        const long i = (long)b * n_per_b + j;
        const float2 xv = x[i], g = score[i], z = get_noise_item(noise, rng, b, n_per_b, j);
        const float mx = xv.x + eps * g.x, my = xv.y + eps * g.y;
        if (x_mean) x_mean[i] = make_float2(mx, my);
        x_out[i] = make_float2(mx + z.x * sq, my + z.y * sq);
    }
}
void launch_corrector_items(const float2* x, const float2* score, const float2* noise, ItemRng rng,
                            const float* step_dev, float step_host, float2* x_out, float2* x_mean, int B, long n_per_b,
                            hipStream_t s) {
    hipLaunchKernelGGL(corrector_items_kernel, dim3(item_blocks(n_per_b, B), B), dim3(256), 0, s, x, score, noise, rng,
                       step_dev, step_host, x_out, x_mean, n_per_b);
}

}
```

Baseline: 3647 spectrogram-frames/s.

## Run sampler sub-batches across streams with SDE updates fused into packed input

```diff
diff --git a/include/use_hip.h b/include/use_hip.h
--- a/include/use_hip.h
+++ b/include/use_hip.h
@@ -101,6 +101,19 @@
                       const void* noise, uint64_t seed, void* x_out, void* x_mean, int64_t n, use_stream_t s);
 int use_sde_corrector(use_handle* h, int corrector, float t, float snr, int B, const void* x, const void* score,
                       const void* noise, uint64_t seed, void* x_out, void* x_mean, int64_t n, use_stream_t s);
+
+int use_op_sde_prior(use_handle* h, const void* y, const void* noise, uint64_t seed, const uint64_t* item_seeds_host, void* x, float* x4,
+                     int pcp, int B, int64_t n_per_b, int b0, int nb, use_stream_t s);
+int use_op_sde_predictor(use_handle* h, int predictor, float t, int N, const void* x, const void* y, const void* score, const void* noise,
+                         uint64_t seed, const uint64_t* item_seeds_host, void* x_out, void* x_mean, float* x4, int pcp, int B,
+                         int64_t n_per_b, int b0, int nb, use_stream_t s);
+int use_op_sde_langevin_norms(use_handle* h, const void* score, const void* noise, uint64_t seed, const uint64_t* item_seeds_host,
+                              float* partial, int blocks_per_b, int B, int64_t n_per_b, int b0, int nb, use_stream_t s);
+int use_op_sde_langevin_step(const float* partial, int blocks_per_b, float snr, float* step, int per_item, int B, int b0, int nb,
+                             use_stream_t s);
+int use_op_sde_corrector(use_handle* h, const void* x, const void* score, const void* noise, uint64_t seed, const uint64_t* item_seeds_host,
+                         const float* step_dev, float step_host, void* x_out, void* x_mean, float* x4, int pcp, int B, int64_t n_per_b,
+                         int b0, int nb, use_stream_t s);
 
 int use_fill_noise(use_handle* h, uint64_t seed, int draw, void* out, int64_t n, use_stream_t s);
 
diff --git a/universal_speech_enhancement_amd/_lib.py b/universal_speech_enhancement_amd/_lib.py
--- a/universal_speech_enhancement_amd/_lib.py
+++ b/universal_speech_enhancement_amd/_lib.py
@@ -98,6 +98,11 @@
     "use_fill_noise_items": (_i, [_vp, C.POINTER(_u64), _i, _i, _vp, _i64, _vp]),
     "use_sde_predictor": (_i, [_vp, _i, _f, _i, _vp, _vp, _vp, _vp, _u64, _vp, _vp, _i64, _vp]),
     "use_sde_corrector": (_i, [_vp, _i, _f, _f, _i, _vp, _vp, _vp, _u64, _vp, _vp, _i64, _vp]),
+    "use_op_sde_prior": (_i, [_vp, _vp, _vp, _u64, C.POINTER(_u64), _vp, _vp, _i, _i, _i64, _i, _i, _vp]),
+    "use_op_sde_predictor": (_i, [_vp, _i, _f, _i, _vp, _vp, _vp, _vp, _u64, C.POINTER(_u64), _vp, _vp, _vp, _i, _i, _i64, _i, _i, _vp]),
+    "use_op_sde_langevin_norms": (_i, [_vp, _vp, _vp, _u64, C.POINTER(_u64), _vp, _i, _i, _i64, _i, _i, _vp]),
+    "use_op_sde_langevin_step": (_i, [_vp, _i, _f, _vp, _i, _i, _i, _i, _vp]),
+    "use_op_sde_corrector": (_i, [_vp, _vp, _vp, _vp, _u64, C.POINTER(_u64), _vp, _f, _vp, _vp, _vp, _i, _i, _i64, _i, _i, _vp]),
     "use_debug_tensor": (_i, [_vp, C.c_char_p, C.POINTER(_vp), C.POINTER(_i), C.POINTER(_i)]),
     "use_flops_per_score": (C.c_double, [_vp]),
     "use_get_stat": (_i, [_vp, C.c_char_p, C.POINTER(C.c_longlong)]),
diff --git a/universal_speech_enhancement_amd/csrc/use_engine.cpp b/universal_speech_enhancement_amd/csrc/use_engine.cpp
--- a/universal_speech_enhancement_amd/csrc/use_engine.cpp
+++ b/universal_speech_enhancement_amd/csrc/use_engine.cpp
@@ -142,6 +142,7 @@
     hipStream_t aux_stream[MAX_SUB] = {};
     hipEvent_t ev_fork = nullptr, ev_stagger[MAX_SUB] = {},
                ev_join[MAX_SUB] = {};
+    hipEvent_t ev_step = nullptr;
     int debug_B = 0;
     std::vector<hipGraphExec_t> graph_exec[4];
     hipGraphExec_t score_graph = nullptr;
@@ -408,6 +409,7 @@
 static int g_attn_fused = 1;
 static int g_stats_part = 1;
 static int g_stagger_level = 2;
+static int g_cross_eval = 1;
 
 __global__ __launch_bounds__(256) void zero16_kernel(uint4* __restrict__ p, size_t n16) {
     for (size_t i = (size_t)blockIdx.x * 256 + threadIdx.x; i < n16; i += (size_t)gridDim.x * 256) p[i] = make_uint4(0, 0, 0, 0);
@@ -749,7 +751,95 @@
 __global__ void set_rng_kernel(unsigned long long* st, unsigned long long seed, unsigned long long base) { st[0] = seed; st[1] = base; }
 __global__ void fill_f32_kernel(float* p, float v, int n) { for (int i = threadIdx.x; i < n; i += blockDim.x) p[i] = v; }
 
+static bool cross_eval_on(const use_handle* h) { return g_cross_eval && h->nsub > 1 && !h->profile; }
+
+static void run_sampler_cross(use_handle* h, const float2* noise, hipStream_t s, int i0, int i1, bool per_item) {
+    const use_sampler_config& sc = h->sc;
+    const long n_per_b = (long)h->cfg.n_freq * h->T, n = (long)h->B * n_per_b;
+    const int ncorr = sc.corrector == USE_CORR_NONE ? 0 : sc.corrector_steps, nsub = h->nsub, pcp = h->pcp;
+    struct PerImage { bool on; PerImage(bool o) : on(o) { if (on) conv_sk_set_per_image(true); } ~PerImage() { if (on) conv_sk_set_per_image(false); } } per_image(per_item);
+    auto nz = [&](unsigned d) { return noise ? noise + (size_t)d * n : nullptr; };
+    unsigned d = 1 + (unsigned)i0 * (unsigned)(ncorr + (sc.predictor == USE_PRED_NONE ? 0 : 1));
+    const float* outw = (const float*)(h->blob + h->outw_off); const float* outb = (const float*)(h->blob + h->outb_off);
+    const X4Out x4{(float2*)h->x4, pcp / 2};
+    hipStream_t st[MAX_SUB]; int ib[MAX_SUB]; long first[MAX_SUB], cnt[MAX_SUB];
+    for (int i = 0, b = 0; i < nsub; b += h->sub_B[i++]) {
+        st[i] = i ? h->aux_stream[i] : s; ib[i] = b; first[i] = b * n_per_b; cnt[i] = h->sub_B[i] * n_per_b;
+    }
+    (void)hipEventRecord(h->ev_fork, s);
+    for (int i = 1; i < nsub; ++i) (void)hipStreamWaitEvent(st[i], h->ev_fork, 0);
+    auto eval = [&](int i, const float* temb, const float* t) {
+        if (i) (void)hipStreamWaitEvent(st[i], h->ev_stagger[i - 1], 0);
+        Fwd f{h, st[i], temb, 0, t, 0};
+        f.B = h->sub_B[i]; f.arena = i ? &h->sub_arena[i] : &h->arena; f.st_arena = &h->st_arena[i]; f.primary = i == 0;
+        if (i + 1 < nsub) { f.ev_stagger = h->ev_stagger[i]; f.stagger_level = g_stagger_level; }
+        Act pyr = f.run(h->x4 + (size_t)first[i] * pcp);
+        if (!h->dry) launch_score_out((const float*)pyr.p, pcp, t, 0, outw, outb, h->score + first[i], h->sub_B[i], n_per_b, -1.f, st[i]);
+    };
+    if (i0 == 0)
+        for (int i = 0; i < nsub; ++i) {
+            if (per_item) launch_prior_items(h->Y, nz(0), ItemRng{h->item_seeds, 0}, ouve_std(h->cfg, 1.0f), h->X, h->sub_B[i], n_per_b, st[i], ib[i], x4);
+            else launch_prior(h->Y, nz(0), RngRef{h->rng_state, 0}, ouve_std(h->cfg, 1.0f), h->X, cnt[i], st[i], first[i], x4);
+        }
+    for (int it = i0; it < i1; ++it) {
+        const float t = h->timesteps[it];
+        const float* temb = h->temb_table + (size_t)it * h->dense_rows;
+        for (int k = 0; k < ncorr; ++k, ++d) {
+            const RngRef rr{h->rng_state, d};
+            const ItemRng ir{h->item_seeds, d};
+            const float sd = sc.snr * ouve_std(h->cfg, t);
+            if (!per_item && sc.corrector == USE_CORR_LANGEVIN) {
+                for (int i = 0; i < nsub; ++i) {
+                    eval(i, temb, h->ts_dev + it);
+                    launch_langevin_norms(h->score, nz(d), rr, h->lang_partial, h->sub_B[i], n_per_b, h->lang_blocks, st[i], ib[i]);
+                    if (i) (void)hipEventRecord(h->ev_join[i], st[i]);
+                }
+                for (int i = 1; i < nsub; ++i) (void)hipStreamWaitEvent(s, h->ev_join[i], 0);
+                launch_langevin_step(h->lang_partial, h->B, h->lang_blocks, sc.snr, h->lang_step, s);
+                (void)hipEventRecord(h->ev_step, s);
+                for (int i = 0; i < nsub; ++i) {
+                    if (i) (void)hipStreamWaitEvent(st[i], h->ev_step, 0);
+                    launch_corrector(h->X, h->score, nz(d), rr, h->lang_step, 0.f, h->X, nullptr, cnt[i], st[i], first[i], x4);
+                }
+                continue;
+            }
+            for (int i = 0; i < nsub; ++i) {
+                eval(i, temb, h->ts_dev + it);
+                if (per_item && sc.corrector == USE_CORR_LANGEVIN) {
+                    launch_langevin_norms_items(h->score, nz(d), ir, h->lang_partial, h->sub_B[i], n_per_b, h->lang_blocks, st[i], ib[i]);
+                    launch_langevin_step_items(h->lang_partial, h->sub_B[i], h->lang_blocks, sc.snr, h->item_step, st[i], ib[i]);
+                    launch_corrector_items(h->X, h->score, nz(d), ir, h->item_step, 0.f, h->X, nullptr, h->sub_B[i], n_per_b, st[i], ib[i], x4);
+                } else if (per_item) {
+                    launch_corrector_items(h->X, h->score, nz(d), ir, nullptr, sd * sd * 2.f, h->X, nullptr, h->sub_B[i], n_per_b, st[i], ib[i], x4);
+                } else {
+                    launch_corrector(h->X, h->score, nz(d), rr, nullptr, sd * sd * 2.f, h->X, nullptr, cnt[i], st[i], first[i], x4);
+                }
+            }
+        }
+        const bool last = it == sc.N - 1;
+        if (sc.predictor == USE_PRED_NONE) {
+            if (last)
+                for (int i = 0; i < nsub; ++i)
+                    (void)hipMemcpyAsync(h->Xmean + first[i], h->X + first[i], (size_t)cnt[i] * 8, hipMemcpyDeviceToDevice, st[i]);
+        } else {
+            float cd, cs, cn; predictor_coeffs(h->cfg, sc.predictor, t, sc.N, cd, cs, cn);
+            for (int i = 0; i < nsub; ++i) {
+                eval(i, temb, h->ts_dev + it);
+                if (per_item)
+                    launch_predictor_items(h->X, h->Y, h->score, nz(d), ItemRng{h->item_seeds, d}, cd, cs, cn, h->X, last ? h->Xmean : nullptr,
+                                           h->sub_B[i], n_per_b, st[i], ib[i], x4);
+                else
+                    launch_predictor(h->X, h->Y, h->score, nz(d), RngRef{h->rng_state, d}, cd, cs, cn, h->X, last ? h->Xmean : nullptr,
+                                     cnt[i], st[i], first[i], x4);
+            }
+            d++;
+        }
+    }
+    for (int i = 1; i < nsub; ++i) { (void)hipEventRecord(h->ev_join[i], st[i]); (void)hipStreamWaitEvent(s, h->ev_join[i], 0); }
+}
+
 static void run_sampler(use_handle* h, const float2* noise, hipStream_t s, int i0, int i1, bool per_item = false) {
+    if (cross_eval_on(h)) { run_sampler_cross(h, noise, s, i0, i1, per_item); return; }
     const use_sampler_config& sc = h->sc;
     const long n = (long)h->B * h->cfg.n_freq * h->T, n_per_b = (long)h->cfg.n_freq * h->T;
     const int ncorr = sc.corrector == USE_CORR_NONE ? 0 : sc.corrector_steps;
@@ -895,6 +985,7 @@
     if (!strcmp(name, "subbatch_min_items")) { g_subbatch_min_items = (int)std::max(1LL, value); return USE_OK; }
     if (!strcmp(name, "subbatch")) { g_subbatch = (int)value; return USE_OK; }
     if (!strcmp(name, "stagger_level")) { g_stagger_level = (int)value; return USE_OK; }
+    if (!strcmp(name, "cross_eval")) { g_cross_eval = value != 0; return USE_OK; }
     if (!strcmp(name, "stats_part")) { g_stats_part = (int)value; return USE_OK; }
     if (!strcmp(name, "gn_inline")) { g_gn_inline = (long)value; return USE_OK; }
     if (!strcmp(name, "conv_v4_min_blocks")) { conv_v4_set_min_blocks((long)value); return USE_OK; }
@@ -942,6 +1033,7 @@
         if (h->ev_stagger[i]) { (void)hipEventDestroy(h->ev_stagger[i]); (void)hipEventDestroy(h->ev_join[i]); }
     }
     if (h->ev_fork) (void)hipEventDestroy(h->ev_fork);
+    if (h->ev_step) (void)hipEventDestroy(h->ev_step);
     if (h->blob) (void)hipFree(h->blob);
     if (h->arena.base) (void)hipFree(h->arena.base);
     if (h->persist) (void)hipFree(h->persist);
@@ -1158,6 +1250,7 @@
         for (int i = 0; i < h->nsub; ++i) { h->sub_arena[i].dry_on_overflow = &h->dry; h->st_arena[i].dry_on_overflow = &h->dry; }
     }
     if (h->nsub > 1 && !h->ev_fork) HIPCHK(hipEventCreateWithFlags(&h->ev_fork, hipEventDisableTiming));
+    if (h->nsub > 1 && !h->ev_step) HIPCHK(hipEventCreateWithFlags(&h->ev_step, hipEventDisableTiming));
     for (int i = 0; i < h->nsub; ++i) {
         if (i && !h->aux_stream[i]) HIPCHK(hipStreamCreateWithFlags(&h->aux_stream[i], hipStreamNonBlocking));
         if (h->nsub > 1 && !h->ev_stagger[i]) {
@@ -1361,13 +1454,14 @@
     return use_sample_cond2(h, y, cond, nullptr, noise, seed, out, stream);
 }
 
-static int load_sampler_inputs(use_handle* h, const void* y, const void* cond, const void* cond2, hipStream_t s) {
+static int load_sampler_inputs(use_handle* h, const void* y, const void* cond, const void* cond2, hipStream_t s, bool pack_cond = false) {
     const size_t n = (size_t)h->B * h->cfg.n_freq * h->T;
     HIPCHK(hipMemcpyAsync(h->Y, y, n * 8, hipMemcpyDeviceToDevice, s));
     if (cond2) HIPCHK(hipMemcpyAsync(h->cond2_buf, cond2, n * 8, hipMemcpyDeviceToDevice, s));
     float2* want = cond ? h->cond_buf : h->Y;
     if (want != h->Cond) { HIPCHK(hipStreamSynchronize(s)); drop_graphs(h); h->Cond = want; }
     if (cond) HIPCHK(hipMemcpyAsync(h->cond_buf, cond, n * 8, hipMemcpyDeviceToDevice, s));
+    if (pack_cond) launch_pack_input(h->Y, h->Cond, h->pcp == 8 ? h->cond2_buf : nullptr, h->x4, (long)n, s);
     return USE_OK;
 }
 
@@ -1394,7 +1488,7 @@
                                                               : "this network takes one conditioning tensor");
     hipStream_t s = (hipStream_t)stream;
     const size_t n = (size_t)h->B * h->cfg.n_freq * h->T;
-    rc = load_sampler_inputs(h, y, cond, cond2, s); if (rc) return rc;
+    rc = load_sampler_inputs(h, y, cond, cond2, s, cross_eval_on(h)); if (rc) return rc;
     if (per_item) { if (seeds_host) upload_item_seeds(h->item_seeds, seeds_host, h->B, s); }
     else hipLaunchKernelGGL(set_rng_kernel, dim3(1), dim3(1), 0, s, h->rng_state, (unsigned long long)seed, 0ull);
     if (!h->sc.use_graph) {
@@ -1935,6 +2029,87 @@
         const float sd = snr * ouve_std(h->cfg, t);
         launch_corrector((const float2*)x, (const float2*)score, (const float2*)noise, rr, nullptr, sd * sd * 2.f, (float2*)x_out, (float2*)x_mean, n, s);
     } else return fail(USE_E_INVALID, "corrector id %d has no update kernel", corrector);
+    HIPCHK(hipGetLastError());
+    return USE_OK;
+}
+
+static int sde_range_args(use_handle* h, int B, int64_t n_per_b, int b0, int nb, const void* x4, int pcp) {
+    if (B < 1 || B > use_handle::SDE_MAX_B || n_per_b < 1 || b0 < 0 || nb < 1 || b0 + nb > B) return fail(USE_E_INVALID, "item range [%d, %d) of B=%d", b0, b0 + nb, B);
+    if (x4 && pcp != 4 && pcp != 8) return fail(USE_E_INVALID, "x4 has 4 or 8 stored channels");
+    return ensure_sde_scratch(h);
+}
+static void sde_range_rng(use_handle* h, uint64_t seed, const uint64_t* item_seeds_host, int B, hipStream_t s) {
+    if (item_seeds_host) upload_item_seeds(h->sde_seeds, item_seeds_host, B, s);
+    else hipLaunchKernelGGL(set_rng_kernel, dim3(1), dim3(1), 0, s, h->sde_rng, (unsigned long long)seed, 0ull);
+}
+
+int use_op_sde_prior(use_handle* h, const void* y, const void* noise, uint64_t seed, const uint64_t* item_seeds_host, void* x, float* x4,
+                     int pcp, int B, int64_t n_per_b, int b0, int nb, use_stream_t st) {
+    if (!y || !x) return fail(USE_E_INVALID, "null tensor");
+    int rc = sde_range_args(h, B, n_per_b, b0, nb, x4, pcp); if (rc) return rc;
+    hipStream_t s = (hipStream_t)st;
+    sde_range_rng(h, seed, item_seeds_host, B, s);
+    const X4Out xo{(float2*)x4, pcp / 2};
+    if (item_seeds_host) launch_prior_items((const float2*)y, (const float2*)noise, ItemRng{h->sde_seeds, 0}, ouve_std(h->cfg, 1.0f), (float2*)x, nb, (long)n_per_b, s, b0, xo);
+    else launch_prior((const float2*)y, (const float2*)noise, RngRef{h->sde_rng, 0}, ouve_std(h->cfg, 1.0f), (float2*)x, (long)(nb * n_per_b), s, (long)(b0 * n_per_b), xo);
+    HIPCHK(hipGetLastError());
+    return USE_OK;
+}
+
+int use_op_sde_predictor(use_handle* h, int predictor, float t, int N, const void* x, const void* y, const void* score, const void* noise,
+                         uint64_t seed, const uint64_t* item_seeds_host, void* x_out, void* x_mean, float* x4, int pcp, int B, int64_t n_per_b,
+                         int b0, int nb, use_stream_t st) {
+    if (!x || !y || !score || !x_out) return fail(USE_E_INVALID, "null tensor");
+    if (predictor != USE_PRED_REVERSE_DIFFUSION && predictor != USE_PRED_EULER_MARUYAMA) return fail(USE_E_INVALID, "predictor id %d has no update kernel", predictor);
+    int rc = sde_range_args(h, B, n_per_b, b0, nb, x4, pcp); if (rc) return rc;
+    hipStream_t s = (hipStream_t)st;
+    float cd, cs, cn; predictor_coeffs(h->cfg, predictor, t, N, cd, cs, cn);
+    sde_range_rng(h, seed, item_seeds_host, B, s);
+    const X4Out xo{(float2*)x4, pcp / 2};
+    if (item_seeds_host)
+        launch_predictor_items((const float2*)x, (const float2*)y, (const float2*)score, (const float2*)noise, ItemRng{h->sde_seeds, 0}, cd, cs, cn,
+                               (float2*)x_out, (float2*)x_mean, nb, (long)n_per_b, s, b0, xo);
+    else
+        launch_predictor((const float2*)x, (const float2*)y, (const float2*)score, (const float2*)noise, RngRef{h->sde_rng, 0}, cd, cs, cn,
+                         (float2*)x_out, (float2*)x_mean, (long)(nb * n_per_b), s, (long)(b0 * n_per_b), xo);
+    HIPCHK(hipGetLastError());
+    return USE_OK;
+}
+
+int use_op_sde_langevin_norms(use_handle* h, const void* score, const void* noise, uint64_t seed, const uint64_t* item_seeds_host, float* partial,
+                              int blocks_per_b, int B, int64_t n_per_b, int b0, int nb, use_stream_t st) {
+    if (!score || !partial || blocks_per_b < 1 || blocks_per_b > 65535) return fail(USE_E_INVALID, "null tensor or bad blocks_per_b");
+    int rc = sde_range_args(h, B, n_per_b, b0, nb, nullptr, 4); if (rc) return rc;
+    hipStream_t s = (hipStream_t)st;
+    sde_range_rng(h, seed, item_seeds_host, B, s);
+    if (item_seeds_host) launch_langevin_norms_items((const float2*)score, (const float2*)noise, ItemRng{h->sde_seeds, 0}, partial, nb, (long)n_per_b, blocks_per_b, s, b0);
+    else launch_langevin_norms((const float2*)score, (const float2*)noise, RngRef{h->sde_rng, 0}, partial, nb, (long)n_per_b, blocks_per_b, s, b0);
+    HIPCHK(hipGetLastError());
+    return USE_OK;
+}
+
+int use_op_sde_langevin_step(const float* partial, int blocks_per_b, float snr, float* step, int per_item, int B, int b0, int nb, use_stream_t st) {
+    if (!partial || !step || blocks_per_b < 1 || B < 1 || b0 < 0 || nb < 1 || b0 + nb > B) return fail(USE_E_INVALID, "use_op_sde_langevin_step: bad arguments");
+    if (per_item) launch_langevin_step_items(partial, nb, blocks_per_b, snr, step, (hipStream_t)st, b0);
+    else launch_langevin_step(partial, B, blocks_per_b, snr, step, (hipStream_t)st);
+    HIPCHK(hipGetLastError());
+    return USE_OK;
+}
+
+int use_op_sde_corrector(use_handle* h, const void* x, const void* score, const void* noise, uint64_t seed, const uint64_t* item_seeds_host,
+                         const float* step_dev, float step_host, void* x_out, void* x_mean, float* x4, int pcp, int B, int64_t n_per_b, int b0,
+                         int nb, use_stream_t st) {
+    if (!x || !score || !x_out) return fail(USE_E_INVALID, "null tensor");
+    int rc = sde_range_args(h, B, n_per_b, b0, nb, x4, pcp); if (rc) return rc;
+    hipStream_t s = (hipStream_t)st;
+    sde_range_rng(h, seed, item_seeds_host, B, s);
+    const X4Out xo{(float2*)x4, pcp / 2};
+    if (item_seeds_host)
+        launch_corrector_items((const float2*)x, (const float2*)score, (const float2*)noise, ItemRng{h->sde_seeds, 0}, step_dev, step_host,
+                               (float2*)x_out, (float2*)x_mean, nb, (long)n_per_b, s, b0, xo);
+    else
+        launch_corrector((const float2*)x, (const float2*)score, (const float2*)noise, RngRef{h->sde_rng, 0}, step_dev, step_host,
+                         (float2*)x_out, (float2*)x_mean, (long)(nb * n_per_b), s, (long)(b0 * n_per_b), xo);
     HIPCHK(hipGetLastError());
     return USE_OK;
 }
diff --git a/universal_speech_enhancement_amd/csrc/use_kernels.h b/universal_speech_enhancement_amd/csrc/use_kernels.h
--- a/universal_speech_enhancement_amd/csrc/use_kernels.h
+++ b/universal_speech_enhancement_amd/csrc/use_kernels.h
@@ -158,28 +158,32 @@
                           const float* bias, float* bias_out, hipStream_t s);
 
 struct RngRef { const unsigned long long* state; unsigned draw; };
-void launch_prior(const float2* y, const float2* noise, RngRef rng, float std1, float2* x, long n, hipStream_t s);
+struct X4Out { float2* p = nullptr; int stride = 2; };
+void launch_prior(const float2* y, const float2* noise, RngRef rng, float std1, float2* x, long n, hipStream_t s,
+                  long first = 0, X4Out x4 = {});
 void launch_predictor(const float2* x, const float2* y, const float2* score, const float2* noise, RngRef rng,
                       float c_drift, float c_score, float c_noise, float2* x_out, float2* x_mean, long n,
-                      hipStream_t s);
+                      hipStream_t s, long first = 0, X4Out x4 = {});
 void launch_langevin_norms(const float2* score, const float2* noise, RngRef rng, float* partial, int B,
-                           long n_per_b, int blocks_per_b, hipStream_t s);
+                           long n_per_b, int blocks_per_b, hipStream_t s, int b0 = 0);
 void launch_langevin_step(const float* partial, int B, int blocks_per_b, float snr, float* step, hipStream_t s);
 void launch_corrector(const float2* x, const float2* score, const float2* noise, RngRef rng, const float* step_dev,
-                      float step_host, float2* x_out, float2* x_mean, long n, hipStream_t s);
+                      float step_host, float2* x_out, float2* x_mean, long n, hipStream_t s, long first = 0,
+                      X4Out x4 = {});
 void launch_fill_noise(float2* out, RngRef rng, long n, hipStream_t s);
 struct ItemRng { const unsigned long long* seeds; unsigned draw; };
 void launch_prior_items(const float2* y, const float2* noise, ItemRng rng, float std1, float2* x, int B, long n_per_b,
-                        hipStream_t s);
+                        hipStream_t s, int b0 = 0, X4Out x4 = {});
 void launch_predictor_items(const float2* x, const float2* y, const float2* score, const float2* noise, ItemRng rng,
                             float c_drift, float c_score, float c_noise, float2* x_out, float2* x_mean, int B,
-                            long n_per_b, hipStream_t s);
+                            long n_per_b, hipStream_t s, int b0 = 0, X4Out x4 = {});
 void launch_langevin_norms_items(const float2* score, const float2* noise, ItemRng rng, float* partial, int B,
-                                 long n_per_b, int blocks_per_b, hipStream_t s);
-void launch_langevin_step_items(const float* partial, int B, int blocks_per_b, float snr, float* step, hipStream_t s);
+                                 long n_per_b, int blocks_per_b, hipStream_t s, int b0 = 0);
+void launch_langevin_step_items(const float* partial, int B, int blocks_per_b, float snr, float* step, hipStream_t s,
+                                int b0 = 0);
 void launch_corrector_items(const float2* x, const float2* score, const float2* noise, ItemRng rng,
                             const float* step_dev, float step_host, float2* x_out, float2* x_mean, int B, long n_per_b,
-                            hipStream_t s);
+                            hipStream_t s, int b0 = 0, X4Out x4 = {});
 void launch_fill_noise_items(float2* out, ItemRng rng, int B, long n_per_b, hipStream_t s);
 
 struct OdeGroup {
diff --git a/universal_speech_enhancement_amd/csrc/use_kernels.hip b/universal_speech_enhancement_amd/csrc/use_kernels.hip
--- a/universal_speech_enhancement_amd/csrc/use_kernels.hip
+++ b/universal_speech_enhancement_amd/csrc/use_kernels.hip
@@ -1808,42 +1808,54 @@
     hipLaunchKernelGGL(fill_noise_kernel, dim3(ew_blocks(n)), dim3(256), 0, s, out, rng, n);
 }
 
+DEVI void put_x4(X4Out o, long i, float vx, float vy) {
+    if (o.p) o.p[i * o.stride] = make_float2(2.f * vx - 1.f, 2.f * vy - 1.f);
+}
+
 __global__ __launch_bounds__(256) void prior_kernel(const float2* __restrict__ y, const float2* __restrict__ noise,
-                                                    RngRef rng, float std1, float2* __restrict__ x, long n) {
-    for (long i = (long)blockIdx.x * 256 + threadIdx.x; i < n; i += (long)gridDim.x * 256) {
+                                                    RngRef rng, float std1, float2* __restrict__ x, X4Out x4, long first,
+                                                    long n) {
+    for (long k = (long)blockIdx.x * 256 + threadIdx.x; k < n; k += (long)gridDim.x * 256) {
+        const long i = first + k;
         const float2 z = get_noise(noise, rng, i), yy = y[i];
-        x[i] = make_float2(yy.x + z.x * std1, yy.y + z.y * std1);
-    }
-}
-void launch_prior(const float2* y, const float2* noise, RngRef rng, float std1, float2* x, long n, hipStream_t s) {
-    hipLaunchKernelGGL(prior_kernel, dim3(ew_blocks(n)), dim3(256), 0, s, y, noise, rng, std1, x, n);
+        const float vx = yy.x + z.x * std1, vy = yy.y + z.y * std1;
+        x[i] = make_float2(vx, vy);
+        put_x4(x4, i, vx, vy);
+    }
+}
+void launch_prior(const float2* y, const float2* noise, RngRef rng, float std1, float2* x, long n, hipStream_t s,
+                  long first, X4Out x4) {
+    hipLaunchKernelGGL(prior_kernel, dim3(ew_blocks(n)), dim3(256), 0, s, y, noise, rng, std1, x, x4, first, n);
 }
 
 __global__ __launch_bounds__(256) void predictor_kernel(const float2* __restrict__ x, const float2* __restrict__ y,
                                                         const float2* __restrict__ score,
                                                         const float2* __restrict__ noise, RngRef rng, float c_drift,
                                                         float c_score, float c_noise, float2* __restrict__ x_out,
-                                                        float2* __restrict__ x_mean, long n) {
-    for (long i = (long)blockIdx.x * 256 + threadIdx.x; i < n; i += (long)gridDim.x * 256) {
+                                                        float2* __restrict__ x_mean, X4Out x4, long first, long n) {
+    for (long k = (long)blockIdx.x * 256 + threadIdx.x; k < n; k += (long)gridDim.x * 256) {
+        const long i = first + k;
         const float2 xv = x[i], yv = y[i], sv = score[i], z = get_noise(noise, rng, i);
         const float fx = c_drift * (yv.x - xv.x) - c_score * sv.x;
         const float fy = c_drift * (yv.y - xv.y) - c_score * sv.y;
         const float mx = xv.x - fx, my = xv.y - fy;
         if (x_mean) x_mean[i] = make_float2(mx, my);
-        x_out[i] = make_float2(mx + c_noise * z.x, my + c_noise * z.y);
+        const float vx = mx + c_noise * z.x, vy = my + c_noise * z.y;
+        x_out[i] = make_float2(vx, vy);
+        put_x4(x4, i, vx, vy);
     }
 }
 void launch_predictor(const float2* x, const float2* y, const float2* score, const float2* noise, RngRef rng,
                       float c_drift, float c_score, float c_noise, float2* x_out, float2* x_mean, long n,
-                      hipStream_t s) {
+                      hipStream_t s, long first, X4Out x4) {
     hipLaunchKernelGGL(predictor_kernel, dim3(ew_blocks(n)), dim3(256), 0, s, x, y, score, noise, rng, c_drift,
-                       c_score, c_noise, x_out, x_mean, n);
+                       c_score, c_noise, x_out, x_mean, x4, first, n);
 }
 
 __global__ __launch_bounds__(256) void langevin_norms_kernel(const float2* __restrict__ score,
                                                              const float2* __restrict__ noise, RngRef rng,
-                                                             float* __restrict__ partial, long n_per_b) {
-    const int b = blockIdx.y;
+                                                             float* __restrict__ partial, long n_per_b, int b0) {
+    const int b = b0 + blockIdx.y;
     float g2 = 0.f, z2 = 0.f;
     for (long i = (long)blockIdx.x * 256 + threadIdx.x; i < n_per_b; i += (long)gridDim.x * 256) {
         const long gi = (long)b * n_per_b + i;
@@ -1860,9 +1872,9 @@
     }
 }
 void launch_langevin_norms(const float2* score, const float2* noise, RngRef rng, float* partial, int B,
-                           long n_per_b, int blocks_per_b, hipStream_t s) {
+                           long n_per_b, int blocks_per_b, hipStream_t s, int b0) {
     hipLaunchKernelGGL(langevin_norms_kernel, dim3(blocks_per_b, B), dim3(256), 0, s, score, noise, rng, partial,
-                       n_per_b);
+                       n_per_b, b0);
 }
 
 __global__ __launch_bounds__(64) void langevin_step_kernel(const float* __restrict__ partial, int B, int blocks_per_b,
@@ -1891,20 +1903,23 @@
                                                         const float2* __restrict__ noise, RngRef rng,
                                                         const float* __restrict__ step_dev, float step_host,
                                                         float2* __restrict__ x_out, float2* __restrict__ x_mean,
-                                                        long n) {
+                                                        X4Out x4, long first, long n) {
     const float eps = step_dev ? step_dev[0] : step_host;
     const float sq = sqrtf(eps * 2.f);
-    for (long i = (long)blockIdx.x * 256 + threadIdx.x; i < n; i += (long)gridDim.x * 256) {
+    for (long k = (long)blockIdx.x * 256 + threadIdx.x; k < n; k += (long)gridDim.x * 256) {
+        const long i = first + k;
         const float2 xv = x[i], g = score[i], z = get_noise(noise, rng, i);
         const float mx = xv.x + eps * g.x, my = xv.y + eps * g.y;
         if (x_mean) x_mean[i] = make_float2(mx, my);
-        x_out[i] = make_float2(mx + z.x * sq, my + z.y * sq);
+        const float vx = mx + z.x * sq, vy = my + z.y * sq;
+        x_out[i] = make_float2(vx, vy);
+        put_x4(x4, i, vx, vy);
     }
 }
 void launch_corrector(const float2* x, const float2* score, const float2* noise, RngRef rng, const float* step_dev,
-                      float step_host, float2* x_out, float2* x_mean, long n, hipStream_t s) {
+                      float step_host, float2* x_out, float2* x_mean, long n, hipStream_t s, long first, X4Out x4) {
     hipLaunchKernelGGL(corrector_kernel, dim3(ew_blocks(n)), dim3(256), 0, s, x, score, noise, rng, step_dev,
-                       step_host, x_out, x_mean, n);
+                       step_host, x_out, x_mean, x4, first, n);
 }
 
 DEVI float2 get_noise_item(const float2* noise, ItemRng rng, int b, long n_per_b, long j) {
@@ -1929,18 +1944,21 @@
 }
 
 __global__ __launch_bounds__(256) void prior_items_kernel(const float2* __restrict__ y, const float2* __restrict__ noise,
-                                                          ItemRng rng, float std1, float2* __restrict__ x, long n_per_b) {
-    const int b = blockIdx.y;
+                                                          ItemRng rng, float std1, float2* __restrict__ x, X4Out x4, int b0,
+                                                          long n_per_b) {
+    const int b = b0 + blockIdx.y;
     for (long j = (long)blockIdx.x * 256 + threadIdx.x; j < n_per_b; j += (long)gridDim.x * 256) {
         const long i = (long)b * n_per_b + j;
         const float2 z = get_noise_item(noise, rng, b, n_per_b, j), yy = y[i];
-        x[i] = make_float2(yy.x + z.x * std1, yy.y + z.y * std1);
+        const float vx = yy.x + z.x * std1, vy = yy.y + z.y * std1;
+        x[i] = make_float2(vx, vy);
+        put_x4(x4, i, vx, vy);
     }
 }
 void launch_prior_items(const float2* y, const float2* noise, ItemRng rng, float std1, float2* x, int B, long n_per_b,
-                        hipStream_t s) {
+                        hipStream_t s, int b0, X4Out x4) {
     hipLaunchKernelGGL(prior_items_kernel, dim3(item_blocks(n_per_b, B), B), dim3(256), 0, s, y, noise, rng, std1, x,
-                       n_per_b);
+                       x4, b0, n_per_b);
 }
 
 __global__ __launch_bounds__(256) void predictor_items_kernel(const float2* __restrict__ x, const float2* __restrict__ y,
@@ -1948,8 +1966,8 @@
                                                               const float2* __restrict__ noise, ItemRng rng,
                                                               float c_drift, float c_score, float c_noise,
                                                               float2* __restrict__ x_out, float2* __restrict__ x_mean,
-                                                              long n_per_b) {
-    const int b = blockIdx.y;
+                                                              X4Out x4, int b0, long n_per_b) {
+    const int b = b0 + blockIdx.y;
     for (long j = (long)blockIdx.x * 256 + threadIdx.x; j < n_per_b; j += (long)gridDim.x * 256) {
         const long i = (long)b * n_per_b + j;
         const float2 xv = x[i], yv = y[i], sv = score[i], z = get_noise_item(noise, rng, b, n_per_b, j);
@@ -1957,20 +1975,22 @@
         const float fy = c_drift * (yv.y - xv.y) - c_score * sv.y;
         const float mx = xv.x - fx, my = xv.y - fy;
         if (x_mean) x_mean[i] = make_float2(mx, my);
-        x_out[i] = make_float2(mx + c_noise * z.x, my + c_noise * z.y);
+        const float vx = mx + c_noise * z.x, vy = my + c_noise * z.y;
+        x_out[i] = make_float2(vx, vy);
+        put_x4(x4, i, vx, vy);
     }
 }
 void launch_predictor_items(const float2* x, const float2* y, const float2* score, const float2* noise, ItemRng rng,
                             float c_drift, float c_score, float c_noise, float2* x_out, float2* x_mean, int B,
-                            long n_per_b, hipStream_t s) {
+                            long n_per_b, hipStream_t s, int b0, X4Out x4) {
     hipLaunchKernelGGL(predictor_items_kernel, dim3(item_blocks(n_per_b, B), B), dim3(256), 0, s, x, y, score, noise,
-                       rng, c_drift, c_score, c_noise, x_out, x_mean, n_per_b);
+                       rng, c_drift, c_score, c_noise, x_out, x_mean, x4, b0, n_per_b);
 }
 
 __global__ __launch_bounds__(256) void langevin_norms_items_kernel(const float2* __restrict__ score,
                                                                    const float2* __restrict__ noise, ItemRng rng,
-                                                                   float* __restrict__ partial, long n_per_b) {
-    const int b = blockIdx.y;
+                                                                   float* __restrict__ partial, long n_per_b, int b0) {
+    const int b = b0 + blockIdx.y;
     float g2 = 0.f, z2 = 0.f;
     for (long j = (long)blockIdx.x * 256 + threadIdx.x; j < n_per_b; j += (long)gridDim.x * 256) {
         const float2 g = score[(long)b * n_per_b + j], z = get_noise_item(noise, rng, b, n_per_b, j);
@@ -1986,14 +2006,14 @@
     }
 }
 void launch_langevin_norms_items(const float2* score, const float2* noise, ItemRng rng, float* partial, int B,
-                                 long n_per_b, int blocks_per_b, hipStream_t s) {
+                                 long n_per_b, int blocks_per_b, hipStream_t s, int b0) {
     hipLaunchKernelGGL(langevin_norms_items_kernel, dim3(blocks_per_b, B), dim3(256), 0, s, score, noise, rng, partial,
-                       n_per_b);
+                       n_per_b, b0);
 }
 
 __global__ __launch_bounds__(64) void langevin_step_items_kernel(const float* __restrict__ partial, int blocks_per_b,
-                                                                 float snr, float* __restrict__ step) {
-    const int b = blockIdx.x;
+                                                                 float snr, float* __restrict__ step, int b0) {
+    const int b = b0 + blockIdx.x;
     double g2 = 0.0, z2 = 0.0;
     for (int k = threadIdx.x; k < blocks_per_b; k += 64) {
         g2 += (double)partial[((size_t)b * blocks_per_b + k) * 2];
@@ -2006,8 +2026,9 @@
         step[b] = r * r * 2.f;
     }
 }
-void launch_langevin_step_items(const float* partial, int B, int blocks_per_b, float snr, float* step, hipStream_t s) {
-    hipLaunchKernelGGL(langevin_step_items_kernel, dim3(B), dim3(64), 0, s, partial, blocks_per_b, snr, step);
+void launch_langevin_step_items(const float* partial, int B, int blocks_per_b, float snr, float* step, hipStream_t s,
+                                int b0) {
+    hipLaunchKernelGGL(langevin_step_items_kernel, dim3(B), dim3(64), 0, s, partial, blocks_per_b, snr, step, b0);
 }
 
 __global__ __launch_bounds__(256) void corrector_items_kernel(const float2* __restrict__ x,
@@ -2015,8 +2036,8 @@
                                                               const float2* __restrict__ noise, ItemRng rng,
                                                               const float* __restrict__ step_dev, float step_host,
                                                               float2* __restrict__ x_out, float2* __restrict__ x_mean,
-                                                              long n_per_b) {
-    const int b = blockIdx.y;
+                                                              X4Out x4, int b0, long n_per_b) {
+    const int b = b0 + blockIdx.y;
     const float eps = step_dev ? step_dev[b] : step_host;
     const float sq = sqrtf(eps * 2.f);
     for (long j = (long)blockIdx.x * 256 + threadIdx.x; j < n_per_b; j += (long)gridDim.x * 256) {
@@ -2024,14 +2045,16 @@
         const float2 xv = x[i], g = score[i], z = get_noise_item(noise, rng, b, n_per_b, j);
         const float mx = xv.x + eps * g.x, my = xv.y + eps * g.y;
         if (x_mean) x_mean[i] = make_float2(mx, my);
-        x_out[i] = make_float2(mx + z.x * sq, my + z.y * sq);
+        const float vx = mx + z.x * sq, vy = my + z.y * sq;
+        x_out[i] = make_float2(vx, vy);
+        put_x4(x4, i, vx, vy);
     }
 }
 void launch_corrector_items(const float2* x, const float2* score, const float2* noise, ItemRng rng,
                             const float* step_dev, float step_host, float2* x_out, float2* x_mean, int B, long n_per_b,
-                            hipStream_t s) {
+                            hipStream_t s, int b0, X4Out x4) {
     hipLaunchKernelGGL(corrector_items_kernel, dim3(item_blocks(n_per_b, B), B), dim3(256), 0, s, x, score, noise, rng,
-                       step_dev, step_host, x_out, x_mean, n_per_b);
-}
-
-}
+                       step_dev, step_host, x_out, x_mean, x4, b0, n_per_b);
+}
+
+}
```

Result: no change. 3665 spectrogram-frames/s, median of 6 (+0.5%).
